# ArthurBrussee/brush

Measured on AMD Instinct MI355X. Metric: train views/sec @ 1M Gaussians, 1080p (fwd + L1/SSIM loss + bwd + Adam per view), higher is better.
Workload: dtype f32

## Files before the change

brush_amd/_ffi.py:

```python
import ctypes as C
import os

_DIR = os.path.dirname(os.path.abspath(__file__))
LIB_PATH = os.environ.get("BRUSH_HIP_LIB") or os.path.join(_DIR, "libbrush_hip.so")

FLAG_MIP = 1
FLAG_BWD_INFO = 2
FLAG_SMOOTH_CUTOFF = 4
FLAG_SLICED_LISTS = 8

fp = C.POINTER(C.c_float)
u32p = C.POINTER(C.c_uint32)


class BhCamera(C.Structure):
    _fields_ = [
        ("vm", C.c_float * 12),
        ("fx", C.c_float), ("fy", C.c_float), ("cx", C.c_float), ("cy", C.c_float),
        ("lim_pos_x", C.c_float), ("lim_pos_y", C.c_float),
        ("lim_neg_x", C.c_float), ("lim_neg_y", C.c_float),
        ("cam_pos", C.c_float * 3),
        ("img_w", C.c_uint32), ("img_h", C.c_uint32),
        ("tile_row_begin", C.c_uint32), ("tile_row_end", C.c_uint32),
        ("model", C.c_uint32), ("dist", C.c_float * 8), ("half_max_render_fov", C.c_float),
# ... 345 lines not shown
                ("reserved", C.c_uint32)]


FEATURE_TRAIN_SYMBOLS = {
    "bh_train_set_features": (C.c_int, [C.c_void_p, C.POINTER(BhFeatureField), C.POINTER(BhFeatureTarget)]),
    "bh_refine_carry_rows": (C.c_int, [C.c_void_p, C.c_void_p, C.c_void_p, C.c_uint32, C.c_uint32]),
}

REGION_BOX, REGION_ELLIPSOID = 0, 1


class BhSceneTransform(C.Structure):
    _fields_ = [("q", C.c_double * 4), ("t", C.c_double * 3), ("s", C.c_double), ("rot", C.c_float * 9), ("quat", C.c_float * 4),
                ("trans", C.c_float * 3), ("scale", C.c_float), ("log_scale", C.c_float), ("sh_rot", C.c_float * 164),
                ("reserved", C.c_uint32 * 2)]


class BhSceneRegion(C.Structure):
    _fields_ = [("kind", C.c_uint32), ("invert", C.c_uint32), ("center", C.c_float * 3), ("half_extent", C.c_float * 3),
                ("rot", C.c_float * 9), ("min_raw_opacity", C.c_float), ("reserved", C.c_uint32)]


SCENE_SYMBOLS = {
    "bh_scene_transform_make": (C.c_int, [dp, dp, C.c_double, C.POINTER(BhSceneTransform)]),
    "bh_scene_transform_compose": (C.c_int, [C.POINTER(BhSceneTransform), C.POINTER(BhSceneTransform), C.POINTER(BhSceneTransform)]),
    "bh_scene_transform_invert": (C.c_int, [C.POINTER(BhSceneTransform), C.POINTER(BhSceneTransform)]),
    "bh_camera_apply_scene_transform": (C.c_int, [C.POINTER(BhCamera), C.POINTER(BhSceneTransform), C.POINTER(BhCamera)]),
    "bh_splats_transform": (C.c_int, [C.c_void_p, C.POINTER(BhSceneTransform), C.c_uint32, C.c_uint32] + [C.c_void_p] * 6),
    "bh_splats_select_region": (C.c_int, [C.c_void_p, C.POINTER(BhSceneRegion), C.c_void_p, C.c_void_p, C.c_uint32, C.c_void_p, u32p]),
}

LIFT_MAX_LABELS, LIFT_UNASSIGNED, LIFT_ANY_LABEL = 256, 255, 0xFFFFFFFF
LIFT_VOTE_ONE = 16777216.0


class BhLiftSelect(C.Structure):
    _fields_ = [("label", C.c_uint32), ("min_share", C.c_float), ("min_weight", C.c_float), ("min_max_weight", C.c_float),
                ("min_pixels", C.c_uint32), ("invert", C.c_uint32)]


LIFT_SYMBOLS = {
    "bh_lift_accumulate": (C.c_int, [C.c_void_p, C.POINTER(BhRenderOut), C.c_void_p, C.c_uint32, C.c_void_p, C.c_void_p, C.c_void_p]),
    "bh_lift_assign": (C.c_int, [C.c_void_p, C.c_void_p, C.c_uint32, C.c_uint32, C.c_float, C.c_void_p, C.c_void_p]),
    "bh_lift_select": (C.c_int, [C.c_void_p, C.c_void_p, C.c_void_p, C.c_void_p, C.c_uint32, C.c_uint32, C.POINTER(BhLiftSelect), C.c_void_p]),
}

ENVMAP_MAX_RESOLUTION = 1024
ENVMAP_SYMBOLS = {
    "bh_envmap_create": (C.c_int, [C.c_void_p, C.c_uint32, C.POINTER(C.c_void_p)]),
    "bh_envmap_destroy": (C.c_int, [C.c_void_p, C.c_void_p]),
    "bh_envmap_set_params": (C.c_int, [C.c_void_p, C.c_void_p, fp]),
    "bh_envmap_get_params": (C.c_int, [C.c_void_p, C.c_void_p, fp]),
    "bh_envmap_get_grad": (C.c_int, [C.c_void_p, C.c_void_p, fp]),
    "bh_envmap_get_state": (C.c_int, [C.c_void_p, C.c_void_p, fp, fp, u32p]),
    "bh_envmap_set_state": (C.c_int, [C.c_void_p, C.c_void_p, fp, fp, C.c_uint32]),
    "bh_envmap_set_adam": (C.c_int, [C.c_void_p, C.c_void_p, C.c_double, C.c_double, C.c_double, C.c_double]),
    "bh_envmap_composite": (C.c_int, [C.c_void_p, C.c_void_p, C.POINTER(BhCamera), C.c_void_p, C.c_uint32, C.c_uint32, C.c_void_p]),
    "bh_envmap_backward": (C.c_int, [C.c_void_p, C.c_void_p, C.POINTER(BhCamera), C.c_void_p, C.c_void_p, C.c_uint32, C.c_uint32, C.c_void_p, C.c_int]),
    "bh_train_set_envmap": (C.c_int, [C.c_void_p, C.c_void_p]),
}

class BhCameraGradTerms(C.Structure):
    _fields_ = [("v_depth", C.c_void_p), ("v_normal", C.c_void_p), ("v_distortion", C.c_void_p), ("depth_mode", C.c_uint32),
                ("normal_mode", C.c_uint32), ("distortion", BhDistortionConfig)]


INTRINSICS_SYMBOLS = {
    "bh_render_backward_intrinsics_saved": (C.c_int, [C.c_void_p, C.POINTER(BhRenderOut)] + [C.c_void_p] * 10),
    "bh_render_backward_camera_saved": (C.c_int, [C.c_void_p, C.POINTER(BhRenderOut), C.c_void_p, C.POINTER(BhCameraGradTerms)] + [C.c_void_p] * 9),
    "bh_train_set_intrinsics_grad": (C.c_int, [C.c_void_p, C.c_void_p]),
    "bh_camera_set_intrinsics": (C.c_int, [C.POINTER(BhCamera), C.c_double, C.c_double, C.c_double, C.c_double]),
}

ABI_VERSION = 7
STRUCT_MIRRORS = (BhCamera, BhRenderOut, BhLossConfig, BhTrainConfig, BhTrainState, BhTrainBatch, BhTrainStats, BhRefineConfig, BhRefineStats, BhPlyInfo)

_lib = None
_lib_th = None
TEST_HOOKS_LIB_PATH = os.path.join(_DIR, "libbrush_hip_testhooks.so")
TEST_HOOK_SYMBOLS = {"bh_debug_fill_train_scratch": (C.c_int, [C.c_void_p, C.c_uint32]),
                     "bh_debug_split_counts": (C.c_int, [C.c_void_p, C.POINTER(C.c_uint32)]),
                     "bh_debug_depth_sort": (C.c_int, [C.c_void_p, C.c_void_p, C.c_void_p, C.c_void_p, C.c_uint32, C.c_void_p, C.c_void_p, C.c_void_p, C.c_void_p,
                                                       C.POINTER(C.c_int), C.POINTER(C.c_uint32)]),
                     "bh_debug_image_loss_window": (C.c_int, [C.c_void_p, C.c_void_p, C.c_void_p, C.c_uint32, C.c_uint32, C.POINTER(BhLossConfig), C.c_float, C.c_uint32,
                                                              C.c_uint32, C.c_void_p, C.c_void_p])}


class BrushHipError(RuntimeError):
    pass


def _bind(path, symbols):
    if not os.path.exists(path):
        raise BrushHipError(
            "%s not found: build it with `python -c 'import __graft_entry__ as g; g.build()'` "
            "(hipcc --offload-arch=gfx950). There is no CPU fallback." % path)
    lib = C.CDLL(path)
    for name, (res, args) in symbols.items():
        fn = getattr(lib, name)
        fn.restype = res
        fn.argtypes = args
    if lib.bh_abi_version() != ABI_VERSION:
        raise BrushHipError("%s speaks ABI %d, this binding ABI %d" % (path, lib.bh_abi_version(), ABI_VERSION))
    for i, mirror in enumerate(STRUCT_MIRRORS):
        if lib.bh_struct_size(i) != C.sizeof(mirror):
            raise BrushHipError("%s: sizeof(%s) is %d in the library, %d in this binding" % (path, mirror.__name__, lib.bh_struct_size(i), C.sizeof(mirror)))
    return lib


def load():
    global _lib
    if _lib is None:
        _lib = _bind(LIB_PATH, dict(SYMBOLS, **LPIPS_SYMBOLS, **COMPRESSED_PLY_SYMBOLS, **IMAGE_SYMBOLS, **DEPTH_SYMBOLS, **POSE_SYMBOLS, **EXPOSURE_SYMBOLS, **BILAGRID_SYMBOLS, **DEPTH_LOSS_SYMBOLS, **NORMAL_SYMBOLS, **NORMAL_LOSS_SYMBOLS, **DISTORTION_SYMBOLS, **MESH_SYMBOLS, **FEATURE_SYMBOLS, **FEATURE_TRAIN_SYMBOLS, **SCENE_SYMBOLS, **LIFT_SYMBOLS, **ENVMAP_SYMBOLS, **INTRINSICS_SYMBOLS))
    return _lib


def load_test_hooks():
    global _lib_th
    if _lib_th is None:
        _lib_th = _bind(TEST_HOOKS_LIB_PATH, dict(SYMBOLS, **LPIPS_SYMBOLS, **COMPRESSED_PLY_SYMBOLS, **IMAGE_SYMBOLS, **DEPTH_SYMBOLS, **POSE_SYMBOLS, **EXPOSURE_SYMBOLS, **BILAGRID_SYMBOLS, **DEPTH_LOSS_SYMBOLS, **NORMAL_SYMBOLS, **NORMAL_LOSS_SYMBOLS, **DISTORTION_SYMBOLS, **MESH_SYMBOLS, **FEATURE_SYMBOLS, **FEATURE_TRAIN_SYMBOLS, **SCENE_SYMBOLS, **LIFT_SYMBOLS, **ENVMAP_SYMBOLS, **INTRINSICS_SYMBOLS,
                                                   **TEST_HOOK_SYMBOLS))
    return _lib_th
```

brush_amd/csrc/api.hip:

```cpp
#include <cmath>
#include <cstdlib>
#include <cstdio>
#include <algorithm>
#include <cstring>
#include <new>

#include "../../include/brush_hip_intrinsics.h"
#include "context.h"
#include "device_rng.h"
#include "param_table.h"

namespace bh {

__global__ __launch_bounds__(256) void zero_two_kernel(float4* __restrict__ a, size_t na, float4* __restrict__ b, size_t nb) {
    const size_t stride = (size_t)gridDim.x * 256;
    const float4 z = make_float4(0.0f, 0.0f, 0.0f, 0.0f);
    for (size_t i = (size_t)blockIdx.x * 256 + threadIdx.x; i < na + nb; i += stride) {
        if (i < na) a[i] = z;
        else b[i - na] = z;
    }
}

int set_error(bh_ctx* ctx, int code, const std::string& msg) {
    if (ctx) ctx->last_error = msg;
    return code;
}

int check_hip(bh_ctx* ctx, hipError_t e, const char* what) {
    if (e == hipSuccess) return 0;
    std::string m = std::string(what) + ": " + hipGetErrorString(e);
    (void)hipGetLastError();
    return set_error(ctx, e == hipErrorOutOfMemory ? BH_ERR_OOM : BH_ERR_HIP, m);
}

static inline void cpu_relax() {
#if defined(__x86_64__) || defined(__i386__)
    __builtin_ia32_pause();
#elif defined(__aarch64__)
    __asm__ __volatile__("yield");
#endif
}
int wait_host_tag(bh_ctx* ctx, const volatile uint32_t* word, uint32_t want, const char* what) {
    for (uint64_t it = 1; it < (1ull << 21); ++it) {
        if (*word == want) return 0;
        if ((it & 0x3FFFull) == 0ull) {
            const hipError_t q = hipStreamQuery(ctx->stream);
            if (q == hipSuccess) break;
            if (q != hipErrorNotReady) return check_hip(ctx, q, what);
        }
        cpu_relax();
    }
    if (*word == want) return 0;
    BH_HIP(ctx, hipEventRecord(ctx->readback_ev, ctx->stream));
    BH_HIP(ctx, hipEventSynchronize(ctx->readback_ev));
    if (*word == want) return 0;
    return set_error(ctx, BH_ERR_STATE, std::string(what) + ": the kernel that signals the host never stored its tag");
}

void* ensure(bh_ctx* ctx, Slot s, size_t bytes) {
    Buffer& b = ctx->slots[s];
    if (bytes == 0) bytes = 16;
    if (b.cap >= bytes) return b.ptr;
    if (b.ptr) {
        (void)hipStreamSynchronize(ctx->stream);
        (void)hipFree(b.ptr);
        b.ptr = nullptr;
        b.cap = 0;
    }
    {
        int best = -1;
        for (size_t i = 0; i < ctx->pool.size(); ++i)
            if (ctx->pool[i].cap >= bytes && ctx->pool[i].cap <= 2 * bytes + 4096 && (best < 0 || ctx->pool[i].cap < ctx->pool[(size_t)best].cap)) best = (int)i;
        if (best >= 0) {
            b = ctx->pool[(size_t)best];
            ctx->pool.erase(ctx->pool.begin() + best);
            return b.ptr;
        }
    }
    size_t cap = bytes + bytes / 4;
    cap = (cap + 255) & ~(size_t)255;
    void* p = nullptr;
    hipError_t e = hipMalloc(&p, cap);
    if (e != hipSuccess) {
        (void)hipGetLastError();
        cap = (bytes + 255) & ~(size_t)255;
        e = hipMalloc(&p, cap);
    }
    if (e != hipSuccess) {
        char msg[160];
        snprintf(msg, sizeof msg, "hipMalloc(%zu bytes) for scratch slot %d failed: %s", cap, (int)s, hipGetErrorString(e));
        (void)hipGetLastError();
// ... 97 lines not shown
uint32_t bh_abi_version(void) { return BH_ABI_VERSION; }

uint32_t bh_struct_size(uint32_t which) {
    switch (which) {
        case BH_STRUCT_CAMERA: return (uint32_t)sizeof(BhCamera);
        case BH_STRUCT_RENDER_OUT: return (uint32_t)sizeof(BhRenderOut);
        case BH_STRUCT_LOSS_CONFIG: return (uint32_t)sizeof(BhLossConfig);
        case BH_STRUCT_TRAIN_CONFIG: return (uint32_t)sizeof(BhTrainConfig);
        case BH_STRUCT_TRAIN_STATE: return (uint32_t)sizeof(BhTrainState);
        case BH_STRUCT_TRAIN_BATCH: return (uint32_t)sizeof(BhTrainBatch);
        case BH_STRUCT_TRAIN_STATS: return (uint32_t)sizeof(BhTrainStats);
        case BH_STRUCT_REFINE_CONFIG: return (uint32_t)sizeof(BhRefineConfig);
        case BH_STRUCT_REFINE_STATS: return (uint32_t)sizeof(BhRefineStats);
        case BH_STRUCT_PLY_INFO: return (uint32_t)sizeof(BhPlyInfo);
        default: return 0u;
    }
}

bh_ctx* bh_create(int device, void* stream, int own_stream) {
    bh_ctx* ctx = new (std::nothrow) bh_ctx();
    if (!ctx) return nullptr;
    ctx->device = device;
    if (hipSetDevice(device) != hipSuccess) {
        (void)hipGetLastError();
        delete ctx;
        return nullptr;
    }
    if (!own_stream) {
        ctx->stream = (hipStream_t)stream;
        ctx->owns_stream = false;
    } else {
        if (hipStreamCreateWithFlags(&ctx->stream, hipStreamNonBlocking) != hipSuccess) {
            (void)hipGetLastError();
            delete ctx;
            return nullptr;
        }
        ctx->owns_stream = true;
    }
    if (hipHostMalloc((void**)&ctx->host_counters, bh::HOST_COUNTERS_BYTES, hipHostMallocCoherent)    != hipSuccess) {
        (void)hipGetLastError();
        if (ctx->owns_stream) (void)hipStreamDestroy(ctx->stream);
        delete ctx;
        return nullptr;
    }
    std::memset(ctx->host_counters, 0, bh::HOST_COUNTERS_BYTES);
#ifdef BH_TEST_HOOKS
    ctx->knob_break_allreduce = getenv("BH_BREAK_ALLREDUCE") != nullptr;
    if (ctx->knob_break_allreduce)
        fprintf(stderr, "brush_hip: BH_BREAK_ALLREDUCE is set - every all-reduce of this context's communicator is deliberately CORRUPTED (test hook)\n");
    if (const char* e = getenv("BH_TEST_FAIL_LOSS_AT")) {
        ctx->knob_fail_loss_at = (uint32_t)atoi(e);
        if (ctx->knob_fail_loss_at) fprintf(stderr, "brush_hip: BH_TEST_FAIL_LOSS_AT=%u - that train step of this context will FAIL on purpose (test hook)\n", ctx->knob_fail_loss_at);
    }
#endif
    if (hipEventCreateWithFlags(&ctx->readback_ev, hipEventDisableTiming) != hipSuccess ||
        hipEventCreateWithFlags(&ctx->gate_ev, hipEventDisableTiming) != hipSuccess) {
        if (ctx->readback_ev) (void)hipEventDestroy(ctx->readback_ev);
        (void)hipGetLastError();
        (void)hipHostFree(ctx->host_counters);
        if (ctx->owns_stream) (void)hipStreamDestroy(ctx->stream);
        delete ctx;
        return nullptr;
    }
    return ctx;
}

void bh_destroy(bh_ctx* ctx) {
    if (!ctx) return;
    (void)hipSetDevice(ctx->device);
    (void)hipStreamSynchronize(ctx->stream);
    prof_resolve(ctx);
    for (hipEvent_t e : ctx->prof.pool) (void)hipEventDestroy(e);
    for (auto& b : ctx->slots)
        if (b.ptr) (void)hipFree(b.ptr);
    for (auto& kv : ctx->views)
        if (kv.second.zcut) (void)hipFree(kv.second.zcut);
    for (auto& rt : ctx->retained)
        for (auto& b : rt.blocks)
            if (b.ptr) (void)hipFree(b.ptr);
    for (auto& b : ctx->pool)
        if (b.ptr) (void)hipFree(b.ptr);
    if (ctx->host_counters) (void)hipHostFree(ctx->host_counters);
    if (ctx->dsort_spl) (void)hipFree(ctx->dsort_spl);
    if (ctx->sort_groups) (void)hipFree(ctx->sort_groups);
    if (ctx->readback_ev) (void)hipEventDestroy(ctx->readback_ev);
    if (ctx->gate_ev) (void)hipEventDestroy(ctx->gate_ev);
    if (ctx->image_tab_host) (void)hipHostFree(ctx->image_tab_host);
    if (ctx->image_tab_ev) (void)hipEventDestroy(ctx->image_tab_ev);
    bh::param_tables_free_all(ctx);
    if (ctx->comm) (void)bh_comm_destroy(ctx);
    if (ctx->owns_stream) (void)hipStreamDestroy(ctx->stream);
    delete ctx;
}

const char* bh_last_error(bh_ctx* ctx) { return ctx ? ctx->last_error.c_str() : "null context"; }

int bh_sync(bh_ctx* ctx) {
    if (!ctx) return BH_ERR_INVALID_ARG;
    if (ctx->far_job.pending) {
        BH_HIP(ctx, hipSetDevice(ctx->device));
        BH_TRY(finish_far_slice(ctx, nullptr));
    }
    BH_HIP(ctx, hipStreamSynchronize(ctx->stream));
    deliver_pending_loss(ctx);
    return 0;
}

int bh_profile_enable(bh_ctx* ctx, int on) {
    if (!ctx) return BH_ERR_INVALID_ARG;
    ctx->prof.level = on < 0 ? 0 : (on > 2 ? 1 : on);
    return 0;
}

int bh_profile_fetch(bh_ctx* ctx, const char** names, float* ms, uint32_t* calls, int cap) {
    if (!ctx) return BH_ERR_INVALID_ARG;
    prof_resolve(ctx);
    Profiler& p = ctx->prof;
    const int n = p.count < cap ? p.count : cap;
    for (int i = 0; i < n; ++i) {
        names[i] = p.names[i];
        ms[i] = p.ms[i];
        calls[i] = p.calls[i];
    }
    p.count = 0;
    return n;
}

namespace {
bool parse_u32(const char* v, uint32_t lo, uint32_t hi, uint32_t* out) {
    if (!v || !*v) return false;
    char* end = nullptr;
    const unsigned long long x = strtoull(v, &end, 10);
    if (*end != '\0' || x < lo || x > hi) return false;
    *out = (uint32_t)x;
    return true;
}
bool parse_flag(const char* v, bool* out) {
    uint32_t x = 0;
    if (!parse_u32(v, 0, 1, &x)) return false;
    *out = x != 0;
    return true;
}
struct Option { const char* name; const char* help; bool (*apply)(bh_ctx* c, const char* v); };
const Option kOptions[] = {
    {"cut_min_pairs", "u32: a view whose last frame had fewer pairs keeps complete lists (= bh_set_list_cut_threshold)",
     [](bh_ctx* c, const char* v) { return parse_u32(v, 0, 0xFFFFFFFFu, &c->cut_min_pairs); }},
    {"cut_margin_pct", "0..10000: base margin behind a tile's last useful splat, % of its depth rank (default 150)",
     [](bh_ctx* c, const char* v) { return parse_u32(v, 0, 10000, &c->knob_cut_margin_pct); }},
    {"cut_margin_fixed", "0|1: the margin is cut_margin_pct for every frame instead of adaptive",
     [](bh_ctx* c, const char* v) { return parse_flag(v, &c->knob_fixed_margin); }},
    {"cut_ctrl", "up:down:floor:gap_exp — the margin controller's constants (default 1.5:0.998:0.5:0.3333)", [](bh_ctx* c, const char* v) {
        float a = 0, b = 0, d = 0, e = 0;
        if (sscanf(v, "%f:%f:%f:%f", &a, &b, &d, &e) != 4 || !(a >= 1.0f && b > 0.0f && b <= 1.0f && d > 0.0f && e >= 0.0f && e <= 1.0f)) return false;
        c->ctrl_up = a; c->ctrl_down = b; c->ctrl_floor = d; c->ctrl_gap_exp = e;
        return true;
    }},
    {"cut_sort_all", "0|1: with per-tile cuts, still depth-sort every visible splat",
     [](bh_ctx* c, const char* v) { return parse_flag(v, &c->knob_cut_sort_all); }},
    {"auto_exact_share", "0..1: a view whose last cut frame listed more than this share of its pairs renders complete lists (default 0.9; 0 = never)", [](bh_ctx* c, const char* v) {
        char* end = nullptr;
        const float x = strtof(v, &end);
        if (end == v || *end != '\0' || !(x >= 0.0f && x <= 1.0f)) return false;
        c->auto_exact_share = x;
        return true;
    }},
    {"no_view_hash", "0|1: frames without a view id share ONE table instead of being keyed by their camera",
     [](bh_ctx* c, const char* v) { return parse_flag(v, &c->knob_no_view_hash); }},
    {"k16_order", "0 index order | 1 by the view's last per-tile work | 2 dealt: the forward blend's tile order",
     [](bh_ctx* c, const char* v) { return parse_u32(v, 0, 2, &c->knob_k16_order); }},
    {"band_mode", "0|1: XCD bands of the blend kernels — contiguous eighths of the tile range, or dealt in chunks of 8 adjacent tiles (default 1)",
     [](bh_ctx* c, const char* v) { return parse_u32(v, 0, 1, &c->knob_band_mode); }},
    {"k16_waves", "0..8: forward blend: resident one-wave tiles per SIMD (0 = 8 = all resident at once; fewer: the lighter tiles are dispatched as the heavier ones finish)",
     [](bh_ctx* c, const char* v) { return parse_u32(v, 0, 8, &c->knob_k16_waves); }},
    {"k16_split", "0..1000: forward blend: a tile whose forecast work is at least max(256, k16_split / 100 x its band's mean) is blended by four quadrant waves (default 250; 0: no tile is split)",
     [](bh_ctx* c, const char* v) { return parse_u32(v, 0, 1000, &c->knob_k16_split); }},
    {"k16_split_of_max", "0..100: ... and at least this many percent of its band's heaviest tile (default 45)",
     [](bh_ctx* c, const char* v) { return parse_u32(v, 0, 100, &c->knob_k16_split_of_max); }},
    {"k16_split_min", "1..1023: a tile below this many blended splats (forecast) is never split (default 256)",
     [](bh_ctx* c, const char* v) { return parse_u32(v, 1, 1023, &c->knob_k16_split_min); }},
    {"k5_exact_spw", "16|32|64: splats per wave of the list builder for complete lists",
     [](bh_ctx* c, const char* v) { uint32_t u = 0; if (!parse_u32(v, 16, 64, &u) || !(u == 16 || u == 32 || u == 64)) return false; c->knob_k5_exact_spw = u; return true; }},
    {"bwd_jobs", "0|1: the blend backward works on checkpointed 128-entry segments of the tiles' lists (default 1) or on whole tiles",
     [](bh_ctx* c, const char* v) { return parse_flag(v, &c->knob_bwd_jobs); }},
    {"bwd_wide_rows", "0|1: the blend backward addresses the gradient accumulator in 64 bits, as it does by itself from 2^32 bytes of accumulator on (default 0)",
     [](bh_ctx* c, const char* v) { return parse_flag(v, &c->knob_bwd_wide_rows); }},
    {"no_lpt", "0|1: the blend backward takes its tiles in index order",
     [](bh_ctx* c, const char* v) { return parse_flag(v, &c->knob_no_lpt); }},
    {"lpt_classes", "log|linear: work classes of the backward's longest-first tile order — two per octave of blended splats, or 1/64 of the mean list length wide",
     [](bh_ctx* c, const char* v) { const std::string w(v); if (w == "log") { c->knob_lpt_linear = false; return true; } if (w == "linear") { c->knob_lpt_linear = true; return true; } return false; }},
    {"generic_depth_sort", "0|1: depth order by the generic radix sort + scan instead of the fused split sort",
     [](bh_ctx* c, const char* v) { return parse_flag(v, &c->knob_generic_depth_sort); }},
    {"dsort_splitters", "0|1: the fused depth sort splits at the 254 depth quantiles of the view's previous frame (default 1) or always linearly over the frame's key range",
     [](bh_ctx* c, const char* v) { return parse_flag(v, &c->knob_dsort_splitters); }},
    {"tile_sort", "auto|bucket|lsd: the forward's tile sort (auto: bucket sort unless the view's pairs are concentrated in few tiles)",
     [](bh_ctx* c, const char* v) { const std::string w(v); if (w == "auto") { c->knob_tile_sort = 0; return true; } if (w == "bucket") { c->knob_tile_sort = 1; return true; } if (w == "lsd") { c->knob_tile_sort = 2; return true; } return false; }},
    {"spec_k5", "0|1: queue the list builder before the host has read the frame's counts (default 1; 0: behind the count readback)",
     [](bh_ctx* c, const char* v) { return parse_flag(v, &c->knob_spec_k5); }},
    {"event_waits", "0|1: the host's mid-step waits use events behind the kernels instead of polled tag words",
     [](bh_ctx* c, const char* v) { return parse_flag(v, &c->knob_event_waits); }},
    {"readback_copy", "0|1: counts and gate word reach the host through copy launches",
     [](bh_ctx* c, const char* v) { return parse_flag(v, &c->knob_readback_copy); }},
    {"force_exchange", "0|1: a one-rank communicator still walks the whole gradient-exchange path (overhead measurement)",
     [](bh_ctx* c, const char* v) { return parse_flag(v, &c->knob_force_exchange); }},
    {"zero_grads", "0|1: the single-GPU train step zero-fills its gradient span like the exchange path",
     [](bh_ctx* c, const char* v) { return parse_flag(v, &c->knob_zero_grads); }},
    {"loss_bands", "0|1: the fused loss's blocks take their tiles by XCD column bands (1) or row-major (0)",
     [](bh_ctx* c, const char* v) { return parse_u32(v, 0, 1, &c->knob_loss_bands); }},
    {"update_rows", "0|64|128|256: splats per block of the update kernel (0 = default)",
     [](bh_ctx* c, const char* v) { uint32_t u = 0; if (!parse_u32(v, 0, 256, &u) || !(u == 0 || u == 64 || u == 128 || u == 256)) return false; c->knob_update_rows = u; return true; }},
    {"no_dormant", "0|1: the update kernel fetches and updates dormant splats like everyone else",
     [](bh_ctx* c, const char* v) { return parse_flag(v, &c->knob_no_dormant); }},
    {"sort_kpt", "0|4|8|16: keys per thread of the generic radix sort (0 = default)",
     [](bh_ctx* c, const char* v) { uint32_t u = 0; if (!parse_u32(v, 0, 16, &u) || !(u == 0 || u == 4 || u == 8 || u == 16)) return false; c->knob_sort_kpt = u; return true; }},
    {"grad_allreduce", "ring|direct: the dense gradient block's collective — ncclAllReduce, or reduce-scatter + all-gather over grouped send/recv",
     [](bh_ctx* c, const char* v) { const std::string w(v); if (w == "ring") { c->knob_direct_allreduce = false; return true; } if (w == "direct") { c->knob_direct_allreduce = true; return true; } return false; }},
    {"update_sparse", "0..256: an update block with at most this many non-dormant rows fetches them in one round trip (0: never; 256: every block that may skip dormant rows; default 64 at SH degree 0, else 0)",
     [](bh_ctx* c, const char* v) { uint32_t u = 0; if (!parse_u32(v, 0, 256, &u)) return false; c->knob_update_sparse = (int)u; return true; }},
    {"feature_chunk", "0|4|8|16: channels per pass over the lists of the feature-map blends (0 = chosen per channel count)",
     [](bh_ctx* c, const char* v) { uint32_t u = 0; if (!parse_u32(v, 0, 16, &u) || !(u == 0 || u == 4 || u == 8 || u == 16)) return false; c->feature_chunk = u; return true; }},
};
constexpr int kOptionCount = (int)(sizeof(kOptions) / sizeof(kOptions[0]));
}

extern "C" int bh_option_count(void) { return kOptionCount; }
extern "C" const char* bh_option_name(int i) { return i >= 0 && i < kOptionCount ? kOptions[i].name : nullptr; }
extern "C" const char* bh_option_help(int i) { return i >= 0 && i < kOptionCount ? kOptions[i].help : nullptr; }

extern "C" int bh_set_option(bh_ctx* ctx, const char* key, const char* value) {
    if (!ctx) return BH_ERR_INVALID_ARG;
    if (!key || !value) return set_error(ctx, BH_ERR_INVALID_ARG, "set_option: null key or value");
    const std::string k(key);
    for (const Option& o : kOptions) {
        if (k != o.name) continue;
        if (!o.apply(ctx, value)) return set_error(ctx, BH_ERR_INVALID_ARG, "set_option: bad value '" + std::string(value) + "' for '" + k + "'");
        return 0;
    }
    return set_error(ctx, BH_ERR_INVALID_ARG, "set_option: unknown key '" + k + "' (bh_option_name lists the keys)");
}

namespace {
struct Kb4Law {
    double k[4];
    explicit Kb4Law(const float* d) { for (int i = 0; i < 4; ++i) k[i] = d ? (double)d[i] : 0.0; }
    double value(double th) const {
        const double t2 = th * th, t3 = t2 * th, t5 = t3 * t2, t7 = t5 * t2, t9 = t7 * t2;
        return th + k[0] * t3 + k[1] * t5 + k[2] * t7 + k[3] * t9;
    }
    double slope(double th) const {
        const double t2 = th * th, t4 = t2 * t2, t6 = t4 * t2, t8 = t6 * t2;
        return 1.0 + 3.0 * k[0] * t2 + 5.0 * k[1] * t4 + 7.0 * k[2] * t6 + 9.0 * k[3] * t8;
    }
    double invert(double target) const {
        if (target <= 0.0) return 0.0;
        const double pi = 3.14159265358979323846;
        double th = target < pi - 1e-6 ? target : pi - 1e-6;
        for (int it = 0; it < 50; ++it) {
            const double fp = slope(th);
            if (std::fabs(fp) < 1e-12) break;
            double next = th - (value(th) - target) / fp;
            next = next < 0.0 ? 0.0 : (next > pi ? pi : next);
            const bool done = std::fabs(next - th) < 1e-12;
            th = next;
            if (done) break;
        }
        return th;
    }
};
struct Rt8Law {
    double k[6];
    explicit Rt8Law(const float* d) { for (int i = 0; i < 6; ++i) k[i] = d ? (double)d[i] : 0.0; }
    double radial(double r) const {
        const double r2 = r * r, r4 = r2 * r2, r6 = r4 * r2;
        return (1.0 + k[0] * r2 + k[1] * r4 + k[2] * r6) / (1.0 + k[3] * r2 + k[4] * r4 + k[5] * r6);
    }
    double undistort(double r_d) const {
        double r = r_d;
// ... 140 lines not shown
    if (!ctx) return BH_ERR_INVALID_ARG;
    if (!cam || !out || !background) return set_error(ctx, BH_ERR_INVALID_ARG, "render_forward: null argument");
    ForwardRequest req;
    req.cam = *cam;
    req.n = n; req.sh_degree = sh_degree; req.flags = flags;
    req.transforms = transforms; req.sh_coeffs = sh_coeffs; req.raw_opacities = raw_opacities;
    req.bg[0] = background[0]; req.bg[1] = background[1]; req.bg[2] = background[2];
    req.view_id = ctx->view_id;
    return render_forward(ctx, req, out);
}

int bh::forward_impl(bh_ctx* ctx, const ForwardRequest& req, BhRenderOut* out) {
    const uint32_t n = req.n, sh_degree = req.sh_degree, flags = req.flags;
    const float* transforms = req.transforms;
    const float* sh_coeffs = req.sh_coeffs;
    const float* raw_opacities = req.raw_opacities;
    ctx->have_forward = false;
    ctx->clears.begin_forward();
    const bool mip = flags & BH_FLAG_MIP;
    Frame f;
    f.bwd_info = flags & BH_FLAG_BWD_INFO; f.smooth = flags & BH_FLAG_SMOOTH_CUTOFF;
    f.bg[0] = req.bg[0]; f.bg[1] = req.bg[1]; f.bg[2] = req.bg[2];
    f.u = make_uniforms(req.cam);
    if (f.u.tile_y0 >= f.u.tile_y1 || f.u.tile_y1 > f.u.tile_bh) return set_error(ctx, BH_ERR_INVALID_ARG, "tile_row window must satisfy begin < end <= ceil(img_h / 16)");
    f.num_tiles = f.u.tile_bw * f.u.tile_bh;
    const size_t npad = n ? n : 1;

    constexpr size_t counter_set_bytes = COUNTER_SET_BYTES, counter_set_words = COUNTER_SET_BYTES / 4, counter_read_bytes = COUNTER_READ_BYTES;
    auto* counter_pairs = (uint32_t*)ensure(ctx, SLOT_COUNTERS, 2 * counter_set_bytes + 64);
    uint32_t* dev_sums = counter_pairs ? counter_pairs + 2 * counter_set_words : nullptr;
    uint32_t* counters = counter_pairs ? counter_pairs + counter_set_words * (ctx->counter_phase & 1u) : nullptr;
    auto* depth_keys = (uint32_t*)ensure(ctx, SLOT_DEPTH_KEYS, npad * 4);
    auto* isect_counts = (uint32_t*)ensure(ctx, SLOT_ISECT_COUNTS, npad * 4);
    auto* max_radius = req.max_radius ? req.max_radius : (float*)ensure(ctx, SLOT_MAX_RADIUS, npad * 4);
    f.proj_by_gid = (float*)ensure(ctx, SLOT_PROJECTED_BY_GID, npad * 9 * 4);
    if (!counters || !depth_keys || !isect_counts || !max_radius || !f.proj_by_gid) return BH_ERR_OOM;

    f.gfc = (uint32_t*)ensure(ctx, SLOT_GLOBAL_FROM_COMPACT, npad * 4);
    auto* depths_sorted = (uint32_t*)ensure(ctx, SLOT_DEPTHS_SORTED, npad * 4);
    if (!f.gfc || !depths_sorted) return BH_ERR_OOM;
    const bool bwd_jobs = f.bwd_info && ctx->knob_bwd_jobs && !ctx->knob_no_lpt && !((flags & BH_FLAG_SLICED_LISTS) && ctx->slice_fraction > 0.0f);
    const size_t lpt_words = LPT_HEADER_WORDS + (size_t)8 * LPT_CLASSES * band_slots(f.num_tiles);
    auto* tile_offsets = (uint32_t*)ensure(ctx, SLOT_TILE_OFFSETS, ((size_t)f.num_tiles * 2 + lpt_words) * 4);
    f.visible = (f.bwd_info && req.visible) ? req.visible : (float*)ensure(ctx, SLOT_VISIBLE, (f.bwd_info ? npad : 1) * 4);
    if (!tile_offsets || !f.visible) return BH_ERR_OOM;
    const size_t visible_words = f.bwd_info ? ((req.visible && req.visible_floats) ? req.visible_floats : npad) : 0;
    const bool want_sliced = (flags & BH_FLAG_SLICED_LISTS) != 0;
    const size_t slice_bit_words = ((size_t)f.num_tiles + 31) / 32;
    const size_t slice_group_words = (size_t)n / (256 * FAR_GROUP_BLOCKS) + 2;
    const size_t slice_words = want_sliced ? SLICE_CTRL_WORDS + slice_bit_words + (size_t)f.num_tiles * 2 + slice_group_words : 0;
    uint32_t* slice_tab = nullptr;
    if (want_sliced) {
        slice_tab = (uint32_t*)ensure(ctx, SLOT_SLICE, slice_words * 4);
        if (!slice_tab) return BH_ERR_OOM;
    }
    ViewState* view = nullptr;
    bool cut_active = false;
    const bool auto_cuts = want_sliced && !(ctx->slice_fraction > 0.0f);
    const bool order_only = !want_sliced && ctx->knob_k16_order != 0u && n >= 8u * 256u;
    if (n > 0 && (auto_cuts || order_only)) {
        view = frame_view(ctx, req, f.u.tile_bw, f.u.tile_bh, order_only && !f.bwd_info);
        if (!view && auto_cuts) return set_error(ctx, BH_ERR_OOM, "hipMalloc for the per-view tile table failed");
        if (!view) (void)hipGetLastError();
        cut_active = auto_cuts && view && cut_this_frame(ctx, view, req.allow_cut);
    }
    uint32_t* const vtab = view_table(view);
    uint32_t* near_counts = nullptr;
    uint32_t* tile_order = nullptr;
    uint32_t* tile_split = nullptr;
    if (cut_active) {
        near_counts = (uint32_t*)ensure(ctx, SLOT_NEAR_COUNTS, npad * 4);
        if (!near_counts) return BH_ERR_OOM;
    }

    uint32_t near_total = 0, nv_true = 0;
    bool fused_scan = false;
    uint32_t* cum_early = nullptr;
    bool k5_queued = false;
    uint32_t spec_pair_cap = 0;
    float* spec_projected = nullptr;
    float4* spec_vc = nullptr;
    uint32_t *spec_tile_ids = nullptr, *spec_isect_gids = nullptr;
    if (n > 0) {
        {
            ProfScope ps(ctx, "ProjectSplats");
            if (!ctx->counters_ready) BH_HIP(ctx, hipMemsetAsync(counter_pairs, 0, 2 * counter_set_bytes, ctx->stream));
            ctx->counters_ready = false;
            ForwardPrep prep;
            prep.next_counters = reinterpret_cast<unsigned long long*>(counter_pairs + counter_set_words * ((ctx->counter_phase & 1u) ^ 1u));
            prep.visible = visible_words ? reinterpret_cast<uint32_t*>(f.visible) : nullptr;
            prep.visible_words = (uint32_t)visible_words;
            prep.tile_table = tile_offsets;
            prep.tile_words = f.num_tiles * 2 + LPT_HEADER_WORDS;
            prep.slice_table = slice_tab;
            prep.slice_words = (uint32_t)slice_words;
            prep.list_all_visible = ctx->knob_cut_sort_all;
            if (view && ctx->knob_k16_order && n >= 8u * 256u) {
                const uint32_t win_t = f.u.tile_bw * (f.u.tile_y1 - f.u.tile_y0);
                tile_order = (uint32_t*)ensure(ctx, SLOT_TILE_ORDER, ((size_t)8 * band_slots(win_t) + SPLIT_TAIL_WORDS) * 4);
                if (!tile_order) return BH_ERR_OOM;
                prep.order_work = vtab + (size_t)f.num_tiles;
                prep.order_out = tile_order;
                prep.order_tiles = win_t;
                prep.order_tile_begin = f.u.tile_bw * f.u.tile_y0;
                prep.order_mode = ctx->knob_k16_order;
                prep.band_mode = ctx->knob_band_mode;
                if (ctx->knob_k16_split && ctx->knob_k16_order == 1u) {
                    tile_split = tile_order + (size_t)8 * band_slots(win_t);
                    prep.split_out = tile_split;
                    prep.split_factor = (float)ctx->knob_k16_split * 0.01f;
                    prep.split_min = ctx->knob_k16_split_min;
                    prep.split_of_max = (float)ctx->knob_k16_split_of_max * 0.01f;
                }
            }
            if (f.bwd_info && req.grad_begin && req.grad_floats && (req.grad_floats & 3u) == 0 &&
                (reinterpret_cast<uintptr_t>(req.grad_begin) & 15u) == 0 && req.grad_floats / 4 <= 0xFFFFFFFFull) {
                prep.span = reinterpret_cast<float4*>(req.grad_begin);
                prep.span_f4 = (uint32_t)(req.grad_floats / 4);
                ctx->clears.k1_cleared_span();
            }
            BH_TRY(launch_project_forward(ctx, f.u, n, mip, sh_degree, transforms, sh_coeffs, raw_opacities, depth_keys, isect_counts, max_radius,
                                          f.proj_by_gid, counters, prep, cut_active ? vtab : nullptr, near_counts));
            ctx->counter_phase ^= 1u;
            ctx->counters_ready = true;
        }
        auto* hslots = reinterpret_cast<unsigned long long*>(ctx->host_counters + 16);
        fused_scan = depth_sort_supported(n) && !ctx->knob_generic_depth_sort;
        const bool sums_on_device = fused_scan && !ctx->knob_readback_copy;
        const bool poll_tag = sums_on_device && !ctx->knob_event_waits;
        if (!sums_on_device) {
            BH_HIP(ctx, hipMemcpyAsync(hslots, counters, counter_read_bytes, hipMemcpyDeviceToHost, ctx->stream));
            BH_HIP(ctx, hipEventRecord(ctx->readback_ev, ctx->stream));
        }
        {
            ProfScope ps(ctx, "DepthSort");
            if (fused_scan) {
                cum_early = (uint32_t*)ensure(ctx, SLOT_CUM_TILES_HIT, npad * 4);
                if (!cum_early) return BH_ERR_OOM;
                if (poll_tag && ++ctx->readback_tag == 0u) ctx->readback_tag = 1u;
                bool* spl_written = nullptr;
                uint32_t* spl = view_splitters(view, cut_active, &spl_written);
                BH_TRY(depth_sort_scan(ctx, depth_keys, counters + COUNTER_MINMAX_WORD, cut_active ? near_counts : isect_counts, n, depths_sorted, f.gfc, cum_early,
                                       sums_on_device ? counters : nullptr, ctx->host_counters + 16, ctx->readback_ev, poll_tag ? ctx->readback_tag : 0u,
                                       sums_on_device ? dev_sums : nullptr, spl, spl_written));
            } else {
                BH_TRY(radix_argsort(ctx, depth_keys, nullptr, n, 32, depths_sorted, f.gfc));
            }
        }
        if (poll_tag && ctx->knob_spec_k5 && !(want_sliced && ctx->slice_fraction > 0.0f)) {
            const size_t cap_pairs = std::min(ctx->slots[SLOT_TILE_IDS].cap, ctx->slots[SLOT_ISECT_GIDS].cap) / 4;
            if (cap_pairs >= 4096) {
                spec_projected = (float*)ensure(ctx, SLOT_PROJECTED, npad * 9 * 4);
                spec_vc = f.bwd_info ? (float4*)ensure(ctx, SLOT_V_COMBINED, npad * 10 * 4 + 16) : nullptr;
                if (!spec_projected || (f.bwd_info && !spec_vc)) return BH_ERR_OOM;
                spec_tile_ids = (uint32_t*)ctx->slots[SLOT_TILE_IDS].ptr;
                spec_isect_gids = (uint32_t*)ctx->slots[SLOT_ISECT_GIDS].ptr;
                spec_pair_cap = (uint32_t)std::min<size_t>(cap_pairs, 0xFFFFFFFEull);
                ProfScope ps(ctx, "MapGaussiansToIntersect");
                BH_TRY(launch_map_gaussians(ctx, n, f.u, f.proj_by_gid, f.gfc, spec_projected, cum_early, spec_tile_ids, spec_isect_gids, spec_vc,
                                            spec_vc ? (uint32_t)(((size_t)n * 10 + 3) / 4) : 0u, 0xFFFFFFFFu, cut_active ? slice_tab : nullptr,
                                            cut_active ? vtab : nullptr, cut_active ? depths_sorted : nullptr, dev_sums + (cut_active ? 3 : 0), spec_pair_cap));
                k5_queued = true;
            }
        }
        if (poll_tag) BH_TRY(wait_host_tag(ctx, reinterpret_cast<const volatile uint32_t*>(hslots) + HOST_SUM_WORDS - 1u, ctx->readback_tag, "count readback"));
        else BH_HIP(ctx, hipEventSynchronize(ctx->readback_ev));
        if (ctx->gate_learn) {
            ctx->gate_learn = false;
            ctx->far_direct = reinterpret_cast<const volatile uint32_t*>(ctx->host_counters)[HOST_GATE_WORD] != 0u;
        }
        unsigned long long hc[4] = {0ull, 0ull, 0ull, 0ull};
        if (sums_on_device) {
            const volatile unsigned long long* hs = hslots;
            for (uint32_t c = 0; c < COUNTER_K1_U64; ++c) hc[c] = hs[c];
        } else {
            for (uint32_t k = 0; k < COUNTER_SLOTS; ++k)
                for (uint32_t c = 0; c < COUNTER_K1_U64; ++c) hc[c] += hslots[COUNTER_K1_U64 * k + c];
        }
        if (hc[1] > 0xFFFFFFFFull) return set_error(ctx, BH_ERR_UNSUPPORTED, "more than 2^32-1 tile intersections");
        nv_true = (uint32_t)hc[0];
        f.ni = (uint32_t)hc[1];
        near_total = cut_active ? (uint32_t)hc[2] : f.ni;
        f.nv = cut_active ? (uint32_t)hc[3] : nv_true;
    } else {
        BH_HIP(ctx, hipMemsetAsync(tile_offsets, 0, ((size_t)f.num_tiles * 2 + LPT_HEADER_WORDS) * 4, ctx->stream));
        if (visible_words) BH_HIP(ctx, hipMemsetAsync(f.visible, 0, visible_words * 4, ctx->stream));
    }

    const size_t nvpad = f.nv ? f.nv : 1, nipad = f.ni ? f.ni : 1;
    f.cum = fused_scan ? cum_early : (uint32_t*)ensure(ctx, SLOT_CUM_TILES_HIT, nvpad * 4);
    f.projected = (float*)ensure(ctx, SLOT_PROJECTED, nvpad * 9 * 4);
    f.tile_ids = (uint32_t*)ensure(ctx, SLOT_TILE_IDS, nipad * 4);
    f.isect_gids = (uint32_t*)ensure(ctx, SLOT_ISECT_GIDS, nipad * 4);
    f.tile_ids_sorted = (uint32_t*)ensure(ctx, SLOT_TILE_IDS_SORTED, nipad * 4);
    f.isect_gids_sorted = (uint32_t*)ensure(ctx, SLOT_ISECT_GIDS_SORTED, nipad * 4);
    const size_t pixels = (size_t)f.u.img_w * f.u.img_h;
    void* out_img = ensure(ctx, SLOT_OUT_IMG, pixels * (f.bwd_info ? 16 : 4));
    if (!f.cum || !f.projected || !f.tile_ids || !f.isect_gids || !f.tile_ids_sorted || !f.isect_gids_sorted || !out_img)
        return BH_ERR_OOM;
    if (k5_queued && ((cut_active ? near_total : f.ni) > spec_pair_cap || f.projected != spec_projected || f.tile_ids != spec_tile_ids || f.isect_gids != spec_isect_gids))
        k5_queued = false;

    f.budget = want_sliced && f.ni > 0 ? list_budget(ctx, cut_active ? view : nullptr, near_total, f.ni) : f.ni;
    const bool sliced = f.budget < f.ni;
    const bool by_cut = cut_active && sliced;
    const uint32_t* zcut_lists = cut_active ? vtab : nullptr;
    f.slice_info = slice_tab;
    f.done_bits = slice_tab ? slice_tab + SLICE_CTRL_WORDS : nullptr;
    f.tile_offsets_far = slice_tab ? slice_tab + SLICE_CTRL_WORDS + slice_bit_words : nullptr;
    f.far_group_totals = slice_tab ? slice_tab + SLICE_CTRL_WORDS + slice_bit_words + (size_t)f.num_tiles * 2 : nullptr;
    while (f.tile_bits < 32 && (f.num_tiles >> f.tile_bits) != 0) f.tile_bits++;
    if (bwd_jobs) {
        const uint32_t listed = cut_active ? near_total : f.ni;
        const uint32_t ckpt_cap = (uint32_t)std::min<uint64_t>((uint64_t)listed / BWD_SEG + f.num_tiles + 1u, BWD_CKPT_MAX_SLOTS);
        f.rs.jobs.ckpt = (float4*)ensure(ctx, SLOT_BWD_CKPT, (size_t)ckpt_cap * 256 * sizeof(float4));
        f.rs.jobs.ckpt_cap = ckpt_cap;
        f.rs.jobs.top_cap = band_slots(f.num_tiles) + ckpt_cap;
        f.rs.jobs.top_list = (uint32_t*)ensure(ctx, SLOT_BWD_TOPLIST, (size_t)8 * f.rs.jobs.top_cap * 4);
        if (!f.rs.jobs.ckpt || !f.rs.jobs.top_list) return BH_ERR_OOM;
    }
    if (view) {
        f.rs.zcut = vtab;
        f.rs.depth_keys_sorted = depths_sorted;
        f.rs.nv = f.nv;
        f.rs.cut_active = by_cut;
        f.rs.margin_pct = cut_margin_pct(ctx, view);
        f.rs.work = vtab + (size_t)f.num_tiles;
        f.rs.order = tile_order;
        f.rs.order_mode = ctx->knob_k16_order;
        f.rs.split = tile_split;
#ifdef BH_TEST_HOOKS
        ctx->last_split = tile_split;
#endif
    }
    const uint32_t win_tiles = f.u.tile_bw * (f.u.tile_y1 - f.u.tile_y0);
    const float class_width_raw = (float)f.ni / (float)(win_tiles ? win_tiles : 1u) / 64.0f;
    f.class_width = ctx->knob_lpt_linear ? (class_width_raw < 8.0f ? 8.0f : class_width_raw) : 0.0f;
    f.lpt = (f.bwd_info && !ctx->knob_no_lpt) ? tile_offsets + (size_t)f.num_tiles * 2 : nullptr;
    f.out_f32 = f.bwd_info ? (float*)out_img : nullptr;
    f.out_u8 = f.bwd_info ? nullptr : (uint32_t*)out_img;

    bool offsets_done = false;
    if (f.nv > 0) {
        if (!fused_scan) {
            ProfScope ps(ctx, "PrefixSumGaussHits");
            BH_TRY(prefix_sum(ctx, cut_active ? near_counts : isect_counts, f.gfc, f.nv, f.cum, false));
        }
        if (f.ni == 0) {
            ProfScope ps(ctx, "ProjectVisible");
            BH_TRY(launch_project_visible(ctx, f.nv, f.proj_by_gid, f.gfc, f.projected));
        }
        if (f.ni > 0) {
            {
                ProfScope ps(ctx, "MapGaussiansToIntersect");
                float4* vc = nullptr;
                if (f.bwd_info) {
                    vc = (float4*)ensure(ctx, SLOT_V_COMBINED, (size_t)f.nv * 10 * 4 + 16);
                    if (!vc) return BH_ERR_OOM;
                }
                if (zcut_lists && near_total == 0u) {
                } else if (k5_queued && (!f.bwd_info || vc == spec_vc)) {
                    ctx->clears.k5_cleared_accum(vc != nullptr);
                } else {
                    ctx->clears.k5_cleared_accum(vc != nullptr);
                    BH_TRY(launch_map_gaussians(ctx, f.nv, f.u, f.proj_by_gid, f.gfc, f.projected, f.cum, f.tile_ids, f.isect_gids, vc, vc ? (uint32_t)(((size_t)f.nv * 10 + 3) / 4) : 0u,
                                                (sliced && !by_cut) ? f.budget : 0xFFFFFFFFu, (sliced || zcut_lists) ? f.slice_info : nullptr, zcut_lists,
// ... 53 lines not shown
        if (ctx->far_direct && !by_cut) {
            BH_TRY(enqueue_far_slice(ctx, j));
            ctx->gate_learn = true;
        } else {
            if (++ctx->gate_tag == 0u) ctx->gate_tag = 1u;
            j.gate_tag = ctx->gate_tag;
            ctx->gate_signal_queued = false;
            j.gate_event_recorded = !(req.defer_decision && !ctx->knob_event_waits && !ctx->knob_readback_copy);
            if (j.gate_event_recorded) BH_HIP(ctx, hipEventRecord(ctx->gate_ev, ctx->stream));
            j.pending = true;
            if (!req.defer_decision) {
                bool again = false;
                BH_TRY(finish_far_slice(ctx, &again));
                if (by_cut && again) {
                    *out = ctx->latest.out;
                    return 0;
                }
            }
        }
    }

    BhRenderOut r{};
    r.num_visible = nv_true;
    r.num_listed_splats = f.nv;
    r.num_intersections = f.ni;
    r.num_tiles = f.num_tiles;
    r.tile_bw = f.u.tile_bw;
    r.tile_bh = f.u.tile_bh;
    r.flags = flags;
    r.out_img = f.bwd_info ? (float*)out_img : nullptr;
    r.out_img_packed = f.bwd_info ? nullptr : (uint32_t*)out_img;
    r.visible = f.bwd_info ? f.visible : nullptr;
    r.max_radius = max_radius;
    r.tile_offsets = tile_offsets;
    r.projected = f.projected;
    r.compact_gid_from_isect = f.isect_gids_sorted;
    r.tile_id_from_isect = f.tile_ids_sorted;
    r.global_from_compact_gid = f.gfc;
    r.cum_tiles_hit = f.cum;
    r.intersect_counts = isect_counts;
    r.depths_sorted = (float*)depths_sorted;
    r.tile_offsets_far = sliced ? f.tile_offsets_far : nullptr;
    r.list_budget = f.budget;
    r.generation = ++ctx->generation;
    ctx->clears.stamp(r.generation);
    *out = r;
    ForwardState& latest = ctx->latest;
    latest.out = r;
    latest.uniforms = f.u;
    latest.n = n; latest.sh_degree = sh_degree; latest.flags = flags;
    latest.bg[0] = f.bg[0]; latest.bg[1] = f.bg[1]; latest.bg[2] = f.bg[2];
    latest.lpt = f.lpt;
    latest.jobs = f.rs.jobs;
    ctx->have_forward = true;
    if (view) view_rendered(view, f.ni);
    return 0;
}

extern "C" {

int bh_set_list_slicing(bh_ctx* ctx, float near_share) {
    if (!ctx) return BH_ERR_INVALID_ARG;
    if (near_share != near_share || near_share > 1.0f) return set_error(ctx, BH_ERR_INVALID_ARG, "set_list_slicing: the near slice's share must be <= 1 (<= 0: automatic)");
    ctx->slice_fraction = near_share > 0.0f ? near_share : 0.0f;
    return 0;
}

int bh_set_list_cut_threshold(bh_ctx* ctx, uint32_t min_pairs) {
    if (!ctx) return BH_ERR_INVALID_ARG;
    ctx->cut_min_pairs = min_pairs;
    return 0;
}

int bh_set_view_id(bh_ctx* ctx, uint32_t view_id) {
    if (!ctx) return BH_ERR_INVALID_ARG;
    ctx->view_id = view_id;
    return 0;
}

int bh_forget_views(bh_ctx* ctx) {
    if (!ctx) return BH_ERR_INVALID_ARG;
    BH_HIP(ctx, hipSetDevice(ctx->device));
    if (ctx->far_job.pending) BH_TRY(finish_far_slice(ctx, nullptr));
    if (ctx->dsort_spl) { BH_HIP(ctx, hipMemsetAsync(ctx->dsort_spl, 0, DSORT_SPL_STRIDE * 4, ctx->stream)); ctx->dsort_spl_written = false; }
    if (ctx->views.empty()) return 0;
    BH_HIP(ctx, hipStreamSynchronize(ctx->stream));
    deliver_pending_loss(ctx);
    for (auto& kv : ctx->views)
        if (kv.second.zcut) (void)hipFree(kv.second.zcut);
    ctx->views.clear();
    ctx->casual_views = 0;
    for (uint64_t& k : ctx->seen_keys) k = 0ull;
    ctx->far_job.view = nullptr;
    ctx->margin_scale = 1.0f;
    return 0;
}

float bh_last_list_share(bh_ctx* ctx) { return ctx ? ctx->last_slice_share : 0.0f; }
uint32_t bh_far_slices_queued(bh_ctx* ctx) { return ctx ? ctx->far_launches : 0u; }
uint32_t bh_view_table_count(bh_ctx* ctx) { return ctx ? (uint32_t)ctx->views.size() : 0u; }

}

namespace bh {

int backward_impl(bh_ctx* ctx, const ForwardState& fs, const float* v_output, const BackwardCall& call) {
    const float *transforms = call.transforms, *sh_coeffs = call.sh_coeffs, *raw_opacities = call.raw_opacities;
    float *v_transforms = call.v_transforms, *v_sh_coeffs = call.v_sh_coeffs, *v_raw_opacities = call.v_raw_opacities, *v_refine_weight = call.v_refine_weight;
    const size_t span_floats = call.span_floats;
    const BhRenderOut& r = fs.out;
    const uint32_t n = fs.n, nv = r.num_listed_splats, C = (fs.sh_degree + 1) * (fs.sh_degree + 1);
    const size_t nvpad = nv ? nv : 1;
    auto* v_combined = (float*)ensure(ctx, SLOT_V_COMBINED, nvpad * 10 * 4 + 16);
    if (!v_combined) return BH_ERR_OOM;
    bool row_marks = false;
    float* v_z = nullptr;
    const float* v_n = nullptr;
    const float* v_f = nullptr;
    {
        ProfScope ps(ctx, "ZeroGradBuffers");
        const bool one_span = n > 0 && span_floats;
        const bool vc_done = ctx->clears.take_accum(r.generation);
        const GradClears::Span span = ctx->clears.take_span(r.generation);
        row_marks = span == GradClears::ROW_MARKS;
        if (row_marks && !one_span) return set_error(ctx, BH_ERR_STATE, "internal: row-marked gradients without the train step's gradient span");
        const bool span_done = one_span && span != GradClears::NONE;
        if (one_span && (span_floats & 3u) == 0 && (reinterpret_cast<uintptr_t>(v_transforms) & 15u) == 0) {
            const size_t na = vc_done ? 0 : (nvpad * 10 + 3) / 4, nb = span_done ? 0 : span_floats / 4;
            if (na + nb) {
                hipLaunchKernelGGL(zero_two_kernel, dim3(2048), dim3(256), 0, ctx->stream, reinterpret_cast<float4*>(v_combined), na,
                                   reinterpret_cast<float4*>(v_transforms), nb);
                BH_LAUNCH_CHECK(ctx, "zero_two_kernel");
            }
        } else {
            if (!vc_done) BH_HIP(ctx, hipMemsetAsync(v_combined, 0, nvpad * 10 * 4, ctx->stream));
            if (n > 0) {
                if (one_span) {
                    BH_HIP(ctx, hipMemsetAsync(v_transforms, 0, span_floats * 4, ctx->stream));
                } else {
                    BH_HIP(ctx, hipMemsetAsync(v_transforms, 0, (size_t)n * 10 * 4, ctx->stream));
                    BH_HIP(ctx, hipMemsetAsync(v_sh_coeffs, 0, (size_t)n * C * 3 * 4, ctx->stream));
                    BH_HIP(ctx, hipMemsetAsync(v_raw_opacities, 0, (size_t)n * 4, ctx->stream));
                    BH_HIP(ctx, hipMemsetAsync(v_refine_weight, 0, (size_t)n * 4, ctx->stream));
                }
            }
        }
    }
    {
        ProfScope ps(ctx, "RasterizeBackwards", true);
        if (r.num_intersections > 0 && v_output)
            BH_TRY(launch_rasterize_backward(ctx, fs.uniforms, fs.bg, fs.flags & BH_FLAG_SMOOTH_CUTOFF,
                                             r.compact_gid_from_isect, r.tile_offsets, r.projected, r.out_img, v_output, v_combined, fs.lpt,
                                             r.tile_offsets_far, call.want_refine, &fs.jobs, nv));
        if (call.depth) BH_TRY(launch_depth_backward(ctx, fs, *call.depth, v_combined, &v_z));
        if (call.normal) BH_TRY(launch_normal_backward(ctx, fs, *call.normal, transforms, v_combined, &v_n));
        if (call.distortion) BH_TRY(launch_distortion_backward(ctx, fs, *call.distortion, v_combined, &v_z));
        if (call.feature) BH_TRY(launch_feature_backward(ctx, fs, *call.feature, v_combined, &v_f));
    }
    {
        ProfScope ps(ctx, "ProjectBackwards");
        BH_TRY(launch_project_backward(ctx, fs.uniforms, nv, fs.flags & BH_FLAG_MIP, fs.sh_degree, transforms, sh_coeffs,
                                       raw_opacities, r.global_from_compact_gid, v_combined, v_transforms, v_sh_coeffs,
                                       v_raw_opacities, v_refine_weight, row_marks, r.projected));
        if (v_z) BH_TRY(launch_depth_vz_scatter(ctx, fs, v_z, v_transforms, row_marks, v_sh_coeffs, v_raw_opacities, v_refine_weight));
        if (v_n) BH_TRY(launch_normal_vn_scatter(ctx, fs, v_n, transforms, v_transforms, row_marks, v_sh_coeffs, v_raw_opacities, v_refine_weight));
        if (v_f) BH_TRY(launch_feature_scatter(ctx, fs, *call.feature, v_f));
    }
// ... 212 lines not shown
        const float v = strength > 0.0f ? base[k] + (2.0f * u[k] - 1.0f) * strength : base[k];
        out[k] = v < 0.0f ? 0.0f : (v > 1.0f ? 1.0f : v);
    }
}

int bh_normal_samples(bh_ctx* ctx, uint64_t seed, uint32_t step, uint64_t n, float* out) {
    if (!ctx) return BH_ERR_INVALID_ARG;
    if (n > 0 && !out) return set_error(ctx, BH_ERR_INVALID_ARG, "normal_samples: null argument");
    if (n > 0xFFFFFFFFull) return set_error(ctx, BH_ERR_INVALID_ARG, "normal_samples: n must fit 32 bits (the splat index is one counter word)");
    BH_HIP(ctx, hipSetDevice(ctx->device));
    return launch_normal_samples(ctx, out, n, seed, step);
}

int bh_fold_min_scale(bh_ctx* ctx, const float* transforms, const float* raw_opacities, const float* min_scale, uint32_t n,
                      float* out_transforms, float* out_raw_opacities) {
    if (!ctx) return BH_ERR_INVALID_ARG;
    if (n > 0 && (!transforms || !raw_opacities || !min_scale || !out_transforms || !out_raw_opacities))
        return set_error(ctx, BH_ERR_INVALID_ARG, "fold_min_scale: null argument");
    BH_HIP(ctx, hipSetDevice(ctx->device));
    return launch_fold_min_scale(ctx, transforms, raw_opacities, min_scale, n, out_transforms, out_raw_opacities);
}

int bh_fold_min_scale_backward(bh_ctx* ctx, const float* transforms, const float* raw_opacities, const float* min_scale, uint32_t n,
                               float* v_transforms, float* v_raw_opacities) {
    if (!ctx) return BH_ERR_INVALID_ARG;
    if (n > 0 && (!transforms || !raw_opacities || !min_scale || !v_transforms || !v_raw_opacities))
        return set_error(ctx, BH_ERR_INVALID_ARG, "fold_min_scale_backward: null argument");
    BH_HIP(ctx, hipSetDevice(ctx->device));
    return launch_fold_min_scale_backward(ctx, transforms, raw_opacities, min_scale, n, v_transforms, v_raw_opacities);
}

int bh_compute_min_scale(bh_ctx* ctx, const float* transforms, uint32_t n, const float* view_cams, uint32_t num_views, float factor,
                         float* out) {
    if (!ctx) return BH_ERR_INVALID_ARG;
    if (!(factor > 0.0f) || num_views == 0) return set_error(ctx, BH_ERR_INVALID_ARG, "compute_min_scale: needs factor > 0 and at least one view camera");
    if (!view_cams || (n > 0 && (!transforms || !out))) return set_error(ctx, BH_ERR_INVALID_ARG, "compute_min_scale: null argument");
    BH_HIP(ctx, hipSetDevice(ctx->device));
    return launch_compute_min_scale(ctx, transforms, n, view_cams, num_views, factor, out);
}

}

extern "C" int bh_tile_sort_offsets(bh_ctx* ctx, const uint32_t* tile_ids, const uint32_t* compact_gids, uint32_t n, uint32_t num_tiles,
                                    uint32_t* tile_ids_sorted, uint32_t* compact_gids_sorted, uint32_t* tile_offsets) {
    if (!ctx) return BH_ERR_INVALID_ARG;
    if (!tile_offsets || (n > 0 && (!tile_ids || !compact_gids || !tile_ids_sorted || !compact_gids_sorted)))
        return set_error(ctx, BH_ERR_INVALID_ARG, "tile_sort_offsets: null argument");
    if (num_tiles == 0) return set_error(ctx, BH_ERR_INVALID_ARG, "tile_sort_offsets: num_tiles == 0");
    BH_HIP(ctx, hipSetDevice(ctx->device));
    uint32_t bits = 0;
    while (bits < 32 && (num_tiles >> bits) != 0) bits++;
    BH_HIP(ctx, hipMemsetAsync(tile_offsets, 0, (size_t)num_tiles * 2 * 4, ctx->stream));
    if (n == 0) return 0;
    if (tile_sort_supported(bits, n) && !(ctx->knob_tile_sort == 2u))
        return tile_sort_offsets(ctx, tile_ids, compact_gids, n, bits, num_tiles, tile_ids_sorted, compact_gids_sorted, tile_offsets);
    BH_TRY(radix_argsort(ctx, tile_ids, compact_gids, n, bits, tile_ids_sorted, compact_gids_sorted));
    return launch_tile_offsets(ctx, tile_ids_sorted, n, num_tiles, tile_offsets, true);
}

#ifdef BH_TEST_HOOKS
extern "C" int bh_debug_split_counts(bh_ctx* ctx, uint32_t* out) {
    if (!ctx || !out) return BH_ERR_INVALID_ARG;
    if (!ctx->last_split) return 0;
    BH_HIP(ctx, hipSetDevice(ctx->device));
    BH_HIP(ctx, hipMemcpyAsync(out, ctx->last_split, 8 * 4, hipMemcpyDeviceToHost, ctx->stream));
    BH_HIP(ctx, hipStreamSynchronize(ctx->stream));
    return 1;
}
extern "C" int bh_debug_depth_sort(bh_ctx* ctx, const uint32_t* keys, const uint32_t* minmax, const uint32_t* counts, uint32_t n, uint32_t* out_keys, uint32_t* out_vals,
                                   uint32_t* cum, uint32_t* spl, int* spl_written, uint32_t* totals_out) {
    if (!ctx) return BH_ERR_INVALID_ARG;
    if (!keys || !minmax || !counts || !out_keys || !out_vals || !cum || !totals_out || (spl && !spl_written))
        return set_error(ctx, BH_ERR_INVALID_ARG, "debug_depth_sort: null argument");
    if (n == 0 || !depth_sort_supported(n)) return set_error(ctx, BH_ERR_INVALID_ARG, "debug_depth_sort: n is outside the fused sort's reach");
    BH_HIP(ctx, hipSetDevice(ctx->device));
    bool written = spl_written ? *spl_written != 0 : false;
    BH_TRY(depth_sort_scan(ctx, keys, minmax, counts, n, out_keys, out_vals, cum, nullptr, nullptr, nullptr, 0u, nullptr, spl, spl ? &written : nullptr));
    if (spl) *spl_written = written ? 1 : 0;
    else if (spl_written) *spl_written = ctx->dsort_spl_written ? 1 : 0;
    BH_HIP(ctx, hipMemcpyAsync(totals_out, ctx->slots[SLOT_SORT_HIST].ptr, 2 * 256 * 4, hipMemcpyDeviceToHost, ctx->stream));
    BH_HIP(ctx, hipStreamSynchronize(ctx->stream));
    return 0;
}
extern "C" int bh_debug_image_loss_window(bh_ctx* ctx, const float* img_hwc4, const uint32_t* gt_packed, uint32_t h, uint32_t w, const BhLossConfig* cfg,
                                          float alpha_weight, uint32_t tile_y0, uint32_t tile_y1, float* loss_out, float* v_output) {
    if (!ctx) return BH_ERR_INVALID_ARG;
    if (!img_hwc4 || !gt_packed || !cfg || !loss_out || !v_output || h == 0 || w == 0)
        return set_error(ctx, BH_ERR_INVALID_ARG, "debug_image_loss_window: bad argument");
    if (tile_y0 >= tile_y1) return set_error(ctx, BH_ERR_INVALID_ARG, "debug_image_loss_window: empty tile-row window");
    BH_HIP(ctx, hipSetDevice(ctx->device));
    const size_t hw = (size_t)h * w;
    const bool alpha = alpha_weight > 0.0f;
    BH_TRY(launch_image_loss_fused_window(ctx, img_hwc4, gt_packed, h, w, *cfg, alpha, 1.0f / (float)(hw * 3), alpha ? alpha_weight / (float)hw : 0.0f, tile_y0,
                                          tile_y1, loss_out, v_output, nullptr, nullptr, 0u));
    BH_HIP(ctx, hipStreamSynchronize(ctx->stream));
    return 0;
}
#endif
```

brush_amd/csrc/context.h:

```cpp
#pragma once
#include <hip/hip_runtime.h>
#include <stdint.h>

#include <memory>
#include <string>
#include <unordered_map>
#include <vector>

#include "../../include/brush_hip.h"
#include "../../include/brush_hip_lpips.h"
#include "../../include/brush_hip_image.h"
#include "../../include/brush_hip_exposure.h"
#include "../../include/brush_hip_bilagrid.h"
#include "../../include/brush_hip_depth_loss.h"
#include "../../include/brush_hip_normal_loss.h"
#include "../../include/brush_hip_distortion.h"
#include "../../include/brush_hip_mesh.h"
#include "../../include/brush_hip_features.h"
#include "../../include/brush_hip_feature_train.h"
#include "../../include/brush_hip_envmap.h"
#include "device_math.h"

namespace bh {

enum Slot : int {
    SLOT_COUNTERS = 0,
    SLOT_DEPTH_KEYS,
    SLOT_ISECT_COUNTS,
    SLOT_MAX_RADIUS,
    SLOT_SORT_KEYS_A,
    SLOT_SORT_KEYS_B,
    SLOT_SORT_VALS_A,
    SLOT_SORT_VALS_B,
    SLOT_SORT_HIST,
    SLOT_COMM_SCRATCH,
    SLOT_BWD_CKPT,
    SLOT_BWD_TOPLIST,
    SLOT_SORT_PARTS,
    SLOT_SCAN_SUMS,
    SLOT_GLOBAL_FROM_COMPACT,
    SLOT_DEPTHS_SORTED,
    SLOT_CUM_TILES_HIT,
    SLOT_PROJECTED,
    SLOT_TILE_IDS,
    SLOT_ISECT_GIDS,
    SLOT_TILE_IDS_SORTED,
    SLOT_ISECT_GIDS_SORTED,
    SLOT_TILE_OFFSETS,
    SLOT_OUT_IMG,
    SLOT_VISIBLE,
    SLOT_V_COMBINED,
    SLOT_LOSS_MAP,
    SLOT_V_OUTPUT,
    SLOT_GRADS,
    SLOT_STATS,
    SLOT_LOSS_SCALAR,
    SLOT_MISC,
    SLOT_REFINE,
    SLOT_REFINE_BOUNDS,
    SLOT_FOLDED_TRANSFORMS,
    SLOT_FOLDED_RAW_OPAC,
    SLOT_PLY_ROWS,
    SLOT_EXCH_BLOCKS,
    SLOT_EXCH_IDX,
    SLOT_EXCH_COMPACT,
    SLOT_PROJECTED_BY_GID,
    SLOT_SLICE,
    SLOT_SLICE_STATE,
    SLOT_SLICE_COUNTS,
    SLOT_SLICE_CUM,
    SLOT_NEAR_COUNTS,
    SLOT_TILE_ORDER,
    SLOT_LOD_GRADS,
    SLOT_LOD_FOLDED,
    SLOT_LOD_LOSS,
    SLOT_LOD_SORT,
    SLOT_KNN,
    SLOT_EVAL,
    SLOT_LPIPS,
    SLOT_PLY_COMPRESS,
    SLOT_IMAGE,
    SLOT_DEPTH,
    SLOT_POSE,
    SLOT_INTRINSICS,
    SLOT_EXPOSURE,
    SLOT_CORRECTED,
    SLOT_PIXEL_LOSS,
    SLOT_DEPTH_TERM,
    SLOT_NORMAL,
    SLOT_NORMAL_TERM,
    SLOT_DISTORTION,
    SLOT_DISTORTION_TERM,
    SLOT_BILAGRID,
    SLOT_TSDF,
    SLOT_FEATURES,
    SLOT_FEATURE_TERM,
    SLOT_FEATURE_GRAD,
    SLOT_ENVMAP_FRAME,
    SLOT_SCENE,
    SLOT_COUNT
};

struct Buffer {
    void* ptr = nullptr;
    size_t cap = 0;
};

constexpr int MAX_PROF = 32;

constexpr uint32_t COUNTER_SLOTS = 128;
constexpr uint32_t COUNTER_K1_U64 = 4;
constexpr size_t COUNTER_SET_BYTES = COUNTER_SLOTS * 8 * COUNTER_K1_U64 + COUNTER_SLOTS * 8;
constexpr uint32_t COUNTER_SET_U64 = (uint32_t)(COUNTER_SET_BYTES / 8);
constexpr uint32_t COUNTER_MINMAX_WORD = COUNTER_SLOTS * 2 * COUNTER_K1_U64;
constexpr uint32_t SLICE_CTRL_WORDS = 8;
constexpr uint32_t SORT_GROUP_BLOCKS = 32;
constexpr uint32_t FAR_GROUP_BLOCKS = 64;
constexpr size_t COUNTER_READ_BYTES = COUNTER_SLOTS * 8 * COUNTER_K1_U64;
constexpr uint32_t HOST_SUM_WORDS = 2 * COUNTER_K1_U64 + 1;
constexpr size_t HOST_LOSS_WORD = 16 + COUNTER_READ_BYTES / 4;
constexpr size_t HOST_GATE_WORD = HOST_LOSS_WORD + 16;
constexpr size_t HOST_GATE_TAG_WORD = HOST_GATE_WORD + 1;
constexpr size_t HOST_COUNTERS_BYTES = 64 + COUNTER_READ_BYTES + 64 + 64;

struct Profiler {
    int level = 0;
    const char* names[MAX_PROF];
    float ms[MAX_PROF];
    uint32_t calls[MAX_PROF];
    int count = 0;
    struct Pending { int idx; hipEvent_t a, b; };
    std::vector<Pending> pending;
    std::vector<hipEvent_t> pool;
    hipEvent_t ext_a = nullptr, ext_b = nullptr;
};

constexpr uint32_t ZCUT_ALL = 0xFFFFFFFEu;
BH_DEV bool zcut_near(uint32_t key, uint32_t cut) { return (key >> 1) <= (cut >> 1); }
struct ViewState {
    uint32_t* zcut = nullptr;
    uint32_t tile_bw = 0, tile_bh = 0;
    bool seeded = false;
    uint32_t exact_frames = 0;
    uint32_t penalty = 0;
    uint64_t last_used = 0;
    uint32_t gap = 0;
    uint32_t last_pairs = 0;
    uint32_t complete_frames = 0;
    bool spl_written[2] = {false, false};
    bool casual = false;
};
constexpr uint32_t CUT_MIN_PAIRS = 1500000u;
constexpr uint32_t LPT_CLASSES = 64;
constexpr uint32_t LPT_HEADER_WORDS = 8 * LPT_CLASSES + 64;
constexpr uint32_t BWD_SEG = 128;
constexpr uint32_t BWD_MAX_SEGS = 64;
struct BwdJobs {
    float4* ckpt = nullptr;
    uint32_t ckpt_cap = 0;
    uint32_t* top_list = nullptr;
    uint32_t top_cap = 0;
};
constexpr uint32_t BAND_CHUNK = 4;
inline __host__ __device__ uint32_t band_slots(uint32_t num_tiles) {
    const uint32_t p = (num_tiles + 7u) / 8u;
    return ((p + BAND_CHUNK - 1u) / BAND_CHUNK) * BAND_CHUNK;
}
inline __host__ __device__ uint32_t band_tile(uint32_t band, uint32_t i, uint32_t per, uint32_t mode) {
    return mode ? ((i / BAND_CHUNK) * 8u + band) * BAND_CHUNK + (i % BAND_CHUNK) : band * per + i;
}
BH_DEV uint32_t tile_of_block(uint32_t b, uint32_t num_tiles, uint32_t band_mode) {
    const uint32_t per = band_slots(num_tiles);
    const uint32_t i = b >> 3;
    return i < per ? band_tile(b & 7u, i, per, band_mode) : 0xFFFFFFFFu;
}
constexpr uint32_t SPLIT_MAX = 128;
constexpr uint32_t SPLIT_MIN_WORK = 256;
constexpr uint32_t SPLIT_TAIL_WORDS = 8u + 8u * SPLIT_MAX * 4u;
constexpr uint32_t BWD_CKPT_MAX_SLOTS = 96u * 1024u;
constexpr uint32_t DSORT_SPL_STRIDE = 260;
constexpr uint32_t VIEW_SPL_WORDS = 2 * DSORT_SPL_STRIDE;
constexpr size_t MAX_VIEW_STATES = 4096;
constexpr uint64_t DIRECT_ALLREDUCE_MIN_FLOATS = 1u << 16;
constexpr uint32_t AUTO_EXACT_FRAMES = 12;
constexpr size_t CASUAL_VIEW_STATES = 32;
constexpr size_t SEEN_KEYS = 64;
constexpr size_t VIEW_TABLE_BYTES = (size_t)256 << 20;

struct RasterSlice {
    uint32_t* done_bits = nullptr;
    uint32_t* unsat_count = nullptr;
    uint32_t* gate_host = nullptr;
    float* state = nullptr;
    const uint32_t* offsets_near = nullptr;
    uint32_t* zcut = nullptr;
    const uint32_t* depth_keys_sorted = nullptr;
    uint32_t nv = 0;
    bool cut_active = false;
    uint32_t* live_bands = nullptr;
    uint32_t* work = nullptr;
    const uint32_t* order = nullptr;
    uint32_t order_mode = 1;
    uint32_t* split = nullptr;
    uint32_t margin_pct = 150;
    BwdJobs jobs{};
};

struct ForwardRequest {
    BhCamera cam{};
    uint32_t n = 0, sh_degree = 0, flags = 0;
    const float* transforms = nullptr;
    const float* sh_coeffs = nullptr;
    const float* raw_opacities = nullptr;
    float bg[3] = {0, 0, 0};
    uint32_t view_id = 0;
    float* visible = nullptr;
    float* max_radius = nullptr;
    size_t visible_floats = 0;
    float* grad_begin = nullptr;
    size_t grad_floats = 0;
    bool defer_decision = false;
    bool allow_cut = true;
};

struct Frame {
    ViewUniforms u{};
    float bg[3] = {0, 0, 0};
    bool bwd_info = false, smooth = false;
    uint32_t nv = 0, ni = 0, budget = 0, num_tiles = 0, tile_bits = 0;
    float* proj_by_gid = nullptr;
    uint32_t* gfc = nullptr;
    float* projected = nullptr;
    uint32_t* cum = nullptr;
    uint32_t* slice_info = nullptr;
    uint32_t* done_bits = nullptr;
    uint32_t* tile_offsets_far = nullptr;
    uint32_t* far_counts = nullptr;
    uint32_t* far_block_totals = nullptr;
    uint32_t* far_group_totals = nullptr;
    uint32_t* tile_ids = nullptr;
    uint32_t* isect_gids = nullptr;
    uint32_t* tile_ids_sorted = nullptr;
    uint32_t* isect_gids_sorted = nullptr;
    float* out_f32 = nullptr;
    uint32_t* out_u8 = nullptr;
    float* visible = nullptr;
    uint32_t* lpt = nullptr;
    float class_width = 8.0f;
    RasterSlice rs{};
};

struct FarJob {
    bool pending = false;
    Frame frame{};
    bool gate_event_recorded = false;
    uint32_t gate_tag = 0;
    bool by_cut = false;
    ViewState* view = nullptr;
    bool view_shared = false;
    ForwardRequest req{};
};

struct GradClears {
    enum Span : uint8_t { NONE = 0, ZEROED, ROW_MARKS };
// ... 81 lines not shown
    bool normal_attached = false;
    BhNormalTermConfig normal_term{};
    bool distortion_attached = false;
    BhDistortionTermConfig distortion_term{};
    bool feature_attached = false;
    BhFeatureField feature_field{};
    BhFeatureTarget feature_target{};
    bh_exposure* exposure = nullptr;
    bh_bilagrid* bilagrid = nullptr;
    float bilagrid_tv_weight = 0.0f;
    bh_envmap* envmap = nullptr;

    bool lpips_on() const { return lpips != nullptr && lpips_weight > 0.0f; }
    bool depth_on() const { return depth_attached && depth_target.weight > 0.0f; }
    bool normal_on() const { return normal_attached && normal_term.weight > 0.0f; }
    bool distortion_on() const { return distortion_attached; }
    bool feature_on() const { return feature_attached && feature_target.weight > 0.0f; }
};

}


struct bh_ctx {
    int device = 0;
    hipStream_t stream = nullptr;
    bool owns_stream = false;
    std::string last_error;
    bh::Buffer slots[bh::SLOT_COUNT];
    uint32_t* host_counters = nullptr;
    hipEvent_t readback_ev = nullptr;
    hipEvent_t gate_ev = nullptr;
    bool counters_ready = false;
    uint32_t counter_phase = 0;
    bool have_forward = false;
    bh::ForwardState latest;
    uint64_t generation = 0;
    std::vector<bh::Retained> retained;
    std::vector<bh::Buffer> pool;
    bh::GradClears clears;
    float* pending_loss_dst = nullptr;
    void* image_tab_host = nullptr;
    size_t image_tab_cap = 0;
    hipEvent_t image_tab_ev = nullptr;
    bh::StepTerms terms;
    std::vector<bh::ParamTable*> param_tables;
    void* comm = nullptr;
    hipStream_t comm_stream = nullptr;
    hipEvent_t comm_ev = nullptr;
    int comm_rank = 0, comm_world = 1;
    float slice_fraction = 0.0f;
    float last_slice_share = 1.0f;
    bool far_direct = false;
    uint32_t readback_tag = 0;
    uint32_t gate_tag = 0;
    bool gate_signal_queued = false;
    bool gate_learn = false;
    uint32_t far_launches = 0;
    std::unordered_map<uint64_t, bh::ViewState> views;
    uint64_t seen_keys[bh::SEEN_KEYS] = {};
    uint32_t seen_pos = 0;
    uint32_t casual_views = 0;
    uint32_t view_id = 0;
    uint64_t view_clock = 0;
    float margin_scale = 1.0f;
    float ctrl_up = 1.5f, ctrl_down = 0.998f, ctrl_floor = 0.5f, ctrl_gap_exp = 1.0f / 3.0f;
    uint32_t cut_min_pairs = bh::CUT_MIN_PAIRS;
    bool knob_spec_k5 = true;
    bool knob_event_waits = false;
    bool knob_readback_copy = false;
    bool knob_no_view_hash = false;
    bool knob_fixed_margin = false;
    bool knob_cut_sort_all = false;
    uint32_t feature_chunk = 0;
    uint32_t knob_band_mode = 1;
    uint32_t knob_k16_waves = 0;
    uint32_t knob_k16_split = 250;
    uint32_t knob_k16_split_min = bh::SPLIT_MIN_WORK;
    uint32_t knob_k16_split_of_max = 45;
    const uint32_t* last_split = nullptr;
    uint32_t knob_k16_order = 1;
    uint32_t knob_cut_margin_pct = 150;
    bh::FarJob far_job;
    uint32_t refine_n = 0, refine_new_n = 0;
    bool dsort_lds_raised = false;
    uint32_t* sort_groups = nullptr;
    size_t sort_groups_cap = 0, sort_groups_dirty = 0;
    uint32_t sort_groups_cur = 0;
    uint32_t* dsort_spl = nullptr;
    bool dsort_spl_written = false;
    bool knob_dsort_splitters = true;
    bool adam_lds_raised = false;
    uint32_t update_lds_raised = 0;
    size_t lds_optin_max = 0;
    bool knob_no_lpt = false;
    bool knob_bwd_wide_rows = false;
    bool knob_bwd_jobs = true;
    bool knob_lpt_linear = false;
    bool knob_force_exchange = false;
    bool knob_break_allreduce = false;
    bool knob_generic_depth_sort = false;
    bool knob_zero_grads = false;
    uint32_t knob_fail_loss_at = 0;
    uint32_t train_steps_seen = 0;
    uint32_t knob_loss_bands = 1;
    uint32_t knob_tile_sort = 0;
    float auto_exact_share = 0.9f;
    bool knob_direct_allreduce = false;
    uint32_t knob_k5_exact_spw = 32;
    bool knob_no_dormant = false;
    int knob_update_sparse = -1;
    uint32_t knob_update_rows = 0;
    uint32_t knob_sort_kpt = 0;
    const void* marks_m2_sh = nullptr; const void* marks_m1_t = nullptr; uint32_t marks_n = 0, marks_step = 0;
    bh::Profiler prof;
};

namespace bh {

int set_error(bh_ctx* ctx, int code, const std::string& msg);
int forward_impl(bh_ctx* ctx, const ForwardRequest& req, BhRenderOut* out);
int wait_host_tag(bh_ctx* ctx, const volatile uint32_t* word, uint32_t want, const char* what);
int find_saved_bwd_forward(bh_ctx* ctx, const BhRenderOut* saved, int not_bwd_code, const char* who, const ForwardState** fs);
int backward_impl(bh_ctx* ctx, const ForwardState& fs, const float* v_output, const BackwardCall& call);
int render_forward(bh_ctx* ctx, const ForwardRequest& req, BhRenderOut* out);
enum : uint32_t { NEED_V_OUTPUT = 1u, NEED_V_DEPTH = 2u, NEED_V_NORMAL = 4u, NEED_V_DISTORTION = 8u, NEED_V_VIEWMAT = 16u, NEED_V_FEATURES = 32u, NEED_V_INTRINSICS = 64u };
int backward_entry(bh_ctx* ctx, const char* who, int not_bwd_code, uint32_t required, const BhRenderOut* saved, const float* v_output, BackwardCall call);
int launch_depth_backward(bh_ctx* ctx, const ForwardState& fs, const DepthTerm& term, float* v_combined, float** v_z);
int launch_depth_vz_scatter(bh_ctx* ctx, const ForwardState& fs, const float* v_z, float* v_transforms, bool mark_rows, float* v_sh_coeffs,
                            float* v_raw_opacities, float* v_refine_weight);
int launch_depth_forward(bh_ctx* ctx, const ForwardState& fs, uint32_t mode, float* out_depth);
int launch_normal_backward(bh_ctx* ctx, const ForwardState& fs, const NormalTerm& term, const float* transforms, float* v_combined, const float** v_n);
int launch_normal_vn_scatter(bh_ctx* ctx, const ForwardState& fs, const float* v_n, const float* transforms, float* v_transforms, bool mark_rows,
                             float* v_sh_coeffs, float* v_raw_opacities, float* v_refine_weight);
int launch_normal_map(bh_ctx* ctx, const ForwardState& fs, const float* transforms, uint32_t mode, float* out);
int launch_normal_loss(bh_ctx* ctx, const BhCamera& cam, const float* normal, const float* depth, const float* image, uint32_t h, uint32_t w, float weight,
                       bool accumulate_v_depth, float* loss, float* v_normal, float* v_depth, float* accum, float* accum_host);
int launch_distortion_backward(bh_ctx* ctx, const ForwardState& fs, const DistortionTerm& term, float* v_combined, float** v_z);
int launch_distortion_map(bh_ctx* ctx, const ForwardState& fs, const DistortionTerm& term, bool moments, float* out);
int check_distortion_kind(bh_ctx* ctx, uint32_t kind, float near_z, float far_z, const char* who);
int launch_distortion_loss(bh_ctx* ctx, const float* map, uint32_t h, uint32_t w, uint32_t channels, float weight, float* loss, float* accum,
                           float* accum_host);
int launch_feature_backward(bh_ctx* ctx, const ForwardState& fs, const FeatureTerm& term, float* v_combined, const float** v_compact);
int launch_feature_scatter(bh_ctx* ctx, const ForwardState& fs, const FeatureTerm& term, const float* v_compact);
int launch_feature_gather(bh_ctx* ctx, const ForwardState& fs, const float* features, uint32_t channels, float* feat);
int launch_feature_forward(bh_ctx* ctx, const ForwardState& fs, uint32_t channels, const float* feat, float* out);
int feature_term_rows(bh_ctx* ctx, const ForwardState& fs, uint32_t channels, float** feat);
int launch_feature_loss(bh_ctx* ctx, const float* map, const BhFeatureTarget& t, float* loss, float* v_map, float* accum, float* accum_host);
int launch_depth_loss(bh_ctx* ctx, const float* depth, const BhDepthTarget& t, float* loss, float* v_depth, float* accum, float* accum_host);
double* loss_partials(bh_ctx* ctx, uint64_t pixels, uint32_t* blocks);
int launch_loss_pair_final(bh_ctx* ctx, uint32_t rows, const double* partials, float c, float* loss, float* accum, float* accum_host);
int launch_pose_grad(bh_ctx* ctx, const ViewUniforms& u, uint32_t nv, bool mip, uint32_t sh_degree, const float* transforms,
                     const float* sh, const uint32_t* gid, const float* v_combined, float* v_viewmat);
int launch_intrinsics_grad(bh_ctx* ctx, const ViewUniforms& u, uint32_t nv, bool mip, const float* transforms, const uint32_t* gid,
                           const float* v_combined, float* v_intrinsics);
int launch_exposure_apply(bh_ctx* ctx, const bh_exposure* tab, uint32_t view, const float* img, uint32_t h, uint32_t w, float* out);
int launch_exposure_backward(bh_ctx* ctx, bh_exposure* tab, uint32_t view, const float* img, const float* v_exposed, uint32_t h, uint32_t w,
                             float* v_img, bool update);
int launch_bilagrid_slice(bh_ctx* ctx, const bh_bilagrid* tab, uint32_t view, const float* img, uint32_t h, uint32_t w, float* out);
int launch_bilagrid_backward(bh_ctx* ctx, bh_bilagrid* tab, uint32_t view, const float* img, const float* v_sliced, uint32_t h, uint32_t w, float* v_img,
                             float tv_weight, bool update);
int launch_bilagrid_tv(bh_ctx* ctx, const bh_bilagrid* tab, uint32_t view, float* value, float weight, float* accum, float* accum_host);
float* bilagrid_tv_scratch(bh_ctx* ctx);
int check_envmap_frame(bh_ctx* ctx, const BhCamera* cam, uint32_t h, uint32_t w, const char* who);
int launch_envmap_composite(bh_ctx* ctx, const bh_envmap* map, const BhCamera& cam, const float* img, uint32_t h, uint32_t w, float* out);
int launch_envmap_backward(bh_ctx* ctx, bh_envmap* map, const BhCamera& cam, const float* img, const float* v_out, uint32_t h, uint32_t w, float* v_img,
                           bool update, float gscale, bool check_host);
int launch_envmap_adam(bh_ctx* ctx, bh_envmap* map, float gscale);
ViewState* frame_view(bh_ctx* ctx, const ForwardRequest& req, uint32_t tile_bw, uint32_t tile_bh, bool casual);
bool cut_this_frame(const bh_ctx* ctx, ViewState* vs, bool allow_cut);
uint32_t* view_table(const ViewState* vs);
uint32_t* view_splitters(ViewState* vs, bool cut, bool** written);
uint32_t cut_margin_pct(const bh_ctx* ctx, const ViewState* vs);
uint32_t list_budget(bh_ctx* ctx, ViewState* cut_view, uint32_t near_total, uint32_t ni);
void view_rendered(ViewState* vs, uint32_t ni);
int enqueue_far_slice(bh_ctx* ctx, const FarJob& j);
int finish_far_slice(bh_ctx* ctx, bool* launched);
bool far_job_decides_first(const bh_ctx* ctx);
void drop_far_job(bh_ctx* ctx);
inline void deliver_pending_loss(bh_ctx* ctx) {
    if (ctx->pending_loss_dst) {
        *ctx->pending_loss_dst = reinterpret_cast<const volatile float*>(ctx->host_counters)[HOST_LOSS_WORD];
        ctx->pending_loss_dst = nullptr;
    }
}
int check_hip(bh_ctx* ctx, hipError_t e, const char* what);
int lpips_train_term(bh_ctx* ctx, const float* img_hwc4, const uint32_t* gt_packed, uint32_t h, uint32_t w, const float* bg, float* v_output,
                     float* loss, float* loss_host);
std::string ply_header_comments(uint32_t sh_degree, bool render_mip, const float* up_axis);
enum ResizeOut : int { RESIZE_OUT_U8 = 0, RESIZE_OUT_PACKED = 1, RESIZE_OUT_PACKED_PREMUL = 2 };
size_t resize_table_bytes(uint32_t src, uint32_t dst, uint32_t filter);
void build_resize_table(uint32_t src, uint32_t dst, uint32_t filter, void* host);
using ResizeTable = std::shared_ptr<const std::vector<uint8_t>>;
ResizeTable resize_table(uint32_t src, uint32_t dst, uint32_t filter);
hipError_t enqueue_resize(hipStream_t st, const uint8_t* src, uint32_t w, uint32_t h, uint32_t channels, uint32_t nw, uint32_t nh,
                          const int32_t* vtab, const int32_t* htab, float* tmp, void* out, int mode);
hipError_t enqueue_mask_merge(hipStream_t st, const uint8_t* img, uint32_t channels, const uint8_t* mask, uint64_t pixels, int invert,
                              int premultiply, uint32_t* out);
void* ensure(bh_ctx* ctx, Slot s, size_t bytes);

struct ProfScope {
    bh_ctx* ctx;
    int idx = -1;
    hipEvent_t a = nullptr, b = nullptr;
    ProfScope(bh_ctx* c, const char* name, bool dominant = false);
    ~ProfScope();
};

#define BH_HIP(ctx, expr)                                            \
    do {                                                             \
        hipError_t _e = (expr);                                      \
        if (_e != hipSuccess) return bh::check_hip(ctx, _e, #expr);  \
    } while (0)
#define BH_TRY(expr)            \
    do {                        \
        int _rc = (expr);       \
        if (_rc != 0) return _rc; \
    } while (0)
#define BH_LAUNCH_CHECK(ctx, what)                                      \
    do {                                                                \
        hipError_t _e = hipGetLastError();                              \
        if (_e != hipSuccess) return bh::check_hip(ctx, _e, what);      \
    } while (0)

ViewUniforms make_uniforms(const BhCamera& c);


struct ForwardPrep {
    unsigned long long* next_counters = nullptr;
    uint32_t* visible = nullptr;
    uint32_t visible_words = 0;
    uint32_t* tile_table = nullptr;
    uint32_t tile_words = 0;
    float4* span = nullptr;
    uint32_t span_f4 = 0;
    uint32_t* slice_table = nullptr;
    uint32_t slice_words = 0;
    const uint32_t* order_work = nullptr;
    uint32_t* order_out = nullptr;
    uint32_t order_tiles = 0, order_tile_begin = 0;
    uint32_t order_mode = 1;
    uint32_t band_mode = 0;
    uint32_t* split_out = nullptr;
    float split_factor = 2.5f;
    uint32_t split_min = SPLIT_MIN_WORK;
    float split_of_max = 0.45f;
    bool list_all_visible = false;
};
int launch_project_forward(bh_ctx* ctx, const ViewUniforms& u, uint32_t n, bool mip, uint32_t sh_degree, const float* transforms,
                           const float* sh, const float* raw_opac, uint32_t* depth_keys, uint32_t* isect_counts, float* max_radius,
                           float* projected_by_gid, uint32_t* counters, const ForwardPrep& prep, uint32_t* zcut = nullptr,
                           uint32_t* near_counts = nullptr);
int launch_project_visible(bh_ctx* ctx, uint32_t nv, const float* projected_by_gid, const uint32_t* gid, float* projected);
int launch_map_gaussians(bh_ctx* ctx, uint32_t nv, const ViewUniforms& u, const float* projected_by_gid, const uint32_t* gid,
                         float* projected, const uint32_t* cum_tiles_hit, uint32_t* tile_ids, uint32_t* isect_gids,
                         float4* zero_span = nullptr, uint32_t zero_f4 = 0, uint32_t budget = 0xFFFFFFFFu, uint32_t* slice_info = nullptr,
                         const uint32_t* zcut = nullptr, const uint32_t* depth_keys_sorted = nullptr, const uint32_t* nv_dev = nullptr, uint32_t pair_cap = 0xFFFFFFFFu);
int launch_map_gaussians_far(bh_ctx* ctx, uint32_t nv, const ViewUniforms& u, const float* projected_by_gid, const uint32_t* gid,
                             float* projected, const uint32_t* cum_tiles_hit, uint32_t budget, const uint32_t* done_bits, const uint32_t* gate,
                             uint32_t* counts, uint32_t* block_totals, uint32_t* group_totals, uint32_t* slice_info, uint32_t* tile_ids, uint32_t* isect_gids);
int launch_project_backward(bh_ctx* ctx, const ViewUniforms& u, uint32_t nv, bool mip, uint32_t sh_degree,
                            const float* transforms, const float* sh, const float* raw_opac, const uint32_t* gid,
                            float* v_combined, float* v_transforms, float* v_sh, float* v_raw_opac,
                            float* v_refine, bool mark_written = false, const float* projected = nullptr);
struct SortGroups {
    uint32_t* sums = nullptr;
    uint32_t* stale = nullptr;
    uint32_t stale_words = 0;
};
inline uint32_t sort_group_count(uint32_t nblocks) { return (nblocks + SORT_GROUP_BLOCKS - 1u) / SORT_GROUP_BLOCKS; }
int sort_groups_next(bh_ctx* ctx, size_t words, SortGroups* out);
constexpr uint32_t SORT_DIRECT_GROUPS = 32;
inline bool sort_groups_scanned(uint32_t ngroups) { return ngroups > SORT_DIRECT_GROUPS; }
int sort_groups_scan(bh_ctx* ctx, uint32_t* sums, uint32_t ngroups, uint32_t tables, uint32_t* totals);
int radix_argsort(bh_ctx* ctx, const uint32_t* keys, const uint32_t* vals, uint32_t n, uint32_t bits,
                  uint32_t* out_keys, uint32_t* out_vals);
int radix_argsort_dev(bh_ctx* ctx, const uint32_t* keys, const uint32_t* vals, uint32_t n_max, const uint32_t* n_dev, const uint32_t* gate,
                      const uint32_t* out_base, uint32_t bits, uint32_t* out_keys, uint32_t* out_vals, uint32_t alloc_n = 0);
bool tile_sort_supported(uint32_t bits, uint32_t n);
int tile_sort_offsets(bh_ctx* ctx, const uint32_t* keys, const uint32_t* vals, uint32_t n, uint32_t bits, uint32_t num_tiles,
                      uint32_t* out_keys, uint32_t* out_vals, uint32_t* tile_offsets, uint32_t alloc_n = 0);
bool depth_sort_supported(uint32_t n);
int depth_sort_scan(bh_ctx* ctx, const uint32_t* keys, const uint32_t* minmax, const uint32_t* counts, uint32_t n, uint32_t* out_keys,
                    uint32_t* out_vals, uint32_t* cum, const uint32_t* rb_set = nullptr, uint32_t* rb_host = nullptr, hipEvent_t rb_done = nullptr,
                    uint32_t rb_tag = 0, uint32_t* rb_dev = nullptr, uint32_t* spl = nullptr, bool* spl_written = nullptr);
int prefix_sum(bh_ctx* ctx, const uint32_t* in, const uint32_t* gather, uint32_t n, uint32_t* out, bool exclusive, const uint32_t* gate = nullptr);
int launch_tile_offsets(bh_ctx* ctx, const uint32_t* tile_ids_sorted, uint32_t num_isect, uint32_t num_tiles,
                        uint32_t* tile_offsets, bool pre_zeroed = false);
int launch_tile_offsets_dev(bh_ctx* ctx, const uint32_t* tile_ids_sorted, uint32_t n_max, const uint32_t* n_dev, const uint32_t* gate,
                            const uint32_t* base, uint32_t num_tiles, uint32_t* tile_offsets);

int launch_rasterize(bh_ctx* ctx, const ViewUniforms& u, const float bg[3], bool bwd_info, bool smooth,
                     const uint32_t* isect_gids, uint32_t* tile_offsets, const float* projected,
                     const uint32_t* global_from_compact, float* out_img, uint32_t* out_packed, float* visible,
                     uint32_t* lpt, float class_width, int phase = 0, const RasterSlice* slice = nullptr);
int launch_rasterize_backward(bh_ctx* ctx, const ViewUniforms& u, const float bg[3], bool smooth,
                              const uint32_t* isect_gids, const uint32_t* tile_offsets, const float* projected,
                              const float* out_img, const float* v_output, float* v_combined, const uint32_t* lpt,
                              const uint32_t* tile_offsets_far = nullptr, bool want_refine = true, const BwdJobs* jobs = nullptr,
                              uint32_t accum_rows = 0u);
int launch_image_loss_forward(bh_ctx* ctx, const float* pred, const uint32_t* gt, uint32_t channels, uint32_t h,
                              uint32_t w, const BhLossConfig& cfg, float* loss_map);
int launch_image_loss_backward(bh_ctx* ctx, const float* pred, const uint32_t* gt, const float* dl_dmap,
                               float dl_const, uint32_t channels, uint32_t h, uint32_t w, const BhLossConfig& cfg,
                               float* dl_dpred);
int launch_image_loss_fused(bh_ctx* ctx, const float* img_hwc4, const uint32_t* gt, uint32_t h, uint32_t w, const BhLossConfig& cfg,
                            bool alpha_match, float dl_rgb, float dl_alpha, float* loss_out, float* v_output, float* loss_host = nullptr,
                            uint32_t* started_host = nullptr, uint32_t started_tag = 0);
int launch_image_loss_fused_window(bh_ctx* ctx, const float* img_hwc4, const uint32_t* gt, uint32_t h, uint32_t w, const BhLossConfig& cfg,
                                   bool alpha_match, float dl_rgb, float dl_alpha, uint32_t tile_y0, uint32_t tile_y1, float* loss_out,
                                   float* v_output, float* loss_host = nullptr, uint32_t* started_host = nullptr, uint32_t started_tag = 0);
int launch_adam(bh_ctx* ctx, float* param, const float* grad, float* m1, float* m2, uint64_t rows, uint32_t row_len,
                const float* col_scale, float lr, uint32_t t, bool reduce_m2, float beta1, float beta2, float eps, float gscale = 1.0f);
struct NoiseArgs { uint64_t seed; uint32_t step; float scale, clamp_abs; };
struct UpdateCall {
    const float *g_transforms, *g_sh, *g_opac;
    const float *refine_weight, *visible, *screen_radius;
    float gscale;
    bool vis_clamp;
    float tab_t[10];
    float lr_sh, sh_rest_scale, lr_opac;
    uint32_t t;
    float beta1, beta2, eps;
    const NoiseArgs* noise;
    bool masked_rows;
};
int launch_train_update(bh_ctx* ctx, const BhTrainState* st, const UpdateCall& c);
int launch_gather_stats(bh_ctx* ctx, float* refine_weight_norm, float* vis_weight, float* max_screen_size,
                        const float* refine_weight, const float* visible, const float* screen_radius, uint64_t n);
int launch_mean_noise(bh_ctx* ctx, float* transforms, const float* raw_opac, const float* visible,
                      const float* samples, uint64_t n, float noise_scale, float clamp_abs, uint64_t seed = 0, uint32_t step = 0);
int launch_normal_samples(bh_ctx* ctx, float* out, uint64_t n, uint64_t seed, uint32_t step);

int launch_fold_min_scale(bh_ctx* ctx, const float* transforms, const float* raw_opac, const float* min_scale, uint32_t n,
                          float* out_transforms, float* out_raw_opac);
int launch_fold_min_scale_backward(bh_ctx* ctx, const float* transforms, const float* raw_opac, const float* min_scale, uint32_t n,
                                   float* v_transforms, float* v_raw_opac);
int launch_compute_min_scale(bh_ctx* ctx, const float* transforms, uint32_t n, const float* view_cams, uint32_t k, float factor, float* out);

int comm_allreduce(bh_ctx* ctx, float* buf, uint64_t count, bool max_op);
int comm_exchange_strip_halos(bh_ctx* ctx, float* img, uint32_t h, uint32_t w, uint32_t row_begin_px, uint32_t row_end_px);

int launch_union_index(bh_ctx* ctx, const float* visible_sum, uint32_t n, uint32_t* block_scratch , uint32_t* count_dev,
                       uint32_t* idx);
int launch_exchange_rows(bh_ctx* ctx, bool gather, const uint32_t* idx, uint32_t count, uint32_t c3, float* g_tr, float* g_sh, float* g_op,
                         float* g_ref , float* compact);

}
```

brush_amd/csrc/depth_sort.hip:

```cpp
#include <cstddef>

#include "context.h"
#include "sort_groups.h"

namespace bh {

constexpr int DS_WG = 256;
constexpr int DS_WAVES = DS_WG / 64;
#define BH_DS_KPT 8
constexpr int DS_KPT = BH_DS_KPT;
constexpr int DS_TILE = DS_WG * DS_KPT;
constexpr int DS_RADIX = 256;
constexpr uint32_t CULLED_KEY = 0xFFFFFFFFu;

struct DepthSplit {
    uint32_t kmin, kmax;
    uint32_t scale;
    bool any_visible;
    const uint32_t* spl;
};
constexpr uint32_t SPL_WORDS = 258;
static_assert(SPL_WORDS <= DSORT_SPL_STRIDE, "context.h reserves the table");
constexpr uint32_t SPL_MIN_KEYS = 16384;
constexpr uint32_t SPL_SAMPLE_STRIDE = 64;
constexpr uint32_t SPL_SAMPLE_MIN_N = 1u << 17;
constexpr uint32_t SPL_SAMPLE_MIN_KEYS = 1024;
BH_DEV DepthSplit make_split(uint32_t kmax, uint32_t nmin) {
    DepthSplit sp;
    sp.any_visible = nmin != 0u;
    sp.kmin = ~nmin;
    sp.kmax = kmax;
    const uint32_t range = sp.any_visible ? kmax - sp.kmin : 0u;
    sp.scale = (uint32_t)min((unsigned long long)0xFFFFFFFFull, (255ull << 32) / ((unsigned long long)range + 1ull));
    if ((((unsigned long long)range * sp.scale) >> 32) > 254ull) sp.scale -= 1u;
    sp.spl = nullptr;
    return sp;
}

BH_DEV DepthSplit depth_split(const uint32_t* __restrict__ minmax, uint32_t* s_red , const uint32_t* __restrict__ spl_in ,
                              uint32_t* s_spl ) {
    const int tid = threadIdx.x, lane = tid & 63, wave = tid >> 6;
    uint32_t a = 0, b = 0;
    if (tid < (int)COUNTER_SLOTS) {
        a = minmax[2 * tid];
        b = minmax[2 * tid + 1];
    }
    if (spl_in != nullptr) {
        s_spl[tid] = spl_in[tid];
        if (tid < (int)SPL_WORDS - DS_WG) s_spl[DS_WG + tid] = spl_in[DS_WG + tid];
    }
#pragma unroll
    for (int off = 32; off > 0; off >>= 1) {
        a = max(a, (uint32_t)__shfl_xor((int)a, off));
        b = max(b, (uint32_t)__shfl_xor((int)b, off));
    }
    if (lane == 0) { s_red[wave] = a; s_red[DS_WAVES + wave] = b; }
    __syncthreads();
    uint32_t kmax = 0, nmin = 0;
#pragma unroll
    for (int w = 0; w < DS_WAVES; ++w) { kmax = max(kmax, s_red[w]); nmin = max(nmin, s_red[DS_WAVES + w]); }
    __syncthreads();
    DepthSplit sp = make_split(kmax, nmin);
    if (spl_in != nullptr && sp.any_visible && s_spl[255] != 0u) {
        const uint32_t tmin = s_spl[256], tmax = s_spl[257], tol = (tmax - tmin) >> 4;
        const uint32_t dmin = sp.kmin > tmin ? sp.kmin - tmin : tmin - sp.kmin, dmax = sp.kmax > tmax ? sp.kmax - tmax : tmax - sp.kmax;
        if (dmin <= tol && dmax <= tol) sp.spl = s_spl;
    }
    return sp;
}
BH_DEV uint32_t depth_digit(uint32_t key, const DepthSplit& sp) {
    if (key == CULLED_KEY) return 255u;
    if (sp.spl != nullptr) {
        uint32_t d = 0;
#pragma unroll
        for (uint32_t step = 128u; step != 0u; step >>= 1) d += sp.spl[d + step - 1u] <= key ? step : 0u;
        return d;
    }
    return min(254u, (uint32_t)(((unsigned long long)(key - sp.kmin) * sp.scale) >> 32));
}

BH_DEV unsigned long long ds_match(uint32_t d) {
    uint32_t lo = 0xFFFFFFFFu, hi = 0xFFFFFFFFu;
#pragma unroll
    for (int b = 0; b < 8; ++b) {
        const uint32_t bit = (d >> b) & 1u;
        const unsigned long long bal = __ballot(bit);
        const uint32_t flip = bit - 1u;
        lo &= (uint32_t)bal ^ flip;
        hi &= (uint32_t)(bal >> 32) ^ flip;
    }
    return ((unsigned long long)hi << 32) | lo;
}

BH_DEV void counter_sums_to_host(const uint32_t* __restrict__ set, uint32_t* __restrict__ host_sums, int lane, uint32_t tag, uint32_t* __restrict__ dev_sums) {
    const unsigned long long* c64 = reinterpret_cast<const unsigned long long*>(set);
    unsigned long long tot[COUNTER_K1_U64];
#pragma unroll
    for (uint32_t c = 0; c < COUNTER_K1_U64; ++c) tot[c] = 0ull;
    for (uint32_t k = (uint32_t)lane; k < COUNTER_SLOTS; k += 64u) {
#pragma unroll
        for (uint32_t c = 0; c < COUNTER_K1_U64; ++c) tot[c] += c64[COUNTER_K1_U64 * k + c];
    }
#pragma unroll
    for (int off = 32; off > 0; off >>= 1) {
#pragma unroll
        for (uint32_t c = 0; c < COUNTER_K1_U64; ++c) tot[c] += __shfl_down(tot[c], off);
    }
    if (lane == 0) {
        if (dev_sums) {
#pragma unroll
            for (uint32_t c = 0; c < COUNTER_K1_U64; ++c) dev_sums[c] = tot[c] > 0xFFFFFFFFull ? 0xFFFFFFFFu : (uint32_t)tot[c];
        }
        volatile unsigned long long* h64 = reinterpret_cast<volatile unsigned long long*>(host_sums);
#pragma unroll
        for (uint32_t c = 0; c < COUNTER_K1_U64; ++c) h64[c] = tot[c];
        if (tag) {
            __threadfence_system();
            reinterpret_cast<volatile uint32_t*>(host_sums)[HOST_SUM_WORDS - 1u] = tag;
        }
    }
}

__global__ __launch_bounds__(DS_WG) void dsort_hist_kernel(const uint32_t* __restrict__ keys, const uint32_t* __restrict__ counts,
                                                          uint32_t n, uint32_t nblocks, const uint32_t* __restrict__ minmax,
                                                          uint32_t* __restrict__ hist , SortGroups grp, uint32_t ngroups,
                                                          const uint32_t* __restrict__ rb_set, uint32_t* __restrict__ rb_host, uint32_t rb_tag, uint32_t* __restrict__ rb_dev,
                                                          const uint32_t* __restrict__ spl_in, uint8_t* __restrict__ digits ) {
    __shared__ uint32_t s_hist[DS_WAVES][DS_RADIX];
    __shared__ uint32_t s_csum[DS_WAVES][DS_RADIX];
    __shared__ uint32_t s_red[2 * DS_WAVES];
    __shared__ uint32_t s_spl[SPL_WORDS];
    const int tid = threadIdx.x, wave = tid >> 6;
    sort_groups_clear(grp.stale, grp.stale_words);
    if (blockIdx.x == nblocks) {
        if (wave == 0) counter_sums_to_host(rb_set, rb_host, tid, rb_tag, rb_dev);
        return;
    }
    for (int i = tid; i < DS_WAVES * DS_RADIX; i += DS_WG) { (&s_hist[0][0])[i] = 0; (&s_csum[0][0])[i] = 0; }
    const DepthSplit sp = depth_split(minmax, s_red, spl_in, s_spl);
    const uint32_t base = blockIdx.x * DS_TILE;
    auto count_one = [&](uint32_t key, uint32_t cnt) {
        const uint32_t d = depth_digit(key, sp);
        if (d != 255u) {
            atomicAdd(&s_hist[wave][d], 1u);
            atomicAdd(&s_csum[wave][d], cnt);
        }
        return d;
    };
    if (base + (uint32_t)DS_TILE <= n && ((reinterpret_cast<uintptr_t>(keys) | reinterpret_cast<uintptr_t>(counts)) & 15u) == 0) {
        const uint4* k4 = reinterpret_cast<const uint4*>(keys + base);
        const uint4* c4 = reinterpret_cast<const uint4*>(counts + base);
        uint4 kv[DS_KPT / 4], cv[DS_KPT / 4];
#pragma unroll
        for (int k = 0; k < DS_KPT / 4; ++k) { kv[k] = k4[k * DS_WG + tid]; cv[k] = c4[k * DS_WG + tid]; }
        uint32_t* d4 = reinterpret_cast<uint32_t*>(digits + base);
#pragma unroll
        for (int k = 0; k < DS_KPT / 4; ++k) {
            const uint32_t d0 = count_one(kv[k].x, cv[k].x);
            const uint32_t d1 = count_one(kv[k].y, cv[k].y);
            const uint32_t d2 = count_one(kv[k].z, cv[k].z);
            const uint32_t d3 = count_one(kv[k].w, cv[k].w);
            d4[k * DS_WG + tid] = d0 | (d1 << 8) | (d2 << 16) | (d3 << 24);
        }
    } else {
#pragma unroll
        for (int k = 0; k < DS_KPT; ++k) {
            const uint32_t idx = base + k * DS_WG + tid;
            if (idx < n) digits[idx] = (uint8_t)count_one(keys[idx], counts[idx]);
        }
    }
    __syncthreads();
    uint32_t t = 0, c = 0;
#pragma unroll
    for (int w = 0; w < DS_WAVES; ++w) { t += s_hist[w][tid]; c += s_csum[w][tid]; }
    hist[(size_t)blockIdx.x * DS_RADIX + tid] = t;
    const size_t gw = (size_t)(blockIdx.x / SORT_GROUP_BLOCKS) * DS_RADIX + tid;
    if (t != 0u) atomicAdd(&grp.sums[gw], t);
    if (c != 0u) atomicAdd(&grp.sums[(size_t)ngroups * DS_RADIX + gw], c);
}

template <int WG>
struct ChunkLds {
    uint32_t cnt[WG / 64][DS_RADIX];
    uint32_t dbase[DS_RADIX];
    uint32_t gofs[DS_RADIX];
    uint32_t wsum[WG / 64];
    uint32_t keys[DS_TILE];
    uint32_t vals[DS_TILE];
    uint8_t digs[DS_TILE];
};
template <int WG, class DigitFn>
BH_DEV void scatter_chunk(ChunkLds<WG>& L, uint32_t* __restrict__ s_base , const uint32_t* __restrict__ src_k,
                          const uint32_t* __restrict__ src_v , uint32_t first, uint32_t count, uint32_t* __restrict__ dst_k,
                          uint32_t* __restrict__ dst_v, DigitFn digit, uint32_t* __restrict__ alt_k = nullptr, uint32_t* __restrict__ alt_v = nullptr,
                          const uint8_t* __restrict__ pre_dig = nullptr ) {
    constexpr int WAVES = WG / 64, KPT = DS_TILE / WG;
    const int tid = threadIdx.x, lane = tid & 63, wave = tid >> 6;
    for (int i = tid; i < WAVES * DS_RADIX; i += WG) (&L.cnt[0][0])[i] = 0;
// ... 129 lines not shown

#define BH_BK_WG 1024
constexpr int BK_WG = BH_BK_WG;
constexpr int BK_WAVES = BK_WG / 64;
constexpr int BK_KPT = DS_TILE / BK_WG;
constexpr int FAST_CAP = BK_WG <= 512 ? 8192 : 7168;
constexpr int FAST_NDIG = 512;
constexpr size_t FAST_LDS_WORDS = 4 * FAST_CAP + (BK_WAVES + 1) * FAST_NDIG;
static_assert(FAST_LDS_WORDS * 4 >= sizeof(ChunkLds<BK_WG>), "the dynamic LDS block holds either path's arrays");
static_assert(offsetof(ChunkLds<BK_WG>, vals) == offsetof(ChunkLds<BK_WG>, keys) + sizeof(uint32_t) * DS_TILE, "scan staging spans keys[] and vals[]");

BH_DEV uint32_t bk_excl_scan(uint32_t v, uint32_t& total, uint32_t* s_w) {
    const int lane = threadIdx.x & 63, wave = threadIdx.x >> 6;
    uint32_t incl = v;
#pragma unroll
    for (int off = 1; off < 64; off <<= 1) {
        const uint32_t x = __shfl_up(incl, off);
        if (lane >= off) incl += x;
    }
    if (lane == 63) s_w[wave] = incl;
    __syncthreads();
    uint32_t wofs = 0, tot = 0;
#pragma unroll
    for (int w = 0; w < BK_WAVES; ++w) { wofs += (w < wave) ? s_w[w] : 0u; tot += s_w[w]; }
    total = tot;
    __syncthreads();
    return incl - v + wofs;
}

BH_DEV void bk_scan_counts(const uint32_t* vals, uint32_t size, const uint32_t* __restrict__ counts, uint32_t carry, uint32_t* __restrict__ cum_out,
                           uint32_t* stage, uint32_t* s_w) {
    const int tid = threadIdx.x;
    const uint32_t nch = (size + DS_TILE - 1) / DS_TILE;
    for (uint32_t c = 0; c < nch; ++c) {
        const uint32_t first = c * DS_TILE;
        const uint32_t count = size - first < (uint32_t)DS_TILE ? size - first : (uint32_t)DS_TILE;
#pragma unroll
        for (int k = 0; k < BK_KPT; ++k) {
            const uint32_t e = k * BK_WG + tid;
            stage[e + e / BK_KPT] = e < count ? counts[vals[first + e]] : 0u;
        }
        __syncthreads();
        uint32_t v[BK_KPT], tsum = 0;
#pragma unroll
        for (int k = 0; k < BK_KPT; ++k) { v[k] = stage[tid * (BK_KPT + 1) + k]; tsum += v[k]; }
        uint32_t total;
        uint32_t run = carry + bk_excl_scan(tsum, total, s_w);
#pragma unroll
        for (int k = 0; k < BK_KPT; ++k) { run += v[k]; stage[tid * (BK_KPT + 1) + k] = run; }
        __syncthreads();
#pragma unroll
        for (int k = 0; k < BK_KPT; ++k) {
            const uint32_t e = k * BK_WG + tid;
            if (e < count) cum_out[first + e] = stage[e + e / BK_KPT];
        }
        carry += total;
        __syncthreads();
    }
}

BH_DEV uint32_t bk_key_bits(uint32_t& lo, uint32_t hi, uint32_t* s_w) {
    const int lane = threadIdx.x & 63, wave = threadIdx.x >> 6;
#pragma unroll
    for (int off = 32; off > 0; off >>= 1) {
        lo = min(lo, (uint32_t)__shfl_xor((int)lo, off));
        hi = max(hi, (uint32_t)__shfl_xor((int)hi, off));
    }
    if (lane == 0) { s_w[wave] = lo; s_w[BK_WAVES + wave] = hi; }
    __syncthreads();
#pragma unroll
    for (int w = 0; w < BK_WAVES; ++w) { lo = min(lo, s_w[w]); hi = max(hi, s_w[BK_WAVES + w]); }
    __syncthreads();
    return hi > lo ? 32u - (uint32_t)__clz(hi - lo) : 0u;
}

BH_DEV void bk_write_splitters(const uint32_t* sorted , uint32_t start, uint32_t size, uint32_t nv,
                               uint32_t* __restrict__ spl_out, uint32_t spl_min_keys) {
    const uint32_t j = threadIdx.x;
    if (spl_out == nullptr || nv < spl_min_keys || j >= 254u) return;
    const uint32_t r = (uint32_t)(((unsigned long long)(j + 1u) * nv) / 255ull);
    if (r >= start && r - start < size) spl_out[j] = sorted[r - start];
}

__global__ __launch_bounds__(BK_WG) void dsort_bucket_kernel(uint32_t* __restrict__ a_keys, uint32_t* __restrict__ a_vals ,
                                                            uint32_t* __restrict__ out_keys, uint32_t* __restrict__ out_vals,
                                                            const uint32_t* __restrict__ minmax, const uint32_t* __restrict__ digit_totals,
                                                            const uint32_t* __restrict__ counts, uint32_t* __restrict__ cum ,
                                                            uint32_t* __restrict__ spl_out , uint32_t spl_min_keys) {
    extern __shared__ __attribute__((aligned(16))) uint32_t s_dyn[];
    __shared__ uint32_t s_base[DS_RADIX];
    __shared__ uint32_t s_hist[DS_RADIX];
    __shared__ uint32_t s_red[2 * BK_WAVES];
    const int tid = threadIdx.x, lane = tid & 63, wave = tid >> 6;
    const uint32_t b = blockIdx.x;
    uint32_t start, size, tiles_before, nv;
    {
        const uint32_t gt = tid < DS_RADIX ? digit_totals[tid] : 0u;
        const uint32_t ct = tid < 255 ? digit_totals[DS_RADIX + tid] : 0u;
        uint32_t tot;
        const uint32_t gex = bk_excl_scan(gt, nv, s_red);
        const uint32_t cex = bk_excl_scan(ct, tot, s_red);
        if (tid < DS_RADIX) { s_base[tid] = gex; s_hist[tid] = cex; }
        __syncthreads();
        start = s_base[b];
        size = s_base[b + 1u] - start;
        tiles_before = s_hist[b];
        __syncthreads();
    }
    if (b == 0u && spl_out != nullptr) {
        uint32_t x = 0, y = 0;
        if (tid < (int)COUNTER_SLOTS) { x = minmax[2 * tid]; y = minmax[2 * tid + 1]; }
#pragma unroll
        for (int off = 32; off > 0; off >>= 1) {
            x = max(x, (uint32_t)__shfl_xor((int)x, off));
            y = max(y, (uint32_t)__shfl_xor((int)y, off));
        }
        if (lane == 0) { s_red[wave] = x; s_red[BK_WAVES + wave] = y; }
        __syncthreads();
        if (tid == 0) {
            uint32_t kmax = 0, nmin = 0;
            for (int w = 0; w < BK_WAVES; ++w) { kmax = max(kmax, s_red[w]); nmin = max(nmin, s_red[BK_WAVES + w]); }
            spl_out[254] = 0xFFFFFFFFu;
            spl_out[255] = nv >= spl_min_keys ? 1u : 0u;
            spl_out[256] = ~nmin;
            spl_out[257] = kmax;
        }
        __syncthreads();
    }
    if (size == 0u) return;
    if (size <= (uint32_t)FAST_CAP) {
        uint32_t* fcnt = s_dyn + 4 * FAST_CAP;
        uint32_t* fdb = fcnt + BK_WAVES * FAST_NDIG;
        uint32_t lo = 0xFFFFFFFFu, hi = 0u;
        for (uint32_t i = tid; i < size; i += BK_WG) {
            const uint32_t k = a_keys[start + i];
            s_dyn[i] = k;
            s_dyn[FAST_CAP + i] = a_vals[start + i];
            lo = min(lo, k);
            hi = max(hi, k);
        }
        const uint32_t bits = bk_key_bits(lo, hi, s_red);
        const uint32_t passes = (bits + 8u) / 9u;
        const uint32_t base_w = passes ? bits / passes : 0u, wide = passes ? bits % passes : 0u;
        const unsigned long long lt_mask = (1ull << lane) - 1ull;
        const uint32_t steps = (size + (uint32_t)BK_WG - 1u) / (uint32_t)BK_WG;
        const uint32_t wave_first = wave * steps * 64u;
        uint32_t cur = 0;
        for (uint32_t p = 0; p < passes; ++p) {
            const uint32_t width = base_w + (p < wide ? 1u : 0u);
            const uint32_t pshift = p * base_w + (p < wide ? p : wide);
            const uint32_t mask = (1u << width) - 1u;
            const uint32_t* sk = s_dyn + cur * (2 * FAST_CAP); const uint32_t* sv = sk + FAST_CAP;
            uint32_t* dk = s_dyn + (cur ^ 1u) * (2 * FAST_CAP); uint32_t* dv = dk + FAST_CAP;
            for (int i = tid; i < BK_WAVES * FAST_NDIG; i += BK_WG) fcnt[i] = 0;
            __syncthreads();
            for (uint32_t r = 0; r < steps; ++r) {
                const uint32_t e = wave_first + r * 64u + lane;
                if (e < size) atomicAdd(&fcnt[wave * FAST_NDIG + (((sk[e] - lo) >> pshift) & mask)], 1u);
            }
            __syncthreads();
            {
                uint32_t run = 0;
                if (tid < FAST_NDIG) {
#pragma unroll
                    for (int w = 0; w < BK_WAVES; ++w) {
                        const uint32_t c = fcnt[w * FAST_NDIG + tid];
                        fcnt[w * FAST_NDIG + tid] = run;
                        run += c;
                    }
                }
                uint32_t tot;
                const uint32_t ex = bk_excl_scan(run, tot, s_red);
                if (tid < FAST_NDIG) fdb[tid] = ex;
            }
            __syncthreads();
            for (uint32_t r = 0; r < steps; ++r) {
                const uint32_t e = wave_first + r * 64u + lane;
                const bool valid = e < size;
                const uint32_t key = valid ? sk[e] : 0u, val = valid ? sv[e] : 0u;
                const uint32_t d = valid ? ((key - lo) >> pshift) & mask : mask;
                uint32_t plo = 0xFFFFFFFFu, phi = 0xFFFFFFFFu;
                for (uint32_t bb = 0; bb < width; ++bb) {
                    const uint32_t bit = (d >> bb) & 1u;
                    const unsigned long long bal = __ballot(bit);
                    const uint32_t flip = bit - 1u;
                    plo &= (uint32_t)bal ^ flip;
                    phi &= (uint32_t)(bal >> 32) ^ flip;
                }
                const unsigned long long peers = ((unsigned long long)phi << 32) | plo;
                const uint32_t cursor = fcnt[wave * FAST_NDIG + d];
                const uint32_t pos = fdb[d] + cursor + (uint32_t)__popcll(peers & lt_mask);
                if ((peers & lt_mask) == 0ull) fcnt[wave * FAST_NDIG + d] = cursor + (uint32_t)__popcll(peers);
                if (valid) { dk[pos] = key; dv[pos] = val; }
            }
            __syncthreads();
            cur ^= 1u;
        }
        const uint32_t* fk = s_dyn + cur * (2 * FAST_CAP); const uint32_t* fv = fk + FAST_CAP;
        uint32_t* spare = s_dyn + (cur ^ 1u) * (2 * FAST_CAP);
        bk_write_splitters(fk, start, size, nv, spl_out, spl_min_keys);
        for (uint32_t i = tid; i < size; i += BK_WG) {
            const uint32_t v = fv[i];
            out_keys[start + i] = fk[i];
            out_vals[start + i] = v;
            if (cum != nullptr) { const uint32_t e = i; spare[e + e / BK_KPT] = counts[v]; }
        }
        if (cum == nullptr) return;
        __syncthreads();
        {
            uint32_t carry = tiles_before;
            const uint32_t nch = (size + DS_TILE - 1) / DS_TILE;
            for (uint32_t c = 0; c < nch; ++c) {
                const uint32_t first = c * DS_TILE;
                uint32_t v[BK_KPT], tsum = 0;
#pragma unroll
                for (int k = 0; k < BK_KPT; ++k) {
                    const uint32_t e = first + tid * BK_KPT + k;
                    v[k] = e < size ? spare[e + e / BK_KPT] : 0u;
                    tsum += v[k];
                }
                uint32_t total;
                uint32_t run = carry + bk_excl_scan(tsum, total, s_red);
#pragma unroll
                for (int k = 0; k < BK_KPT; ++k) {
                    const uint32_t e = first + tid * BK_KPT + k;
                    run += v[k];
                    if (e < size) spare[e + e / BK_KPT] = run;
                }
                carry += total;
            }
            __syncthreads();
            for (uint32_t i = tid; i < size; i += BK_WG) cum[start + i] = spare[i + i / BK_KPT];
        }
        return;
    }
    ChunkLds<BK_WG>& L = *reinterpret_cast<ChunkLds<BK_WG>*>(s_dyn);
    uint32_t lo = 0xFFFFFFFFu, hi = 0u;
    for (uint32_t i = tid; i < size; i += BK_WG) {
        const uint32_t k = a_keys[start + i];
        lo = min(lo, k);
        hi = max(hi, k);
    }
    const uint32_t bits = bk_key_bits(lo, hi, s_red);
    const uint32_t passes = bits <= 8u ? 1u : (bits <= 24u ? 3u : 5u);
    const uint32_t base_w = bits / passes, wide = bits % passes;
    uint32_t* src_k = a_keys; uint32_t* src_v = a_vals;
    uint32_t* dst_k = out_keys; uint32_t* dst_v = out_vals;
    const uint32_t nchunks = (size + DS_TILE - 1) / DS_TILE;
    for (uint32_t p = 0; p < passes; ++p) {
        const uint32_t width = base_w + (p < wide ? 1u : 0u);
        const uint32_t pshift = p * base_w + (p < wide ? p : wide);
        const uint32_t mask = (1u << width) - 1u;
        auto digit = [=](uint32_t k) { return ((k - lo) >> pshift) & mask; };
        if (tid < DS_RADIX) s_hist[tid] = 0;
        __syncthreads();
        if (width != 0u) {
            for (uint32_t i = tid; i < size; i += BK_WG) atomicAdd(&s_hist[digit(src_k[start + i])], 1u);
        } else if (tid == 0) {
            s_hist[0] = size;
        }
        __syncthreads();
        {
            uint32_t tot;
            const uint32_t ex = bk_excl_scan(tid < DS_RADIX ? s_hist[tid] : 0u, tot, s_red);
            if (tid < DS_RADIX) s_base[tid] = start + ex;
        }
        __syncthreads();
        for (uint32_t c = 0; c < nchunks; ++c) {
            const uint32_t first = start + c * DS_TILE;
            const uint32_t count = size - c * DS_TILE < (uint32_t)DS_TILE ? size - c * DS_TILE : (uint32_t)DS_TILE;
            scatter_chunk<BK_WG>(L, s_base, src_k, src_v, first, count, dst_k, dst_v, digit);
        }
        __threadfence_block();
        __syncthreads();
        uint32_t* tk = src_k; src_k = dst_k; dst_k = tk;
        uint32_t* tv = src_v; src_v = dst_v; dst_v = tv;
    }
    bk_write_splitters(out_keys + start, start, size, nv, spl_out, spl_min_keys);
    if (cum != nullptr) bk_scan_counts(out_vals + start, size, counts, tiles_before, cum + start, &L.keys[0], s_red);
}

#define BH_DSORT_MAX_N (16u << 20)
constexpr uint32_t DSORT_MAX_N = BH_DSORT_MAX_N;
constexpr uint32_t DS_MAX_BLOCKS = 4096;
bool depth_sort_supported(uint32_t n) { return n > 0 && n <= DSORT_MAX_N && (n + DS_TILE - 1) / DS_TILE <= DS_MAX_BLOCKS; }

__global__ __launch_bounds__(256) void dsort_sample_kernel(const uint32_t* __restrict__ keys, uint32_t stride, uint32_t m, uint32_t* __restrict__ out) {
    const uint32_t i = blockIdx.x * 256u + threadIdx.x;
    if (i < m) out[i] = keys[(size_t)i * stride];
}

static int dsort_launches(bh_ctx* ctx, const uint32_t* keys, const uint32_t* minmax, const uint32_t* counts, uint32_t n, uint32_t* out_keys, uint32_t* out_vals,
                          uint32_t* cum, const uint32_t* rb_set, uint32_t* rb_host, hipEvent_t rb_done, uint32_t rb_tag, uint32_t* rb_dev, uint32_t* totals,
                          uint32_t* a_keys, uint32_t* a_vals, const uint32_t* spl_in, uint32_t* spl_out, uint32_t spl_min_keys) {
    const uint32_t nblocks = (n + DS_TILE - 1) / DS_TILE;
    uint32_t* hist = totals + 2 * DS_RADIX;
    uint8_t* digits = reinterpret_cast<uint8_t*>(hist + (size_t)DS_RADIX * nblocks);
    const uint32_t ngroups = sort_group_count(nblocks);
    SortGroups grp;
    BH_TRY(sort_groups_next(ctx, (size_t)2 * ngroups * DS_RADIX, &grp));
    hipLaunchKernelGGL(dsort_hist_kernel, dim3(nblocks + (rb_set ? 1u : 0u)), dim3(DS_WG), 0, ctx->stream, keys, counts, n, nblocks, minmax, hist, grp, ngroups,
                       rb_set, rb_host, rb_tag, rb_dev, spl_in, digits);
    BH_LAUNCH_CHECK(ctx, "dsort_hist_kernel");
    if (rb_set && !rb_tag) BH_HIP(ctx, hipEventRecord(rb_done, ctx->stream));
    const uint32_t scanned = sort_groups_scanned(ngroups) ? 1u : 0u;
    if (scanned) BH_TRY(sort_groups_scan(ctx, grp.sums, ngroups, 2u, totals));
    hipLaunchKernelGGL(dsort_split_kernel, dim3(nblocks), dim3(DS_WG), 0, ctx->stream, keys, n, nblocks, hist, grp.sums, ngroups, scanned, totals, a_keys, a_vals, out_keys, out_vals,
                       digits);
    BH_LAUNCH_CHECK(ctx, "dsort_split_kernel");
    if (!ctx->dsort_lds_raised) {
        BH_HIP(ctx, hipFuncSetAttribute((const void*)dsort_bucket_kernel, hipFuncAttributeMaxDynamicSharedMemorySize, (int)(FAST_LDS_WORDS * 4)));
        ctx->dsort_lds_raised = true;
    }
    hipLaunchKernelGGL(dsort_bucket_kernel, dim3(DS_RADIX - 1), dim3(BK_WG), FAST_LDS_WORDS * 4, ctx->stream, a_keys, a_vals, out_keys, out_vals, minmax, totals, counts, cum, spl_out,
                       spl_min_keys);
    BH_LAUNCH_CHECK(ctx, "dsort_bucket_kernel");
    return 0;
}

int depth_sort_scan(bh_ctx* ctx, const uint32_t* keys, const uint32_t* minmax, const uint32_t* counts, uint32_t n, uint32_t* out_keys,
                    uint32_t* out_vals, uint32_t* cum, const uint32_t* rb_set, uint32_t* rb_host, hipEvent_t rb_done, uint32_t rb_tag, uint32_t* rb_dev, uint32_t* spl,
                    bool* spl_written) {
    if (n == 0) return 0;
    const uint32_t nblocks = (n + DS_TILE - 1) / DS_TILE;
    if (!ctx->knob_dsort_splitters) spl = nullptr;
    else if (spl == nullptr) {
        if (ctx->dsort_spl == nullptr) {
            if (hipMalloc((void**)&ctx->dsort_spl, DSORT_SPL_STRIDE * 4) != hipSuccess) { (void)hipGetLastError(); ctx->dsort_spl = nullptr; return BH_ERR_OOM; }
            BH_HIP(ctx, hipMemsetAsync(ctx->dsort_spl, 0, DSORT_SPL_STRIDE * 4, ctx->stream));
            ctx->dsort_spl_written = false;
        }
        spl = ctx->dsort_spl;
        spl_written = &ctx->dsort_spl_written;
    }
    uint32_t* totals = (uint32_t*)ensure(ctx, SLOT_SORT_HIST, ((size_t)DS_RADIX * nblocks + 2 * DS_RADIX) * 4 + (size_t)nblocks * DS_TILE);
    uint32_t* a_keys = (uint32_t*)ensure(ctx, SLOT_SORT_KEYS_A, (size_t)n * 4);
    uint32_t* a_vals = (uint32_t*)ensure(ctx, SLOT_SORT_VALS_A, (size_t)n * 4);
    if (!totals || !a_keys || !a_vals) return BH_ERR_OOM;
    if (spl && spl_written && !*spl_written && n >= SPL_SAMPLE_MIN_N) {
        const uint32_t m = n / SPL_SAMPLE_STRIDE;
        uint32_t* sample = (uint32_t*)ensure(ctx, SLOT_SORT_KEYS_B, (size_t)m * 4);
        if (!sample) return BH_ERR_OOM;
        hipLaunchKernelGGL(dsort_sample_kernel, dim3((m + 255u) / 256u), dim3(256), 0, ctx->stream, keys, SPL_SAMPLE_STRIDE, m, sample);
        BH_LAUNCH_CHECK(ctx, "dsort_sample_kernel");
        BH_TRY(dsort_launches(ctx, sample, minmax, sample, m, out_keys, out_vals, nullptr, nullptr, nullptr, nullptr, 0u, nullptr, totals, a_keys, a_vals, nullptr, spl,
                              SPL_SAMPLE_MIN_KEYS));
    }
    BH_TRY(dsort_launches(ctx, keys, minmax, counts, n, out_keys, out_vals, cum, rb_set, rb_host, rb_done, rb_tag, rb_dev, totals, a_keys, a_vals, spl, spl, SPL_MIN_KEYS));
    if (spl && spl_written) *spl_written = true;
    return 0;
}

}
```

brush_amd/csrc/lists.hip:

```cpp
#include <algorithm>
#include <cmath>
#include <cstring>

#include "context.h"

namespace bh {

static uint64_t view_key(const bh_ctx* ctx, uint32_t view_id, const BhCamera& c) {
    if (view_id != 0u || ctx->knob_no_view_hash) return (uint64_t)view_id;
    uint64_t h = 0x9E3779B97F4A7C15ull;
    auto mix = [&](uint32_t w) {
        h += (uint64_t)w + 0x9E3779B97F4A7C15ull;
        uint64_t z = h;
        z = (z ^ (z >> 30)) * 0xBF58476D1CE4E5B9ull;
        z = (z ^ (z >> 27)) * 0x94D049BB133111EBull;
        h = z ^ (z >> 31);
    };
    auto bits = [](float f) { uint32_t u; std::memcpy(&u, &f, 4); return u; };
    for (int i = 0; i < 12; ++i) mix(bits(c.vm[i]));
    mix(bits(c.fx)); mix(bits(c.fy)); mix(bits(c.cx)); mix(bits(c.cy));
    mix(c.img_w); mix(c.img_h); mix(c.tile_row_begin); mix(c.tile_row_end); mix(c.model);
    if (c.model != BH_CAMERA_PINHOLE) for (int i = 0; i < 8; ++i) mix(bits(c.dist[i]));
    return h | (1ull << 63);
}
// ... 9 lines not shown
        else {
            (void)hipStreamSynchronize(ctx->stream);
            (void)hipFree(v->second.zcut);
        }
        ctx->views.erase(v);
    };
    if (it != ctx->views.end() && (it->second.tile_bw != tile_bw || it->second.tile_bh != tile_bh)) {
        forget(it, false);
        it = ctx->views.end();
    }
    if (it == ctx->views.end()) {
        if (casual) {
            bool seen = false;
            for (uint64_t k : ctx->seen_keys) seen = seen || k == key;
            if (!seen) {
                ctx->seen_keys[ctx->seen_pos++ % SEEN_KEYS] = key;
                return nullptr;
            }
            while (ctx->casual_views >= CASUAL_VIEW_STATES) {
                auto old = ctx->views.end();
                for (auto k = ctx->views.begin(); k != ctx->views.end(); ++k)
                    if (k->second.casual && (old == ctx->views.end() || k->second.last_used < old->second.last_used)) old = k;
                if (old == ctx->views.end()) { ctx->casual_views = 0; break; }
                forget(old, recycled == nullptr && old->second.tile_bw == tile_bw && old->second.tile_bh == tile_bh);
            }
        }
        const size_t max_views = std::min(MAX_VIEW_STATES, std::max<size_t>(8, VIEW_TABLE_BYTES / ((2 * words + VIEW_SPL_WORDS) * 4)));
        while (ctx->views.size() >= max_views) {
            auto old = ctx->views.begin();
            for (auto k = ctx->views.begin(); k != ctx->views.end(); ++k)
                if (k->second.last_used < old->second.last_used) old = k;
            forget(old, recycled == nullptr && old->second.tile_bw == tile_bw && old->second.tile_bh == tile_bh);
        }
        ViewState vs;
        vs.tile_bw = tile_bw;
        vs.tile_bh = tile_bh;
        vs.casual = casual;
        vs.zcut = recycled;
        if (!vs.zcut && hipMalloc((void**)&vs.zcut, (2 * words + VIEW_SPL_WORDS) * 4) != hipSuccess) {
            (void)hipGetLastError();
            return nullptr;
        }
        if (hipMemsetD32Async(reinterpret_cast<hipDeviceptr_t>(vs.zcut), (int)ZCUT_ALL, words, ctx->stream) != hipSuccess ||
            hipMemsetD32Async(reinterpret_cast<hipDeviceptr_t>(vs.zcut + words), 0, words + VIEW_SPL_WORDS, ctx->stream) != hipSuccess) {
            (void)hipGetLastError();
            (void)hipFree(vs.zcut);
            return nullptr;
        }
        vs.gap = (uint32_t)ctx->views.size() + 1u;
        vs.last_used = ++ctx->view_clock;
        if (casual) ctx->casual_views++;
        return &ctx->views.emplace(key, vs).first->second;
    }
    if (it->second.casual && !casual) {
        it->second.casual = false;
        if (ctx->casual_views) ctx->casual_views--;
    }
    if (touch) {
        const uint64_t now = ++ctx->view_clock;
        it->second.gap = (uint32_t)std::min<uint64_t>(now - it->second.last_used, 1u << 20);
        it->second.last_used = now;
    }
    return &it->second;
}

ViewState* frame_view(bh_ctx* ctx, const ForwardRequest& req, uint32_t tile_bw, uint32_t tile_bh, bool casual) {
    const uint64_t vkey = view_key(ctx, req.view_id, req.cam);
    return view_state(ctx, vkey, tile_bw, tile_bh, req.allow_cut, casual && (vkey >> 63) != 0ull);
}

bool cut_this_frame(const bh_ctx* ctx, ViewState* vs, bool allow_cut) {
    if (!allow_cut) return false;
    if (vs->seeded && vs->exact_frames == 0u && vs->last_pairs >= ctx->cut_min_pairs) {
        if (vs->complete_frames == 0u) return true;
        vs->complete_frames--;
    } else if (vs->exact_frames) {
        vs->exact_frames--;
    }
    return false;
}

uint32_t* view_table(const ViewState* vs) { return vs ? vs->zcut : nullptr; }

uint32_t* view_splitters(ViewState* vs, bool cut, bool** written) {
    *written = vs ? &vs->spl_written[cut ? 1 : 0] : nullptr;
    return vs ? vs->zcut + 2 * (size_t)vs->tile_bw * vs->tile_bh + (cut ? DSORT_SPL_STRIDE : 0u) : nullptr;
}

uint32_t cut_margin_pct(const bh_ctx* ctx, const ViewState* vs) {
    if (ctx->knob_fixed_margin) return ctx->knob_cut_margin_pct;
    const float gap = vs && vs->gap > 2u ? (float)vs->gap : 2.0f;
    const float m = (float)ctx->knob_cut_margin_pct * ctx->margin_scale * std::pow(gap * 0.5f, ctx->ctrl_gap_exp);
    return m < 6400.0f ? (m > 10.0f ? (uint32_t)m : 10u) : 6400u;
}

uint32_t list_budget(bh_ctx* ctx, ViewState* cut_view, uint32_t near_total, uint32_t ni) {
    uint32_t budget = ni;
    const float share = ctx->slice_fraction;
    if (share > 0.0f) {
        if (share < 1.0f) {
            const double b = (double)share * (double)ni;
            const uint32_t floor_b = ni < 1024u ? ni : 1024u;
            budget = b < (double)floor_b ? floor_b : (uint32_t)b;
            if (budget > ni) budget = ni;
        }
        ctx->last_slice_share = (float)((double)budget / (double)ni);
    } else if (cut_view && near_total < ni) {
        budget = near_total;
        const float cut_share = (float)((double)near_total / (double)ni);
        ctx->last_slice_share = cut_share;
        if (ctx->auto_exact_share > 0.0f && cut_share > ctx->auto_exact_share) cut_view->complete_frames = AUTO_EXACT_FRAMES;
    } else {
        if (cut_view && ctx->auto_exact_share > 0.0f) cut_view->complete_frames = AUTO_EXACT_FRAMES;
        ctx->last_slice_share = 1.0f;
    }
    return budget;
}

void view_rendered(ViewState* vs, uint32_t ni) {
    vs->seeded = true;
    vs->last_pairs = ni;
}

static void view_outcome(bh_ctx* ctx, ViewState* vs, bool missed, bool shared_table) {
    if (!ctx->knob_fixed_margin) {
        const float s = ctx->margin_scale * (missed ? ctx->ctrl_up : ctx->ctrl_down);
        ctx->margin_scale = s < ctx->ctrl_floor ? ctx->ctrl_floor : (s > 16.0f ? 16.0f : s);
    }
    if (!vs) return;
    vs->penalty = ((vs->penalty << 1) | (missed ? 1u : 0u)) & 0xFFu;
    if (__builtin_popcount(vs->penalty) >= (shared_table ? 3 : 6)) {
        vs->exact_frames = shared_table ? 32u : 8u;
        vs->penalty = 0u;
    }
}

int enqueue_far_slice(bh_ctx* ctx, const FarJob& j) {
    const Frame& f = j.frame;
    const uint32_t* gate = f.slice_info + 2;
    const uint32_t far_max = f.ni;
    {
        ProfScope ps(ctx, "MapGaussiansToIntersect");
        BH_TRY(launch_map_gaussians_far(ctx, f.nv, f.u, f.proj_by_gid, f.gfc, f.projected, f.cum, f.budget, f.done_bits, gate, f.far_counts, f.far_block_totals,
                                        f.far_group_totals, f.slice_info, f.tile_ids, f.isect_gids));
    }
    {
        ProfScope ps(ctx, "TileSort");
        BH_TRY(radix_argsort_dev(ctx, f.tile_ids, f.isect_gids, far_max, f.slice_info + 3, gate, f.slice_info + 1, f.tile_bits, f.tile_ids_sorted,
                                 f.isect_gids_sorted));
    }
    {
        ProfScope ps(ctx, "GetTileOffsets");
        BH_TRY(launch_tile_offsets_dev(ctx, f.tile_ids_sorted, far_max, f.slice_info + 3, gate, f.slice_info + 1, f.num_tiles, f.tile_offsets_far));
    }
    {
        ProfScope ps(ctx, "Rasterize");
        BH_TRY(launch_rasterize(ctx, f.u, f.bg, f.bwd_info, f.smooth, f.isect_gids_sorted, f.tile_offsets_far, f.projected, f.gfc, f.out_f32, f.out_u8, f.visible,
                                f.lpt, f.class_width, 2, &f.rs));
    }
    ctx->far_launches++;
    return 0;
}

int finish_far_slice(bh_ctx* ctx, bool* launched) {
    if (launched) *launched = false;
    if (!ctx->far_job.pending) return 0;
    ctx->far_job.pending = false;
    if (!ctx->far_job.gate_event_recorded && ctx->gate_signal_queued) {
// ... 40 lines not shown
```

brush_amd/csrc/project.hip:

```cpp
#include "context.h"
#include "device_camera.h"
#include "device_f64_sum.h"
#include "device_sh.h"

namespace bh {

constexpr int PROJ_WG = 256;
constexpr int PROJ_WAVES = PROJ_WG / 64;
constexpr uint32_t ORDER_BINS = 1024;

struct WalkLds {
    uint32_t count[64];
    float mx[64], my[64], c00[64], c01[64], c11[64], pt[64];
    uint32_t magic[64];
    uint32_t box[64];
    uint32_t boxw[64];
    uint32_t start[64];
    uint32_t lane_of[64];
    uint32_t zkey[64];
    uint32_t near[64];
    uint8_t flags[64];
};

BH_DEV uint32_t walk_magic(uint32_t bw, uint32_t nb) {
    if (bw < 2u || (unsigned long long)nb * bw >= (1ull << 32)) return 0u;
    return 0xFFFFFFFFu / bw + 1u;
}
BH_DEV uint32_t walk_row(uint32_t i, uint32_t bw, uint32_t magic) {
    if (magic) return __umulhi(i, magic);
    if (bw < 2u) return i;
    uint32_t row = (uint32_t)(((float)i + 0.5f) / (float)bw);
    if (row * bw > i) --row;
    else if ((row + 1u) * bw <= i) ++row;
    return row;
}

BH_DEV uint32_t wave_inclusive_scan_u32(uint32_t v, int lane) {
#pragma unroll
    for (int off = 1; off < 64; off <<= 1) {
        const uint32_t t = __shfl_up(v, off);
        if (lane >= off) v += t;
    }
    return v;
}

struct KeepAllTiles { static constexpr bool EAGER = false; BH_DEV bool operator()(const WalkLds&, uint32_t, uint32_t, uint32_t) const { return true; } };
struct KeepLiveTiles {
    static constexpr bool EAGER = false;
    const uint32_t* done_bits;
    uint32_t tile_bw;
    BH_DEV bool operator()(const WalkLds&, uint32_t, uint32_t tx, uint32_t ty) const {
        const uint32_t t = tx + ty * tile_bw;
        return ((done_bits[t >> 5] >> (t & 31u)) & 1u) == 0u;
    }
};
struct KeepNearOfCut {
    const uint32_t* zcut;
    uint32_t tile_bw;
    static constexpr bool EAGER = true;
    BH_DEV uint32_t fetch(uint32_t tx, uint32_t ty) const { return zcut[tx + ty * tile_bw]; }
    BH_DEV bool decide(const WalkLds& w, uint32_t r, uint32_t cut) const { return zcut_near(w.zkey[r], cut); }
    BH_DEV bool operator()(const WalkLds& w, uint32_t r, uint32_t tx, uint32_t ty) const { return decide(w, r, fetch(tx, ty)); }
};

struct NoPrefetch { BH_DEV uint32_t operator()(uint32_t, uint32_t) const { return 0u; } };
template <class OnHit, class Keep = KeepAllTiles, class Pre = NoPrefetch>
BH_DEV uint32_t flat_tile_walk(WalkLds& w, int lane, uint32_t nb, float mx, float my, Sym2 conic, float pt, TileBbox bb,
                               OnHit on_hit, Keep keep = Keep{}, uint32_t zkey = 0u, Pre pre = Pre{}) {
    const uint32_t incl = wave_inclusive_scan_u32(nb, lane);
    const uint32_t start = incl - nb;
    const bool nz = nb > 0u;
    const unsigned long long nzmask = __ballot(nz);
    const unsigned long long below = (1ull << lane) - 1ull;
    const uint32_t rank = (uint32_t)__popcll(nzmask & below);
    const uint32_t bb_w = bb.max_x - bb.min_x;
    if (nz) {
        w.count[rank] = 0;
        w.near[rank] = 0;
        w.zkey[rank] = zkey;
        w.mx[rank] = mx; w.my[rank] = my;
        w.c00[rank] = conic.c00; w.c01[rank] = conic.c01; w.c11[rank] = conic.c11;
        w.pt[rank] = pt;
        w.magic[rank] = walk_magic(bb_w, nb);
// ... 40 lines not shown
    const uint32_t start = incl - nb;
    const bool nz = nb > 0u;
    const unsigned long long nzmask = __ballot(nz);
    const unsigned long long below = (1ull << lane) - 1ull;
    const uint32_t rank = (uint32_t)__popcll(nzmask & below);
    const uint32_t bb_w = bb.max_x - bb.min_x;
    if (nz) {
        w.zkey[rank] = zkey;
        w.mx[rank] = mx; w.my[rank] = my;
        w.c00[rank] = conic.c00; w.c01[rank] = conic.c01; w.c11[rank] = conic.c11;
        w.pt[rank] = pt;
        w.magic[rank] = walk_magic(bb_w, nb);
        w.box[rank] = bb.min_x | (bb.min_y << 16);
        w.boxw[rank] = bb_w;
        w.start[rank] = start;
        w.lane_of[rank] = (uint32_t)lane;
    }
    __builtin_amdgcn_fence(__ATOMIC_SEQ_CST, "wavefront");
    uint8_t* flags = w.flags;
    const uint32_t tot = __shfl(incl, 63);
    const unsigned long long le = below | (1ull << lane);
    uint32_t before = 0;
    uint32_t emitted = 0;
    for (uint32_t base = 0; base < tot; base += 64) {
        flags[lane] = 0;
        const uint32_t rel = start - base;
        if (nz && rel < 64u) flags[rel] = 1;
        asm volatile("" ::: "memory");
        const unsigned long long marks = __ballot(flags[lane] != 0);
        asm volatile("" ::: "memory");
        const uint32_t c = base + (uint32_t)lane;
        bool hit = false;
        uint32_t tile = 0, owner = 0;
        if (c < tot) {
            const uint32_t r = before + (uint32_t)__popcll(marks & le) - 1u;
            const uint32_t i = c - w.start[r];
            const uint32_t box = w.box[r];
            const uint32_t bw = w.boxw[r];
            const uint32_t row = walk_row(i, bw, w.magic[r]);
            const uint32_t tx = (box & 0xFFFFu) + (i - __umul24(row, bw));
            const uint32_t ty = (box >> 16) + row;
            if constexpr (Keep::EAGER) {
                const uint32_t cut = keep.fetch(tx, ty);
                uint32_t contributes = will_primitive_contribute(tx, ty, w.mx[r], w.my[r], Sym2{w.c00[r], w.c01[r], w.c11[r]}, w.pt[r]) ? 1u : 0u;
                asm volatile("" : "+v"(contributes));
                hit = contributes != 0u && keep.decide(w, r, cut);
            } else {
                hit = keep(w, r, tx, ty) && will_primitive_contribute(tx, ty, w.mx[r], w.my[r], Sym2{w.c00[r], w.c01[r], w.c11[r]}, w.pt[r]);
            }
            tile = tx + ty * tile_bw;
            owner = cg0 + w.lane_of[r];
        }
        const unsigned long long hits = __ballot(hit);
        if (hit) {
            const uint32_t local = emitted + (uint32_t)__popcll(hits & below);
            if (local < wave_total) {
                tile_ids[wave_base + local] = tile;
                isect_gids[wave_base + local] = owner;
            }
        }
        emitted += (uint32_t)__popcll(hits);
        before += (uint32_t)__popcll(marks);
    }
    for (uint32_t k = emitted + (uint32_t)lane; k < wave_total; k += 64u) {
        tile_ids[wave_base + k] = 0xFFFFFFFFu;
        isect_gids[wave_base + k] = 0u;
    }
    return emitted;
}

template <bool MIP, bool PINHOLE, int DEG>
__global__ __launch_bounds__(PROJ_WG) void project_forward_kernel(
    ViewUniforms u, uint32_t n, const float* __restrict__ transforms, const float* __restrict__ coeffs,
    const float* __restrict__ raw_opacities, uint32_t* __restrict__ depth_keys, uint32_t* __restrict__ isect_counts,
    float* __restrict__ max_radius, float* __restrict__ projected_by_gid, unsigned long long* __restrict__ counters, ForwardPrep prep,
    uint32_t* __restrict__ zcut, uint32_t* __restrict__ near_counts) {
    __shared__ WalkLds s_walk[PROJ_WAVES];
    __shared__ uint32_t s_vis[PROJ_WAVES];
    __shared__ uint32_t s_hit[PROJ_WAVES];
    __shared__ uint32_t s_near[PROJ_WAVES];
    __shared__ uint32_t s_listed[PROJ_WAVES];
    __shared__ uint32_t s_kmax[PROJ_WAVES];
    __shared__ uint32_t s_nmax[PROJ_WAVES];
    const uint32_t gid = blockIdx.x * PROJ_WG + threadIdx.x;
    if (prep.order_out && blockIdx.x < 8u) {
        __shared__ uint32_t s_bins[ORDER_BINS];
        const uint32_t per = band_slots(prep.order_tiles);
        __shared__ uint32_t s_band_work, s_band_cnt, s_band_tail, s_band_max;
        for (uint32_t i = threadIdx.x; i < ORDER_BINS; i += PROJ_WG) s_bins[i] = 0u;
        if (threadIdx.x == 0) s_band_work = s_band_cnt = s_band_tail = s_band_max = 0u;
        __syncthreads();
        uint32_t my_work = 0u, my_cnt = 0u, my_max = 0u;
        for (uint32_t i = threadIdx.x; i < per; i += PROJ_WG) {
            const uint32_t lt = band_tile(blockIdx.x, i, per, prep.band_mode);
            if (lt >= prep.order_tiles) continue;
            const uint32_t wk = prep.order_work[prep.order_tile_begin + lt];
            atomicAdd(&s_bins[ORDER_BINS - 1u - (wk < ORDER_BINS ? wk : ORDER_BINS - 1u)], 1u);
            my_work += wk < ORDER_BINS ? wk : ORDER_BINS - 1u;
            my_max = max(my_max, wk < ORDER_BINS ? wk : ORDER_BINS - 1u);
            my_cnt++;
        }
        if (prep.split_out && my_work) atomicAdd(&s_band_work, my_work);
        if (my_cnt) atomicAdd(&s_band_cnt, my_cnt);
        if (prep.split_out && my_max) atomicMax(&s_band_max, my_max);
        __syncthreads();
        const uint32_t cnt = s_band_cnt;
        {
            __shared__ uint32_t s_part[PROJ_WG];
            const uint32_t b0 = threadIdx.x * (ORDER_BINS / PROJ_WG);
            uint32_t loc[ORDER_BINS / PROJ_WG], sum = 0;
#pragma unroll
            for (uint32_t k = 0; k < ORDER_BINS / PROJ_WG; ++k) { loc[k] = sum; sum += s_bins[b0 + k]; }
            s_part[threadIdx.x] = sum;
            __syncthreads();
            if (threadIdx.x == 0) {
                uint32_t run = 0;
                for (uint32_t k = 0; k < (uint32_t)PROJ_WG; ++k) { const uint32_t t = s_part[k]; s_part[k] = run; run += t; }
            }
            __syncthreads();
#pragma unroll
            for (uint32_t k = 0; k < ORDER_BINS / PROJ_WG; ++k) s_bins[b0 + k] = s_part[threadIdx.x] + loc[k];
        }
        __syncthreads();
        if (prep.split_out) {
            if (threadIdx.x == 0) {
                const float mean = cnt ? (float)s_band_work / (float)cnt : 0.0f;
                const float thr_f = fmaxf(fmaxf((float)prep.split_min, prep.split_factor * mean), prep.split_of_max * (float)s_band_max);
                uint32_t h = 0u;
                if (prep.order_mode == 1u && thr_f < (float)(ORDER_BINS - 1u)) {
                    const uint32_t thr = (uint32_t)ceilf(thr_f);
                    h = s_bins[ORDER_BINS - thr];
                }
                prep.split_out[blockIdx.x] = h < SPLIT_MAX ? h : SPLIT_MAX;
            }
            uint32_t* scr = prep.split_out + 8u + blockIdx.x * (SPLIT_MAX * 4u);
            for (uint32_t i = threadIdx.x; i < SPLIT_MAX * 4u; i += PROJ_WG) scr[i] = 0u;
        }
        __syncthreads();
        for (uint32_t i = threadIdx.x; i < per; i += PROJ_WG) {
            const uint32_t lt = band_tile(blockIdx.x, i, per, prep.band_mode);
            if (lt < prep.order_tiles) {
                const uint32_t wk = prep.order_work[prep.order_tile_begin + lt];
                const uint32_t rank = atomicAdd(&s_bins[ORDER_BINS - 1u - (wk < ORDER_BINS ? wk : ORDER_BINS - 1u)], 1u);
                prep.order_out[blockIdx.x * per + rank] = lt;
            } else {
                prep.order_out[blockIdx.x * per + cnt + atomicAdd(&s_band_tail, 1u)] = 0xFFFFFFFFu;
            }
        }
        __syncthreads();
    }
    if (gid < prep.visible_words) prep.visible[gid] = 0u;
    if (gid < prep.tile_words) prep.tile_table[gid] = 0u;
    if (gid < prep.slice_words) prep.slice_table[gid] = 0u;
    if (gid < COUNTER_SET_U64 && prep.next_counters) prep.next_counters[gid] = 0ull;
    for (size_t i = gid; i < prep.span_f4; i += (size_t)gridDim.x * PROJ_WG) prep.span[i] = make_float4(0.0f, 0.0f, 0.0f, 0.0f);
    const int lane = threadIdx.x & 63, wave = threadIdx.x >> 6;
    uint32_t key = 0xFFFFFFFFu;
    float radius = 0.0f;
    bool visible = false;
    float mx = 0.0f, my = 0.0f, pt = 0.0f, opac = 0.0f;
    Sym2 conic = Sym2{0.0f, 0.0f, 0.0f};
    TileBbox bb = TileBbox{0, 0, 0, 0};
    Vec3A mean = v3(0.0f, 0.0f, 0.0f);
    const uint32_t gsafe = gid < n ? gid : (n ? n - 1u : 0u);
    float tr[10];
    {
        const float* trp = transforms + (size_t)gsafe * 10;
#pragma unroll
        for (int k = 0; k < 10; ++k) tr[k] = trp[k];
    }
    float raw_opac = raw_opacities[gsafe];
    constexpr int C_ALL = (DEG + 1) * (DEG + 1);
    float sh_dc[3];
#pragma unroll
    for (int k = 0; k < 3; ++k) sh_dc[k] = coeffs[(size_t)gsafe * C_ALL * 3 + k];
    asm volatile("" : "+v"(tr[0]), "+v"(tr[1]), "+v"(tr[2]), "+v"(tr[3]), "+v"(tr[4]), "+v"(tr[5]), "+v"(tr[6]), "+v"(tr[7]), "+v"(tr[8]), "+v"(tr[9]),
                      "+v"(raw_opac), "+v"(sh_dc[0]), "+v"(sh_dc[1]), "+v"(sh_dc[2]));
    if (gid < n) {
        do {
            mean = v3(tr[0], tr[1], tr[2]);
            const Vec3A mean_c = world_to_cam(mean, u);
            if (!(finite3(mean_c) && mean_c.z <= 1.0e10f)) break;
            if (!in_front_of_camera<PINHOLE>(mean_c, u)) break;
            const Vec3A scl = v3(bh_expf(tr[7]), bh_expf(tr[8]), bh_expf(tr[9]));
            if (!finite3(scl)) break;
            const Quat qu = Quat{tr[3], tr[4], tr[5], tr[6]};
            const float qn = qdot(qu, qu);
            if (!(qn >= 1.0e-6f && is_finite_f32(qn))) break;
            if (!is_finite_f32(raw_opac)) break;
            const Quat q = qnormalize(qu);
            const Sym2 raw_cov = calc_cov2d<PINHOLE>(scl, q, mean_c, u);
            float filter_comp;
            const Sym2 cov = compensate_cov2d<MIP>(raw_cov, filter_comp);
            opac = sigmoid(raw_opac) * filter_comp;
            if (!sym2_finite(cov)) break;
            project_point<PINHOLE>(mean_c, u, mx, my);
            if (!(opac >= 1.0f / 255.0f)) break;
            pt = bh_logf(opac * 255.0f);
            conic = sym2_inverse(cov);
            float ex, ey;
            compute_bbox_extent(conic, pt, ex, ey);
            if (!(ex >= 0.0f && ey >= 0.0f)) break;
            const float wf = (float)u.img_w, hf = (float)u.img_h;
            const bool on_screen = mx + ex > 0.0f && mx - ex < wf && my + ey > 0.0f && my - ey < hf;
            if (!on_screen) break;
            bb = get_tile_bbox(mx, my, ex, ey, u.tile_bw, u.tile_y0, u.tile_y1);
            const bool whole = u.tile_y0 == 0u && u.tile_y1 == u.tile_bh;
            if (!whole && (bb.max_y <= bb.min_y || bb.max_x <= bb.min_x)) break;
            radius = __builtin_fmaxf(ex / wf, ey / hf);
            key = f2u(mean_c.z);
            visible = true;
        } while (false);
    }
    const uint32_t nb = visible ? (bb.max_y - bb.min_y) * (bb.max_x - bb.min_x) : 0u;
    WalkLds& w = s_walk[wave];
    const uint32_t tile_bw = u.tile_bw;
    struct CutOfTile {
        const uint32_t* zcut;
        uint32_t tile_bw;
        BH_DEV uint32_t operator()(uint32_t tx, uint32_t ty) const { return zcut ? zcut[tx + ty * tile_bw] : 0u; }
    };
    const uint32_t wrank = flat_tile_walk(w, lane, nb, mx, my, conic, pt, bb, [&](uint32_t r, uint32_t tx, uint32_t ty, uint32_t cut) {
        atomicAdd(&w.count[r], 1u);
        if (zcut) {
            if (zcut_near(w.zkey[r], cut)) atomicAdd(&w.near[r], 1u);
            else if ((cut & 1u) == 0u) zcut[tx + ty * tile_bw] = cut | 1u;
        }
    }, KeepAllTiles{}, key, CutOfTile{zcut, tile_bw});
    const uint32_t tiles_hit = nb ? w.count[wrank] : 0u;
    const uint32_t near_hit = (nb && zcut) ? w.near[wrank] : 0u;
    const bool listed = visible && (!zcut || near_hit > 0u || prep.list_all_visible);
    if (listed) {
        const Vec3A v = normalize(sub(mean, camera_pos(u)));
        constexpr int C = (DEG + 1) * (DEG + 1);
        const Vec3A raw = sh_coeffs_to_color_dc<DEG>(coeffs + (size_t)gid * C * 3, v, sh_dc);
        const float cr = raw.x + 0.5f, cgc = raw.y + 0.5f, cb = raw.z + 0.5f;
        float* o = projected_by_gid + (size_t)gid * 9;
        o[0] = mx;
        o[1] = my;
        o[2] = conic.c00;
        o[3] = conic.c01;
        o[4] = conic.c11;
        o[5] = opac;
        o[6] = clampf(is_finite_f32(cr) ? cr : 0.0f, -100.0f, 100.0f);
        o[7] = clampf(is_finite_f32(cgc) ? cgc : 0.0f, -100.0f, 100.0f);
        o[8] = clampf(is_finite_f32(cb) ? cb : 0.0f, -100.0f, 100.0f);
    }
    if (gid < n) {
        depth_keys[gid] = listed ? key : 0xFFFFFFFFu;
        isect_counts[gid] = tiles_hit;
        max_radius[gid] = radius;
        if (zcut) near_counts[gid] = near_hit;
    }
    const unsigned long long ball = __ballot(visible);
    const unsigned long long lball = __ballot(listed);
    uint32_t wave_hits = tiles_hit;
#pragma unroll
    for (int off = 32; off > 0; off >>= 1) wave_hits += __shfl_down(wave_hits, off);
    uint32_t wave_near = 0;
    if (zcut) {
        wave_near = near_hit;
#pragma unroll
        for (int off = 32; off > 0; off >>= 1) wave_near += __shfl_down(wave_near, off);
    }
    uint32_t kmax = listed ? key : 0u, nmax = listed ? ~key : 0u;
#pragma unroll
    for (int off = 32; off > 0; off >>= 1) {
        kmax = max(kmax, (uint32_t)__shfl_xor((int)kmax, off));
        nmax = max(nmax, (uint32_t)__shfl_xor((int)nmax, off));
    }
    if (lane == 0) {
        s_vis[wave] = (uint32_t)__popcll(ball);
        s_hit[wave] = wave_hits;
        s_near[wave] = wave_near;
        s_listed[wave] = (uint32_t)__popcll(lball);
        s_kmax[wave] = kmax;
        s_nmax[wave] = nmax;
    }
    __syncthreads();
    if (threadIdx.x == 0) {
        uint32_t v = 0, h = 0, nh = 0, ls = 0, km = 0, nm = 0;
#pragma unroll
        for (int k = 0; k < PROJ_WAVES; ++k) { v += s_vis[k]; h += s_hit[k]; nh += s_near[k]; ls += s_listed[k]; km = max(km, s_kmax[k]); nm = max(nm, s_nmax[k]); }
        const uint32_t sl = blockIdx.x & (COUNTER_SLOTS - 1u);
        unsigned long long* slot = counters + COUNTER_K1_U64 * sl;
        if (v) atomicAdd(&slot[0], (unsigned long long)v);
        if (h) atomicAdd(&slot[1], (unsigned long long)h);
        if (nh) atomicAdd(&slot[2], (unsigned long long)nh);
        if (ls && zcut) atomicAdd(&slot[3], (unsigned long long)ls);
        if (ls) {
            uint32_t* mm = reinterpret_cast<uint32_t*>(counters) + COUNTER_MINMAX_WORD + 2u * sl;
            atomicMax(&mm[0], km);
            atomicMax(&mm[1], nm);
        }
    }
}

template <bool MIP, bool PINHOLE>
static int launch_pf_deg(bh_ctx* ctx, const ViewUniforms& u, uint32_t n, uint32_t deg, const float* t, const float* sh, const float* ro,
                         uint32_t* keys, uint32_t* counts, float* radius, float* proj, unsigned long long* c64, const ForwardPrep& prep,
                         uint32_t* zcut, uint32_t* near_counts) {
    const dim3 grid((n + PROJ_WG - 1) / PROJ_WG), block(PROJ_WG);
    switch (deg) {
        case 0: hipLaunchKernelGGL((project_forward_kernel<MIP, PINHOLE, 0>), grid, block, 0, ctx->stream, u, n, t, sh, ro, keys, counts, radius, proj, c64, prep, zcut, near_counts); break;
        case 1: hipLaunchKernelGGL((project_forward_kernel<MIP, PINHOLE, 1>), grid, block, 0, ctx->stream, u, n, t, sh, ro, keys, counts, radius, proj, c64, prep, zcut, near_counts); break;
        case 2: hipLaunchKernelGGL((project_forward_kernel<MIP, PINHOLE, 2>), grid, block, 0, ctx->stream, u, n, t, sh, ro, keys, counts, radius, proj, c64, prep, zcut, near_counts); break;
        case 3: hipLaunchKernelGGL((project_forward_kernel<MIP, PINHOLE, 3>), grid, block, 0, ctx->stream, u, n, t, sh, ro, keys, counts, radius, proj, c64, prep, zcut, near_counts); break;
        case 4: hipLaunchKernelGGL((project_forward_kernel<MIP, PINHOLE, 4>), grid, block, 0, ctx->stream, u, n, t, sh, ro, keys, counts, radius, proj, c64, prep, zcut, near_counts); break;
        default: return set_error(ctx, BH_ERR_INVALID_ARG, "sh_degree must be 0..4");
    }
    BH_LAUNCH_CHECK(ctx, "project_forward_kernel");
    return 0;
}

int launch_project_forward(bh_ctx* ctx, const ViewUniforms& u, uint32_t n, bool mip, uint32_t sh_degree, const float* transforms,
                           const float* sh, const float* raw_opac, uint32_t* depth_keys, uint32_t* isect_counts, float* max_radius,
                           float* projected_by_gid, uint32_t* counters, const ForwardPrep& want, uint32_t* zcut, uint32_t* near_counts) {
    if (zcut && !near_counts) return set_error(ctx, BH_ERR_INVALID_ARG, "project_forward: a depth-cut table needs the near-count output");
    ForwardPrep prep = want;
    const size_t covered = (size_t)((n + PROJ_WG - 1) / PROJ_WG) * PROJ_WG;
    if (prep.visible && prep.visible_words > covered) {
        BH_HIP(ctx, hipMemsetAsync(prep.visible, 0, (size_t)prep.visible_words * 4, ctx->stream));
        prep.visible_words = 0;
    }
    if (prep.next_counters && COUNTER_SET_U64 > covered) {
        BH_HIP(ctx, hipMemsetAsync(prep.next_counters, 0, COUNTER_SET_BYTES, ctx->stream));
        prep.next_counters = nullptr;
    }
    if (prep.tile_table && prep.tile_words > covered) {
        BH_HIP(ctx, hipMemsetAsync(prep.tile_table, 0, (size_t)prep.tile_words * 4, ctx->stream));
        prep.tile_words = 0;
    }
    if (prep.slice_table && prep.slice_words > covered) {
        BH_HIP(ctx, hipMemsetAsync(prep.slice_table, 0, (size_t)prep.slice_words * 4, ctx->stream));
        prep.slice_words = 0;
    }
    if (n == 0) {
        if (prep.next_counters) BH_HIP(ctx, hipMemsetAsync(prep.next_counters, 0, COUNTER_SET_BYTES, ctx->stream));
        if (prep.span && prep.span_f4) BH_HIP(ctx, hipMemsetAsync(prep.span, 0, (size_t)prep.span_f4 * 16, ctx->stream));
        return 0;
    }
    auto* c64 = reinterpret_cast<unsigned long long*>(counters);
    const bool pinhole = u.model == CAM_PINHOLE;
    if (mip && pinhole) return launch_pf_deg<true, true>(ctx, u, n, sh_degree, transforms, sh, raw_opac, depth_keys, isect_counts, max_radius, projected_by_gid, c64, prep, zcut, near_counts);
    if (pinhole) return launch_pf_deg<false, true>(ctx, u, n, sh_degree, transforms, sh, raw_opac, depth_keys, isect_counts, max_radius, projected_by_gid, c64, prep, zcut, near_counts);
    if (mip) return launch_pf_deg<true, false>(ctx, u, n, sh_degree, transforms, sh, raw_opac, depth_keys, isect_counts, max_radius, projected_by_gid, c64, prep, zcut, near_counts);
    return launch_pf_deg<false, false>(ctx, u, n, sh_degree, transforms, sh, raw_opac, depth_keys, isect_counts, max_radius, projected_by_gid, c64, prep, zcut, near_counts);
}

__global__ __launch_bounds__(PROJ_WG) void project_visible_kernel(uint32_t nv, const float* __restrict__ projected_by_gid,
                                                                 const uint32_t* __restrict__ global_from_compact_gid,
                                                                 float* __restrict__ projected) {
    const uint32_t e = blockIdx.x * PROJ_WG + threadIdx.x;
    if (e >= nv * 9u) return;
    const uint32_t cg = e / 9u, j = e - cg * 9u;
    projected[e] = projected_by_gid[(size_t)global_from_compact_gid[cg] * 9 + j];
}

int launch_project_visible(bh_ctx* ctx, uint32_t nv, const float* projected_by_gid, const uint32_t* gid, float* projected) {
    if (nv == 0) return 0;
    const uint64_t total = (uint64_t)nv * 9u;
    if (total > 0xFFFFFFFFull) return set_error(ctx, BH_ERR_UNSUPPORTED, "more than 2^32/9 visible splats");
    hipLaunchKernelGGL(project_visible_kernel, dim3((unsigned)((total + PROJ_WG - 1) / PROJ_WG)), dim3(PROJ_WG), 0, ctx->stream, nv,
                       projected_by_gid, gid, projected);
    BH_LAUNCH_CHECK(ctx, "project_visible_kernel");
    return 0;
}

template <bool FAR, int SPW>
__global__ __launch_bounds__(PROJ_WG) void map_gaussians_kernel(
    uint32_t nv, uint32_t tile_bw, uint32_t tile_bh, uint32_t tile_y0, uint32_t tile_y1, const float* __restrict__ projected_by_gid,
    const uint32_t* __restrict__ global_from_compact_gid, float* __restrict__ projected,
    const uint32_t* __restrict__ cum_tiles_hit, uint32_t* __restrict__ tile_id_from_isect,
    uint32_t* __restrict__ compact_gid_from_isect, float4* __restrict__ zero_span, uint32_t zero_f4, uint32_t budget,
    uint32_t* __restrict__ slice_info, const uint32_t* __restrict__ far_counts, const uint32_t* __restrict__ far_block_totals,
    const uint32_t* __restrict__ far_group_totals, const uint32_t* __restrict__ done_bits, const uint32_t* __restrict__ gate,
    const uint32_t* __restrict__ zcut, const uint32_t* __restrict__ depth_keys_sorted, const uint32_t* __restrict__ nv_dev, uint32_t pair_cap) {
    __shared__ WalkLds s_walk[PROJ_WAVES];
    __shared__ uint32_t s_far[2 * PROJ_WAVES];
    if (FAR && *gate == 0u) return;
    if (nv_dev) {
        const uint32_t live = *nv_dev;
        nv = live < nv ? live : nv;
        const size_t zf = ((size_t)nv * 10 + 3) / 4;
        zero_f4 = zf < (size_t)zero_f4 ? (uint32_t)zf : zero_f4;
    }
    const uint32_t tid_lin = blockIdx.x * PROJ_WG + threadIdx.x;
    for (size_t i = tid_lin; i < zero_f4; i += (size_t)gridDim.x * PROJ_WG) zero_span[i] = make_float4(0.0f, 0.0f, 0.0f, 0.0f);
    const int lane = threadIdx.x & 63, wave = threadIdx.x >> 6;
    const uint32_t cg0 = (blockIdx.x * PROJ_WAVES + (uint32_t)wave) * (uint32_t)SPW;
    const uint32_t cg = lane < SPW ? cg0 + (uint32_t)lane : 0xFFFFFFFFu;
    uint32_t far_base = 0, far_cnt = 0;
    if (FAR) {
        far_cnt = cg < nv ? far_counts[cg] : 0u;
        uint32_t ahead = 0;
        const uint32_t group = blockIdx.x / FAR_GROUP_BLOCKS;
        for (uint32_t g = threadIdx.x; g < group; g += PROJ_WG) ahead += far_group_totals[g];
        { const uint32_t b = group * FAR_GROUP_BLOCKS + threadIdx.x; if (threadIdx.x < FAR_GROUP_BLOCKS && b < blockIdx.x) ahead += far_block_totals[b]; }
        uint32_t incl = far_cnt;
#pragma unroll
        for (int off = 1; off < 64; off <<= 1) {
            const uint32_t t = __shfl_up(incl, off);
            if (lane >= off) incl += t;
        }
#pragma unroll
        for (int off = 32; off > 0; off >>= 1) ahead += __shfl_down(ahead, off);
        if (lane == 63) s_far[wave] = incl;
        if (lane == 0) s_far[PROJ_WAVES + wave] = ahead;
        __syncthreads();
        uint32_t before = 0, block_ahead = 0, block_total = 0;
// ... 463 lines not shown
```

Before: 1356.

## Deal listed splats into depth-sort buckets directly from projection kernel

The projection kernel now uses the view's previous-frame depth quantile splitters to place each listed splat straight into a per-bucket region via atomic slot counters. This lets the depth sort skip its histogram and split launches and run a single bucket kernel. Double-buffered deal counters are cleared inside the projection kernel. On bucket overflow the host detects a flag and reruns the full sort, at the cost of extra atomics in K1 and a fallback path.

```diff
diff --git a/brush_amd/_ffi.py b/brush_amd/_ffi.py
--- a/brush_amd/_ffi.py
+++ b/brush_amd/_ffi.py
@@ -451,6 +451,10 @@
                      "bh_debug_split_counts": (C.c_int, [C.c_void_p, C.POINTER(C.c_uint32)]),
                      "bh_debug_depth_sort": (C.c_int, [C.c_void_p, C.c_void_p, C.c_void_p, C.c_void_p, C.c_uint32, C.c_void_p, C.c_void_p, C.c_void_p, C.c_void_p,
                                                        C.POINTER(C.c_int), C.POINTER(C.c_uint32)]),
+                     "bh_debug_depth_deal": (C.c_int, [C.c_void_p, C.c_void_p, C.c_void_p, C.c_void_p, C.c_uint32, C.c_void_p, C.c_void_p, C.c_void_p, C.c_void_p,
+                                                       C.c_uint32, C.c_uint32, C.POINTER(C.c_uint64), C.POINTER(C.c_int)]),
+                     "bh_debug_dsort_deal_counts": (C.c_int, [C.c_void_p, C.POINTER(C.c_uint32)]),
+                     "bh_debug_set_deal_capacity": (C.c_int, [C.c_void_p, C.c_uint32]),
                      "bh_debug_image_loss_window": (C.c_int, [C.c_void_p, C.c_void_p, C.c_void_p, C.c_uint32, C.c_uint32, C.POINTER(BhLossConfig), C.c_float, C.c_uint32,
                                                               C.c_uint32, C.c_void_p, C.c_void_p])}
 
diff --git a/brush_amd/csrc/api.hip b/brush_amd/csrc/api.hip
--- a/brush_amd/csrc/api.hip
+++ b/brush_amd/csrc/api.hip
@@ -7,6 +7,7 @@
 
 #include "../../include/brush_hip_intrinsics.h"
 #include "context.h"
+#include "depth_deal.h"
 #include "device_rng.h"
 #include "param_table.h"
 
@@ -270,6 +271,7 @@
         if (b.ptr) (void)hipFree(b.ptr);
     if (ctx->host_counters) (void)hipHostFree(ctx->host_counters);
     if (ctx->dsort_spl) (void)hipFree(ctx->dsort_spl);
+    if (ctx->deal_ctr) (void)hipFree(ctx->deal_ctr);
     if (ctx->sort_groups) (void)hipFree(ctx->sort_groups);
     if (ctx->readback_ev) (void)hipEventDestroy(ctx->readback_ev);
     if (ctx->gate_ev) (void)hipEventDestroy(ctx->gate_ev);
@@ -380,6 +382,8 @@
      [](bh_ctx* c, const char* v) { return parse_flag(v, &c->knob_generic_depth_sort); }},
     {"dsort_splitters", "0|1: the fused depth sort splits at the 254 depth quantiles of the view's previous frame (default 1) or always linearly over the frame's key range",
      [](bh_ctx* c, const char* v) { return parse_flag(v, &c->knob_dsort_splitters); }},
+    {"dsort_deal", "0|1: K1 deals the listed splats straight into the depth sort's buckets when the view's splitter table holds quantiles (default 1) or the histogram and split launches always run",
+     [](bh_ctx* c, const char* v) { return parse_flag(v, &c->knob_dsort_deal); }},
     {"tile_sort", "auto|bucket|lsd: the forward's tile sort (auto: bucket sort unless the view's pairs are concentrated in few tiles)",
      [](bh_ctx* c, const char* v) { const std::string w(v); if (w == "auto") { c->knob_tile_sort = 0; return true; } if (w == "bucket") { c->knob_tile_sort = 1; return true; } if (w == "lsd") { c->knob_tile_sort = 2; return true; } return false; }},
     {"spec_k5", "0|1: queue the list builder before the host has read the frame's counts (default 1; 0: behind the count readback)",
@@ -686,6 +690,13 @@
     float4* spec_vc = nullptr;
     uint32_t *spec_tile_ids = nullptr, *spec_isect_gids = nullptr;
     if (n > 0) {
+        fused_scan = depth_sort_supported(n) && !ctx->knob_generic_depth_sort;
+        const bool sums_on_device = fused_scan && !ctx->knob_readback_copy;
+        bool* spl_written = nullptr;
+        uint32_t* spl_listed = nullptr;
+        uint32_t* spl = view_splitters(view, cut_active, &spl_written, &spl_listed);
+        if (!spl && ctx->dsort_spl) { spl = ctx->dsort_spl; spl_written = &ctx->dsort_spl_written; spl_listed = &ctx->dsort_spl_keys; }
+        DealArgs dealt;
         {
             ProfScope ps(ctx, "ProjectSplats");
             if (!ctx->counters_ready) BH_HIP(ctx, hipMemsetAsync(counter_pairs, 0, 2 * counter_set_bytes, ctx->stream));
@@ -723,14 +734,14 @@
                 prep.span_f4 = (uint32_t)(req.grad_floats / 4);
                 ctx->clears.k1_cleared_span();
             }
+            BH_TRY(depth_deal_prepare(ctx, n, spl, sums_on_device && spl_written && *spl_written && depth_deal_table_usable(*spl_listed), &prep));
+            dealt = prep.deal;
             BH_TRY(launch_project_forward(ctx, f.u, n, mip, sh_degree, transforms, sh_coeffs, raw_opacities, depth_keys, isect_counts, max_radius,
                                           f.proj_by_gid, counters, prep, cut_active ? vtab : nullptr, near_counts));
             ctx->counter_phase ^= 1u;
             ctx->counters_ready = true;
         }
         auto* hslots = reinterpret_cast<unsigned long long*>(ctx->host_counters + 16);
-        fused_scan = depth_sort_supported(n) && !ctx->knob_generic_depth_sort;
-        const bool sums_on_device = fused_scan && !ctx->knob_readback_copy;
         const bool poll_tag = sums_on_device && !ctx->knob_event_waits;
         if (!sums_on_device) {
             BH_HIP(ctx, hipMemcpyAsync(hslots, counters, counter_read_bytes, hipMemcpyDeviceToHost, ctx->stream));
@@ -742,11 +753,9 @@
                 cum_early = (uint32_t*)ensure(ctx, SLOT_CUM_TILES_HIT, npad * 4);
                 if (!cum_early) return BH_ERR_OOM;
                 if (poll_tag && ++ctx->readback_tag == 0u) ctx->readback_tag = 1u;
-                bool* spl_written = nullptr;
-                uint32_t* spl = view_splitters(view, cut_active, &spl_written);
                 BH_TRY(depth_sort_scan(ctx, depth_keys, counters + COUNTER_MINMAX_WORD, cut_active ? near_counts : isect_counts, n, depths_sorted, f.gfc, cum_early,
                                        sums_on_device ? counters : nullptr, ctx->host_counters + 16, ctx->readback_ev, poll_tag ? ctx->readback_tag : 0u,
-                                       sums_on_device ? dev_sums : nullptr, spl, spl_written));
+                                       sums_on_device ? dev_sums : nullptr, spl, spl_written, &dealt));
             } else {
                 BH_TRY(radix_argsort(ctx, depth_keys, nullptr, n, 32, depths_sorted, f.gfc));
             }
@@ -786,6 +795,14 @@
         f.ni = (uint32_t)hc[1];
         near_total = cut_active ? (uint32_t)hc[2] : f.ni;
         f.nv = cut_active ? (uint32_t)hc[3] : nv_true;
+        if (dealt.ctr && reinterpret_cast<const volatile uint32_t*>(hslots)[HOST_DEAL_WORD] != 0u) {
+            ProfScope ps(ctx, "DepthSort");
+            ctx->deal_fallbacks++;
+            BH_TRY(depth_sort_scan(ctx, depth_keys, counters + COUNTER_MINMAX_WORD, cut_active ? near_counts : isect_counts, n, depths_sorted, f.gfc, cum_early,
+                                   counters, ctx->host_counters + 16, ctx->readback_ev, 0u, dev_sums, spl, spl_written));
+            k5_queued = false;
+        }
+        if (fused_scan && spl_listed && (spl_written == nullptr || *spl_written)) *spl_listed = f.nv;
     } else {
         BH_HIP(ctx, hipMemsetAsync(tile_offsets, 0, ((size_t)f.num_tiles * 2 + LPT_HEADER_WORDS) * 4, ctx->stream));
         if (visible_words) BH_HIP(ctx, hipMemsetAsync(f.visible, 0, visible_words * 4, ctx->stream));
@@ -1005,7 +1022,7 @@
     if (!ctx) return BH_ERR_INVALID_ARG;
     BH_HIP(ctx, hipSetDevice(ctx->device));
     if (ctx->far_job.pending) BH_TRY(finish_far_slice(ctx, nullptr));
-    if (ctx->dsort_spl) { BH_HIP(ctx, hipMemsetAsync(ctx->dsort_spl, 0, DSORT_SPL_STRIDE * 4, ctx->stream)); ctx->dsort_spl_written = false; }
+    if (ctx->dsort_spl) { BH_HIP(ctx, hipMemsetAsync(ctx->dsort_spl, 0, DSORT_SPL_STRIDE * 4, ctx->stream)); ctx->dsort_spl_written = false; ctx->dsort_spl_keys = 0u; }
     if (ctx->views.empty()) return 0;
     BH_HIP(ctx, hipStreamSynchronize(ctx->stream));
     deliver_pending_loss(ctx);
@@ -1384,6 +1401,64 @@
     BH_HIP(ctx, hipStreamSynchronize(ctx->stream));
     return 0;
 }
+__global__ __launch_bounds__(256) void debug_deal_kernel(const uint32_t* __restrict__ keys, const uint32_t* __restrict__ counts, uint32_t n, uint32_t stride, bh::DealArgs d) {
+    __shared__ uint32_t s_spl[bh::DEAL_SPL_WORDS];
+    bh::deal_stage(d, s_spl);
+    __syncthreads();
+    const uint32_t t = blockIdx.x * 256u + threadIdx.x;
+    if (t >= n) return;
+    const uint32_t e = (uint32_t)(((unsigned long long)t * stride) % n);
+    const uint32_t key = keys[e];
+    if (key != 0xFFFFFFFFu) bh::deal_put(d, bh::deal_take(d, s_spl, key, counts[e]), key, e);
+}
+extern "C" int bh_debug_depth_deal(bh_ctx* ctx, const uint32_t* keys, const uint32_t* minmax, const uint32_t* counts, uint32_t n, uint32_t* out_keys, uint32_t* out_vals,
+                                   uint32_t* cum, uint32_t* spl, uint32_t cap, uint32_t stride, unsigned long long* ctr_out, int* fell_back) {
+    if (!ctx) return BH_ERR_INVALID_ARG;
+    if (!keys || !minmax || !counts || !out_keys || !out_vals || !cum || !spl || !ctr_out || !fell_back || stride == 0u)
+        return set_error(ctx, BH_ERR_INVALID_ARG, "debug_depth_deal: bad argument");
+    if (n == 0 || !depth_sort_supported(n)) return set_error(ctx, BH_ERR_INVALID_ARG, "debug_depth_deal: n is outside the fused sort's reach");
+    BH_HIP(ctx, hipSetDevice(ctx->device));
+    DealArgs d;
+    d.spl = spl;
+    d.cap = cap ? cap : deal_capacity(n);
+    d.region = (uint2*)ensure(ctx, SLOT_DEAL_REGION, (size_t)DEAL_BUCKETS * d.cap * sizeof(uint2));
+    if (!d.region) return BH_ERR_OOM;
+    if (hipMalloc((void**)&d.ctr, (size_t)DEAL_SET_U64 * 8) != hipSuccess) { (void)hipGetLastError(); return BH_ERR_OOM; }
+    int rc = check_hip(ctx, hipMemsetAsync(d.ctr, 0, (size_t)DEAL_SET_U64 * 8, ctx->stream), "debug_depth_deal: clear");
+    if (rc == 0) {
+        hipLaunchKernelGGL(debug_deal_kernel, dim3((n + 255u) / 256u), dim3(256), 0, ctx->stream, keys, counts, n, stride, d);
+        rc = check_hip(ctx, hipGetLastError(), "debug_deal_kernel");
+    }
+    bool written = true;
+    if (rc == 0) rc = depth_sort_scan(ctx, keys, minmax, counts, n, out_keys, out_vals, cum, nullptr, nullptr, nullptr, 0u, nullptr, spl, &written, &d);
+    unsigned long long host[DEAL_BUCKETS + 1u];
+    if (rc == 0) rc = check_hip(ctx, hipMemcpy2DAsync(host, 8, d.ctr, (size_t)DEAL_LINE_U64 * 8, 8, DEAL_BUCKETS + 1u, hipMemcpyDeviceToHost, ctx->stream), "debug_depth_deal: counters");
+    if (rc == 0) rc = check_hip(ctx, hipStreamSynchronize(ctx->stream), "debug_depth_deal: sync");
+    if (rc == 0) {
+        for (uint32_t i = 0; i <= DEAL_BUCKETS; ++i) ctr_out[i] = host[i];
+        *fell_back = host[DEAL_BUCKETS] != 0ull ? 1 : 0;
+        if (*fell_back) {
+            ctx->deal_fallbacks++;
+            rc = depth_sort_scan(ctx, keys, minmax, counts, n, out_keys, out_vals, cum, nullptr, nullptr, nullptr, 0u, nullptr, spl, &written);
+            if (rc == 0) rc = check_hip(ctx, hipStreamSynchronize(ctx->stream), "debug_depth_deal: sync");
+        }
+    } else {
+        (void)hipStreamSynchronize(ctx->stream);
+    }
+    (void)hipFree(d.ctr);
+    return rc;
+}
+extern "C" int bh_debug_set_deal_capacity(bh_ctx* ctx, uint32_t cap) {
+    if (!ctx) return BH_ERR_INVALID_ARG;
+    ctx->deal_cap_override = cap;
+    return 0;
+}
+extern "C" int bh_debug_dsort_deal_counts(bh_ctx* ctx, uint32_t* out) {
+    if (!ctx || !out) return BH_ERR_INVALID_ARG;
+    out[0] = ctx->deal_frames;
+    out[1] = ctx->deal_fallbacks;
+    return 0;
+}
 extern "C" int bh_debug_image_loss_window(bh_ctx* ctx, const float* img_hwc4, const uint32_t* gt_packed, uint32_t h, uint32_t w, const BhLossConfig* cfg,
                                           float alpha_weight, uint32_t tile_y0, uint32_t tile_y1, float* loss_out, float* v_output) {
     if (!ctx) return BH_ERR_INVALID_ARG;
diff --git a/brush_amd/csrc/context.h b/brush_amd/csrc/context.h
--- a/brush_amd/csrc/context.h
+++ b/brush_amd/csrc/context.h
@@ -97,6 +97,7 @@
     SLOT_FEATURE_TERM,
     SLOT_FEATURE_GRAD,
     SLOT_ENVMAP_FRAME,
+    SLOT_DEAL_REGION,
     SLOT_SCENE,
     SLOT_COUNT
 };
@@ -118,6 +119,7 @@
 constexpr uint32_t FAR_GROUP_BLOCKS = 64;
 constexpr size_t COUNTER_READ_BYTES = COUNTER_SLOTS * 8 * COUNTER_K1_U64;
 constexpr uint32_t HOST_SUM_WORDS = 2 * COUNTER_K1_U64 + 1;
+constexpr uint32_t HOST_DEAL_WORD = HOST_SUM_WORDS;
 constexpr size_t HOST_LOSS_WORD = 16 + COUNTER_READ_BYTES / 4;
 constexpr size_t HOST_GATE_WORD = HOST_LOSS_WORD + 16;
 constexpr size_t HOST_GATE_TAG_WORD = HOST_GATE_WORD + 1;
@@ -148,6 +150,7 @@
     uint32_t last_pairs = 0;
     uint32_t complete_frames = 0;
     bool spl_written[2] = {false, false};
+    uint32_t spl_keys[2] = {0, 0};
     bool casual = false;
 };
 constexpr uint32_t CUT_MIN_PAIRS = 1500000u;
@@ -180,6 +183,16 @@
 constexpr uint32_t BWD_CKPT_MAX_SLOTS = 96u * 1024u;
 constexpr uint32_t DSORT_SPL_STRIDE = 260;
 constexpr uint32_t VIEW_SPL_WORDS = 2 * DSORT_SPL_STRIDE;
+constexpr uint32_t DEAL_BUCKETS = 255;
+constexpr uint32_t DEAL_LINE_U64 = 16;
+constexpr uint32_t DEAL_SET_U64 = (DEAL_BUCKETS + 1u) * DEAL_LINE_U64;
+constexpr uint32_t DEAL_OVERFLOW_U64 = DEAL_BUCKETS * DEAL_LINE_U64;
+struct DealArgs {
+    const uint32_t* spl = nullptr;
+    unsigned long long* ctr = nullptr;
+    uint2* region = nullptr;
+    uint32_t cap = 0;
+};
 constexpr size_t MAX_VIEW_STATES = 4096;
 constexpr uint64_t DIRECT_ALLREDUCE_MIN_FLOATS = 1u << 16;
 constexpr uint32_t AUTO_EXACT_FRAMES = 12;
@@ -427,12 +440,19 @@
     uint32_t knob_cut_margin_pct = 150;
     bh::FarJob far_job;
     uint32_t refine_n = 0, refine_new_n = 0;
+    bool dsort_deal_lds_raised = false;
     bool dsort_lds_raised = false;
     uint32_t* sort_groups = nullptr;
     size_t sort_groups_cap = 0, sort_groups_dirty = 0;
     uint32_t sort_groups_cur = 0;
     uint32_t* dsort_spl = nullptr;
     bool dsort_spl_written = false;
+    uint32_t dsort_spl_keys = 0;
+    unsigned long long* deal_ctr = nullptr;
+    uint32_t deal_phase = 0;
+    uint32_t deal_frames = 0, deal_fallbacks = 0;
+    uint32_t deal_cap_override = 0;
+    bool knob_dsort_deal = true;
     bool knob_dsort_splitters = true;
     bool adam_lds_raised = false;
     uint32_t update_lds_raised = 0;
@@ -514,7 +534,7 @@
 ViewState* frame_view(bh_ctx* ctx, const ForwardRequest& req, uint32_t tile_bw, uint32_t tile_bh, bool casual);
 bool cut_this_frame(const bh_ctx* ctx, ViewState* vs, bool allow_cut);
 uint32_t* view_table(const ViewState* vs);
-uint32_t* view_splitters(ViewState* vs, bool cut, bool** written);
+uint32_t* view_splitters(ViewState* vs, bool cut, bool** written, uint32_t** listed = nullptr);
 uint32_t cut_margin_pct(const bh_ctx* ctx, const ViewState* vs);
 uint32_t list_budget(bh_ctx* ctx, ViewState* cut_view, uint32_t near_total, uint32_t ni);
 void view_rendered(ViewState* vs, uint32_t ni);
@@ -590,6 +610,8 @@
     uint32_t split_min = SPLIT_MIN_WORK;
     float split_of_max = 0.45f;
     bool list_all_visible = false;
+    DealArgs deal;
+    unsigned long long* deal_next = nullptr;
 };
 int launch_project_forward(bh_ctx* ctx, const ViewUniforms& u, uint32_t n, bool mip, uint32_t sh_degree, const float* transforms,
                            const float* sh, const float* raw_opac, uint32_t* depth_keys, uint32_t* isect_counts, float* max_radius,
@@ -627,7 +649,9 @@
 bool depth_sort_supported(uint32_t n);
 int depth_sort_scan(bh_ctx* ctx, const uint32_t* keys, const uint32_t* minmax, const uint32_t* counts, uint32_t n, uint32_t* out_keys,
                     uint32_t* out_vals, uint32_t* cum, const uint32_t* rb_set = nullptr, uint32_t* rb_host = nullptr, hipEvent_t rb_done = nullptr,
-                    uint32_t rb_tag = 0, uint32_t* rb_dev = nullptr, uint32_t* spl = nullptr, bool* spl_written = nullptr);
+                    uint32_t rb_tag = 0, uint32_t* rb_dev = nullptr, uint32_t* spl = nullptr, bool* spl_written = nullptr, const DealArgs* dealt = nullptr);
+int depth_deal_prepare(bh_ctx* ctx, uint32_t n, const uint32_t* spl, bool table_usable, ForwardPrep* prep);
+bool depth_deal_table_usable(uint32_t listed_by_writer);
 int prefix_sum(bh_ctx* ctx, const uint32_t* in, const uint32_t* gather, uint32_t n, uint32_t* out, bool exclusive, const uint32_t* gate = nullptr);
 int launch_tile_offsets(bh_ctx* ctx, const uint32_t* tile_ids_sorted, uint32_t num_isect, uint32_t num_tiles,
                         uint32_t* tile_offsets, bool pre_zeroed = false);
diff --git a/brush_amd/csrc/depth_deal.h b/brush_amd/csrc/depth_deal.h
--- /dev/null
+++ b/brush_amd/csrc/depth_deal.h
@@ -0,0 +1,33 @@
+#pragma once
+#include "context.h"
+
+namespace bh {
+
+constexpr uint32_t DEAL_SPL_WORDS = 256;
+
+inline uint32_t deal_capacity(uint32_t n) { return n / 128u > 2048u ? (n + 127u) / 128u : 2048u; }
+
+BH_DEV void deal_stage(const DealArgs& d, uint32_t* s_spl ) {
+    for (uint32_t i = threadIdx.x; i < DEAL_SPL_WORDS; i += blockDim.x) s_spl[i] = d.spl[i];
+}
+
+BH_DEV uint32_t deal_digit(uint32_t key, const uint32_t* s_spl) {
+    uint32_t dg = 0;
+#pragma unroll
+    for (uint32_t step = 128u; step != 0u; step >>= 1) dg += s_spl[dg + step - 1u] <= key ? step : 0u;
+    return dg < DEAL_BUCKETS ? dg : DEAL_BUCKETS - 1u;
+}
+
+struct DealSlot { uint32_t bucket, slot; };
+BH_DEV DealSlot deal_take(const DealArgs& d, const uint32_t* s_spl, uint32_t key, uint32_t tiles) {
+    if (s_spl[255] == 0u) return DealSlot{DEAL_BUCKETS, 0u};
+    const uint32_t dg = deal_digit(key, s_spl);
+    const unsigned long long old = atomicAdd(&d.ctr[(size_t)dg * DEAL_LINE_U64], ((unsigned long long)tiles << 32) | 1ull);
+    return DealSlot{dg, (uint32_t)old};
+}
+BH_DEV void deal_put(const DealArgs& d, DealSlot at, uint32_t key, uint32_t id) {
+    if (at.bucket < DEAL_BUCKETS && at.slot < d.cap) d.region[(size_t)at.bucket * d.cap + at.slot] = make_uint2(key, id);
+    else d.ctr[DEAL_OVERFLOW_U64] = 1ull;
+}
+
+}
diff --git a/brush_amd/csrc/depth_sort.hip b/brush_amd/csrc/depth_sort.hip
--- a/brush_amd/csrc/depth_sort.hip
+++ b/brush_amd/csrc/depth_sort.hip
@@ -1,6 +1,7 @@
 #include <cstddef>
 
 #include "context.h"
+#include "depth_deal.h"
 #include "sort_groups.h"
 
 namespace bh {
@@ -92,7 +93,8 @@
     return ((unsigned long long)hi << 32) | lo;
 }
 
-BH_DEV void counter_sums_to_host(const uint32_t* __restrict__ set, uint32_t* __restrict__ host_sums, int lane, uint32_t tag, uint32_t* __restrict__ dev_sums) {
+BH_DEV void counter_sums_to_host(const uint32_t* __restrict__ set, uint32_t* __restrict__ host_sums, int lane, uint32_t tag, uint32_t* __restrict__ dev_sums,
+                                 uint32_t deal_overflow = 0u) {
     const unsigned long long* c64 = reinterpret_cast<const unsigned long long*>(set);
     unsigned long long tot[COUNTER_K1_U64];
 #pragma unroll
@@ -109,11 +111,12 @@
     if (lane == 0) {
         if (dev_sums) {
 #pragma unroll
-            for (uint32_t c = 0; c < COUNTER_K1_U64; ++c) dev_sums[c] = tot[c] > 0xFFFFFFFFull ? 0xFFFFFFFFu : (uint32_t)tot[c];
+            for (uint32_t c = 0; c < COUNTER_K1_U64; ++c) dev_sums[c] = deal_overflow ? 0u : (tot[c] > 0xFFFFFFFFull ? 0xFFFFFFFFu : (uint32_t)tot[c]);
         }
         volatile unsigned long long* h64 = reinterpret_cast<volatile unsigned long long*>(host_sums);
 #pragma unroll
         for (uint32_t c = 0; c < COUNTER_K1_U64; ++c) h64[c] = tot[c];
+        reinterpret_cast<volatile uint32_t*>(host_sums)[HOST_DEAL_WORD] = deal_overflow;
         if (tag) {
             __threadfence_system();
             reinterpret_cast<volatile uint32_t*>(host_sums)[HOST_SUM_WORDS - 1u] = tag;
@@ -409,21 +412,40 @@
     if (r >= start && r - start < size) spl_out[j] = sorted[r - start];
 }
 
-__global__ __launch_bounds__(BK_WG) void dsort_bucket_kernel(uint32_t* __restrict__ a_keys, uint32_t* __restrict__ a_vals ,
-                                                            uint32_t* __restrict__ out_keys, uint32_t* __restrict__ out_vals,
-                                                            const uint32_t* __restrict__ minmax, const uint32_t* __restrict__ digit_totals,
-                                                            const uint32_t* __restrict__ counts, uint32_t* __restrict__ cum ,
-                                                            uint32_t* __restrict__ spl_out , uint32_t spl_min_keys) {
+constexpr uint32_t TIE_RUN_MAX = 8;
+struct DealIn {
+    const unsigned long long* ctr;
+    const uint2* region;
+    uint32_t cap;
+    const uint32_t* rb_set; uint32_t* rb_host; uint32_t rb_tag; uint32_t* rb_dev;
+};
+template <bool DEAL>
+BH_DEV void dsort_bucket_body(uint32_t* __restrict__ a_keys, uint32_t* __restrict__ a_vals, uint32_t* __restrict__ out_keys, uint32_t* __restrict__ out_vals,
+                              const uint32_t* __restrict__ minmax, const uint32_t* __restrict__ digit_totals, const uint32_t* __restrict__ counts,
+                              uint32_t* __restrict__ cum, uint32_t* __restrict__ spl_out, uint32_t spl_min_keys, const DealIn& deal) {
     extern __shared__ __attribute__((aligned(16))) uint32_t s_dyn[];
     __shared__ uint32_t s_base[DS_RADIX];
     __shared__ uint32_t s_hist[DS_RADIX];
     __shared__ uint32_t s_red[2 * BK_WAVES];
     const int tid = threadIdx.x, lane = tid & 63, wave = tid >> 6;
-    const uint32_t b = blockIdx.x;
+    if (DEAL && blockIdx.x == 0u) {
+        if (wave == 0 && deal.rb_set) counter_sums_to_host(deal.rb_set, deal.rb_host, tid, deal.rb_tag, deal.rb_dev, deal.ctr[DEAL_OVERFLOW_U64] != 0ull ? 1u : 0u);
+        return;
+    }
+    if (DEAL && deal.ctr[DEAL_OVERFLOW_U64] != 0ull) return;
+    const uint32_t b = DEAL ? blockIdx.x - 1u : blockIdx.x;
+    const uint2* reg = DEAL ? deal.region + (size_t)b * deal.cap : nullptr;
     uint32_t start, size, tiles_before, nv;
     {
-        const uint32_t gt = tid < DS_RADIX ? digit_totals[tid] : 0u;
-        const uint32_t ct = tid < 255 ? digit_totals[DS_RADIX + tid] : 0u;
+        uint32_t gt, ct;
+        if (DEAL) {
+            const unsigned long long w = tid < (int)DEAL_BUCKETS ? deal.ctr[(size_t)tid * DEAL_LINE_U64] : 0ull;
+            gt = (uint32_t)w;
+            ct = (uint32_t)(w >> 32);
+        } else {
+            gt = tid < DS_RADIX ? digit_totals[tid] : 0u;
+            ct = tid < 255 ? digit_totals[DS_RADIX + tid] : 0u;
+        }
         uint32_t tot;
         const uint32_t gex = bk_excl_scan(gt, nv, s_red);
         const uint32_t cex = bk_excl_scan(ct, tot, s_red);
@@ -460,30 +482,34 @@
         uint32_t* fdb = fcnt + BK_WAVES * FAST_NDIG;
         uint32_t lo = 0xFFFFFFFFu, hi = 0u;
         for (uint32_t i = tid; i < size; i += BK_WG) {
-            const uint32_t k = a_keys[start + i];
+            uint32_t k, v;
+            if (DEAL) { const uint2 kv = reg[i]; k = kv.x; v = kv.y; }
+            else { k = a_keys[start + i]; v = a_vals[start + i]; }
             s_dyn[i] = k;
-            s_dyn[FAST_CAP + i] = a_vals[start + i];
+            s_dyn[FAST_CAP + i] = v;
             lo = min(lo, k);
             hi = max(hi, k);
         }
-        const uint32_t bits = bk_key_bits(lo, hi, s_red);
-        const uint32_t passes = (bits + 8u) / 9u;
-        const uint32_t base_w = passes ? bits / passes : 0u, wide = passes ? bits % passes : 0u;
+        const uint32_t kbits = bk_key_bits(lo, hi, s_red);
         const unsigned long long lt_mask = (1ull << lane) - 1ull;
         const uint32_t steps = (size + (uint32_t)BK_WG - 1u) / (uint32_t)BK_WG;
         const uint32_t wave_first = wave * steps * 64u;
         uint32_t cur = 0;
+        auto lsd_sort = [&](const bool by_id, const uint32_t slo, const uint32_t bits) {
+        const uint32_t passes = (bits + 8u) / 9u;
+        const uint32_t base_w = passes ? bits / passes : 0u, wide = passes ? bits % passes : 0u;
         for (uint32_t p = 0; p < passes; ++p) {
             const uint32_t width = base_w + (p < wide ? 1u : 0u);
             const uint32_t pshift = p * base_w + (p < wide ? p : wide);
             const uint32_t mask = (1u << width) - 1u;
             const uint32_t* sk = s_dyn + cur * (2 * FAST_CAP); const uint32_t* sv = sk + FAST_CAP;
+            const uint32_t* ss = by_id ? sv : sk;
             uint32_t* dk = s_dyn + (cur ^ 1u) * (2 * FAST_CAP); uint32_t* dv = dk + FAST_CAP;
             for (int i = tid; i < BK_WAVES * FAST_NDIG; i += BK_WG) fcnt[i] = 0;
             __syncthreads();
             for (uint32_t r = 0; r < steps; ++r) {
                 const uint32_t e = wave_first + r * 64u + lane;
-                if (e < size) atomicAdd(&fcnt[wave * FAST_NDIG + (((sk[e] - lo) >> pshift) & mask)], 1u);
+                if (e < size) atomicAdd(&fcnt[wave * FAST_NDIG + (((ss[e] - slo) >> pshift) & mask)], 1u);
             }
             __syncthreads();
             {
@@ -505,7 +531,7 @@
                 const uint32_t e = wave_first + r * 64u + lane;
                 const bool valid = e < size;
                 const uint32_t key = valid ? sk[e] : 0u, val = valid ? sv[e] : 0u;
-                const uint32_t d = valid ? ((key - lo) >> pshift) & mask : mask;
+                const uint32_t d = valid ? (((by_id ? val : key) - slo) >> pshift) & mask : mask;
                 uint32_t plo = 0xFFFFFFFFu, phi = 0xFFFFFFFFu;
                 for (uint32_t bb = 0; bb < width; ++bb) {
                     const uint32_t bit = (d >> bb) & 1u;
@@ -523,6 +549,33 @@
             __syncthreads();
             cur ^= 1u;
         }
+        };
+        lsd_sort(false, lo, kbits);
+        if (DEAL) {
+            const uint32_t* tk = s_dyn + cur * (2 * FAST_CAP); uint32_t* tv = s_dyn + cur * (2 * FAST_CAP) + FAST_CAP;
+            int tied = 0;
+            for (uint32_t i = tid; i < size; i += BK_WG) {
+                const uint32_t k = tk[i];
+                if (i + 1u < size && tk[i + 1u] == k && (i == 0u || tk[i - 1u] != k)) {
+                    uint32_t e = i + 2u;
+                    while (e < size && e - i <= TIE_RUN_MAX && tk[e] == k) ++e;
+                    if (e - i > TIE_RUN_MAX) { tied = 1; continue; }
+                    for (uint32_t a = i + 1u; a < e; ++a) {
+                        const uint32_t v = tv[a];
+                        uint32_t c = a;
+                        while (c > i && tv[c - 1u] > v) { tv[c] = tv[c - 1u]; --c; }
+                        tv[c] = v;
+                    }
+                }
+            }
+            if (__syncthreads_or(tied)) {
+                uint32_t ilo = 0xFFFFFFFFu, ihi = 0u;
+                for (uint32_t i = tid; i < size; i += BK_WG) { ilo = min(ilo, tv[i]); ihi = max(ihi, tv[i]); }
+                const uint32_t ibits = bk_key_bits(ilo, ihi, s_red);
+                lsd_sort(true, ilo, ibits);
+                lsd_sort(false, lo, kbits);
+            }
+        }
         const uint32_t* fk = s_dyn + cur * (2 * FAST_CAP); const uint32_t* fv = fk + FAST_CAP;
         uint32_t* spare = s_dyn + (cur ^ 1u) * (2 * FAST_CAP);
         bk_write_splitters(fk, start, size, nv, spl_out, spl_min_keys);
@@ -562,6 +615,59 @@
         return;
     }
     ChunkLds<BK_WG>& L = *reinterpret_cast<ChunkLds<BK_WG>*>(s_dyn);
+    if (DEAL) {
+        uint32_t klo = 0xFFFFFFFFu, khi = 0u, ilo = 0xFFFFFFFFu, ihi = 0u;
+        for (uint32_t i = tid; i < size; i += BK_WG) {
+            const uint2 kv = reg[i];
+            klo = min(klo, kv.x); khi = max(khi, kv.x);
+            ilo = min(ilo, kv.y); ihi = max(ihi, kv.y);
+        }
+        const uint32_t kbits = bk_key_bits(klo, khi, s_red), ibits = bk_key_bits(ilo, ihi, s_red);
+        const uint32_t kpasses = (kbits + 7u) / 8u, ipasses = (ibits + 7u) / 8u, passes = kpasses + ipasses;
+        uint32_t* src_k = (passes & 1u) ? a_keys : out_keys; uint32_t* src_v = (passes & 1u) ? a_vals : out_vals;
+        uint32_t* dst_k = (passes & 1u) ? out_keys : a_keys; uint32_t* dst_v = (passes & 1u) ? out_vals : a_vals;
+        for (uint32_t i = tid; i < size; i += BK_WG) {
+            const uint2 kv = reg[i];
+            src_k[start + i] = kv.x;
+            src_v[start + i] = kv.y;
+        }
+        __threadfence_block();
+        __syncthreads();
+        const uint32_t nchunks = (size + DS_TILE - 1) / DS_TILE;
+        for (uint32_t p = 0; p < passes; ++p) {
+            const bool by_id = p < ipasses;
+            const uint32_t q = by_id ? p : p - ipasses, sbits = by_id ? ibits : kbits, np = by_id ? ipasses : kpasses, slo = by_id ? ilo : klo;
+            const uint32_t base_w = sbits / np, wide = sbits % np;
+            const uint32_t width = base_w + (q < wide ? 1u : 0u);
+            const uint32_t pshift = q * base_w + (q < wide ? q : wide);
+            const uint32_t mask = (1u << width) - 1u;
+            auto digit = [=](uint32_t x) { return ((x - slo) >> pshift) & mask; };
+            const uint32_t* dsrc = by_id ? src_v : src_k;
+            if (tid < DS_RADIX) s_hist[tid] = 0;
+            __syncthreads();
+            for (uint32_t i = tid; i < size; i += BK_WG) atomicAdd(&s_hist[digit(dsrc[start + i])], 1u);
+            __syncthreads();
+            {
+                uint32_t tot;
+                const uint32_t ex = bk_excl_scan(tid < DS_RADIX ? s_hist[tid] : 0u, tot, s_red);
+                if (tid < DS_RADIX) s_base[tid] = start + ex;
+            }
+            __syncthreads();
+            for (uint32_t c = 0; c < nchunks; ++c) {
+                const uint32_t first = start + c * DS_TILE;
+                const uint32_t count = size - c * DS_TILE < (uint32_t)DS_TILE ? size - c * DS_TILE : (uint32_t)DS_TILE;
+                if (by_id) scatter_chunk<BK_WG>(L, s_base, src_v, src_k, first, count, dst_v, dst_k, digit);
+                else scatter_chunk<BK_WG>(L, s_base, src_k, src_v, first, count, dst_k, dst_v, digit);
+            }
+            __threadfence_block();
+            __syncthreads();
+            uint32_t* tk = src_k; src_k = dst_k; dst_k = tk;
+            uint32_t* tv = src_v; src_v = dst_v; dst_v = tv;
+        }
+        bk_write_splitters(out_keys + start, start, size, nv, spl_out, spl_min_keys);
+        if (cum != nullptr) bk_scan_counts(out_vals + start, size, counts, tiles_before, cum + start, &L.keys[0], s_red);
+        return;
+    }
     uint32_t lo = 0xFFFFFFFFu, hi = 0u;
     for (uint32_t i = tid; i < size; i += BK_WG) {
         const uint32_t k = a_keys[start + i];
@@ -605,6 +711,20 @@
     }
     bk_write_splitters(out_keys + start, start, size, nv, spl_out, spl_min_keys);
     if (cum != nullptr) bk_scan_counts(out_vals + start, size, counts, tiles_before, cum + start, &L.keys[0], s_red);
+}
+
+__global__ __launch_bounds__(BK_WG) void dsort_bucket_kernel(uint32_t* __restrict__ a_keys, uint32_t* __restrict__ a_vals ,
+                                                            uint32_t* __restrict__ out_keys, uint32_t* __restrict__ out_vals,
+                                                            const uint32_t* __restrict__ minmax, const uint32_t* __restrict__ digit_totals,
+                                                            const uint32_t* __restrict__ counts, uint32_t* __restrict__ cum ,
+                                                            uint32_t* __restrict__ spl_out , uint32_t spl_min_keys) {
+    dsort_bucket_body<false>(a_keys, a_vals, out_keys, out_vals, minmax, digit_totals, counts, cum, spl_out, spl_min_keys, DealIn{});
+}
+__global__ __launch_bounds__(BK_WG) void dsort_deal_bucket_kernel(uint32_t* __restrict__ a_keys, uint32_t* __restrict__ a_vals ,
+                                                                 uint32_t* __restrict__ out_keys, uint32_t* __restrict__ out_vals,
+                                                                 const uint32_t* __restrict__ minmax, const uint32_t* __restrict__ counts,
+                                                                 uint32_t* __restrict__ cum, uint32_t* __restrict__ spl_out, uint32_t spl_min_keys, DealIn deal) {
+    dsort_bucket_body<true>(a_keys, a_vals, out_keys, out_vals, minmax, nullptr, counts, cum, spl_out, spl_min_keys, deal);
 }
 
 #define BH_DSORT_MAX_N (16u << 20)
@@ -645,10 +765,53 @@
     return 0;
 }
 
+constexpr uint32_t DEAL_MIN_N = 16384;
+int depth_deal_prepare(bh_ctx* ctx, uint32_t n, const uint32_t* spl, bool table_usable, ForwardPrep* prep) {
+    prep->deal = DealArgs{};
+    prep->deal_next = nullptr;
+    if (ctx->deal_ctr == nullptr) {
+        if (!ctx->knob_dsort_deal) return 0;
+        if (hipMalloc((void**)&ctx->deal_ctr, (size_t)2 * DEAL_SET_U64 * 8) != hipSuccess) { (void)hipGetLastError(); ctx->deal_ctr = nullptr; return BH_ERR_OOM; }
+        BH_HIP(ctx, hipMemsetAsync(ctx->deal_ctr, 0, (size_t)2 * DEAL_SET_U64 * 8, ctx->stream));
+        ctx->deal_phase = 0u;
+    }
+    unsigned long long* cur = ctx->deal_ctr + (size_t)DEAL_SET_U64 * (ctx->deal_phase & 1u);
+    prep->deal_next = ctx->deal_ctr + (size_t)DEAL_SET_U64 * ((ctx->deal_phase & 1u) ^ 1u);
+    ctx->deal_phase ^= 1u;
+    if (!ctx->knob_dsort_deal || !ctx->knob_dsort_splitters || spl == nullptr || !table_usable || n < DEAL_MIN_N || !depth_sort_supported(n)) return 0;
+    const uint32_t cap = ctx->deal_cap_override ? ctx->deal_cap_override : deal_capacity(n);
+    uint2* region = (uint2*)ensure(ctx, SLOT_DEAL_REGION, (size_t)DEAL_BUCKETS * cap * sizeof(uint2));
+    if (!region) return BH_ERR_OOM;
+    prep->deal.spl = spl;
+    prep->deal.ctr = cur;
+    prep->deal.region = region;
+    prep->deal.cap = cap;
+    return 0;
+}
+bool depth_deal_table_usable(uint32_t listed_by_writer) { return listed_by_writer >= SPL_MIN_KEYS; }
+
 int depth_sort_scan(bh_ctx* ctx, const uint32_t* keys, const uint32_t* minmax, const uint32_t* counts, uint32_t n, uint32_t* out_keys,
                     uint32_t* out_vals, uint32_t* cum, const uint32_t* rb_set, uint32_t* rb_host, hipEvent_t rb_done, uint32_t rb_tag, uint32_t* rb_dev, uint32_t* spl,
-                    bool* spl_written) {
+                    bool* spl_written, const DealArgs* dealt) {
     if (n == 0) return 0;
+    if (dealt && dealt->ctr) {
+        uint32_t* a_keys = (uint32_t*)ensure(ctx, SLOT_SORT_KEYS_A, (size_t)n * 4);
+        uint32_t* a_vals = (uint32_t*)ensure(ctx, SLOT_SORT_VALS_A, (size_t)n * 4);
+        if (!a_keys || !a_vals) return BH_ERR_OOM;
+        if (!ctx->dsort_deal_lds_raised) {
+            BH_HIP(ctx, hipFuncSetAttribute((const void*)dsort_deal_bucket_kernel, hipFuncAttributeMaxDynamicSharedMemorySize, (int)(FAST_LDS_WORDS * 4)));
+            ctx->dsort_deal_lds_raised = true;
+        }
+        DealIn in;
+        in.ctr = dealt->ctr; in.region = dealt->region; in.cap = dealt->cap;
+        in.rb_set = rb_set; in.rb_host = rb_host; in.rb_tag = rb_tag; in.rb_dev = rb_dev;
+        hipLaunchKernelGGL(dsort_deal_bucket_kernel, dim3(DEAL_BUCKETS + 1u), dim3(BK_WG), FAST_LDS_WORDS * 4, ctx->stream, a_keys, a_vals, out_keys, out_vals, minmax, counts, cum,
+                           const_cast<uint32_t*>(dealt->spl), SPL_MIN_KEYS, in);
+        BH_LAUNCH_CHECK(ctx, "dsort_deal_bucket_kernel");
+        if (rb_set && !rb_tag) BH_HIP(ctx, hipEventRecord(rb_done, ctx->stream));
+        ctx->deal_frames++;
+        return 0;
+    }
     const uint32_t nblocks = (n + DS_TILE - 1) / DS_TILE;
     if (!ctx->knob_dsort_splitters) spl = nullptr;
     else if (spl == nullptr) {
diff --git a/brush_amd/csrc/lists.hip b/brush_amd/csrc/lists.hip
--- a/brush_amd/csrc/lists.hip
+++ b/brush_amd/csrc/lists.hip
@@ -115,8 +115,9 @@
 
 uint32_t* view_table(const ViewState* vs) { return vs ? vs->zcut : nullptr; }
 
-uint32_t* view_splitters(ViewState* vs, bool cut, bool** written) {
+uint32_t* view_splitters(ViewState* vs, bool cut, bool** written, uint32_t** listed) {
     *written = vs ? &vs->spl_written[cut ? 1 : 0] : nullptr;
+    if (listed) *listed = vs ? &vs->spl_keys[cut ? 1 : 0] : nullptr;
     return vs ? vs->zcut + 2 * (size_t)vs->tile_bw * vs->tile_bh + (cut ? DSORT_SPL_STRIDE : 0u) : nullptr;
 }
 
diff --git a/brush_amd/csrc/project.hip b/brush_amd/csrc/project.hip
--- a/brush_amd/csrc/project.hip
+++ b/brush_amd/csrc/project.hip
@@ -1,4 +1,5 @@
 #include "context.h"
+#include "depth_deal.h"
 #include "device_camera.h"
 #include "device_f64_sum.h"
 #include "device_sh.h"
@@ -205,9 +206,11 @@
     __shared__ uint32_t s_listed[PROJ_WAVES];
     __shared__ uint32_t s_kmax[PROJ_WAVES];
     __shared__ uint32_t s_nmax[PROJ_WAVES];
+    __shared__ uint32_t s_bins[ORDER_BINS];
+    static_assert(DEAL_SPL_WORDS <= ORDER_BINS, "the splitters are staged in the bins' words");
+    uint32_t* const s_spl = s_bins;
     const uint32_t gid = blockIdx.x * PROJ_WG + threadIdx.x;
     if (prep.order_out && blockIdx.x < 8u) {
-        __shared__ uint32_t s_bins[ORDER_BINS];
         const uint32_t per = band_slots(prep.order_tiles);
         __shared__ uint32_t s_band_work, s_band_cnt, s_band_tail, s_band_max;
         for (uint32_t i = threadIdx.x; i < ORDER_BINS; i += PROJ_WG) s_bins[i] = 0u;
@@ -272,10 +275,15 @@
         }
         __syncthreads();
     }
+    if (prep.deal.ctr) {
+        deal_stage(prep.deal, s_spl);
+        __syncthreads();
+    }
     if (gid < prep.visible_words) prep.visible[gid] = 0u;
     if (gid < prep.tile_words) prep.tile_table[gid] = 0u;
     if (gid < prep.slice_words) prep.slice_table[gid] = 0u;
     if (gid < COUNTER_SET_U64 && prep.next_counters) prep.next_counters[gid] = 0ull;
+    if (gid < DEAL_SET_U64 && prep.deal_next) prep.deal_next[gid] = 0ull;
     for (size_t i = gid; i < prep.span_f4; i += (size_t)gridDim.x * PROJ_WG) prep.span[i] = make_float4(0.0f, 0.0f, 0.0f, 0.0f);
     const int lane = threadIdx.x & 63, wave = threadIdx.x >> 6;
     uint32_t key = 0xFFFFFFFFu;
@@ -353,6 +361,9 @@
     const uint32_t tiles_hit = nb ? w.count[wrank] : 0u;
     const uint32_t near_hit = (nb && zcut) ? w.near[wrank] : 0u;
     const bool listed = visible && (!zcut || near_hit > 0u || prep.list_all_visible);
+    constexpr bool DEAL_EARLY = DEG <= 2;
+    DealSlot deal_place = DealSlot{0u, 0u};
+    if (DEAL_EARLY && prep.deal.ctr && listed) deal_place = deal_take(prep.deal, s_spl, key, zcut ? near_hit : tiles_hit);
     if (listed) {
         const Vec3A v = normalize(sub(mean, camera_pos(u)));
         constexpr int C = (DEG + 1) * (DEG + 1);
@@ -401,6 +412,8 @@
         s_nmax[wave] = nmax;
     }
     __syncthreads();
+    if (!DEAL_EARLY && prep.deal.ctr && listed) deal_place = deal_take(prep.deal, s_spl, key, zcut ? near_hit : tiles_hit);
+    if (prep.deal.ctr && listed) deal_put(prep.deal, deal_place, key, gid);
     if (threadIdx.x == 0) {
         uint32_t v = 0, h = 0, nh = 0, ls = 0, km = 0, nm = 0;
 #pragma unroll
@@ -449,6 +462,10 @@
     if (prep.next_counters && COUNTER_SET_U64 > covered) {
         BH_HIP(ctx, hipMemsetAsync(prep.next_counters, 0, COUNTER_SET_BYTES, ctx->stream));
         prep.next_counters = nullptr;
+    }
+    if (prep.deal_next && DEAL_SET_U64 > covered) {
+        BH_HIP(ctx, hipMemsetAsync(prep.deal_next, 0, (size_t)DEAL_SET_U64 * 8, ctx->stream));
+        prep.deal_next = nullptr;
     }
     if (prep.tile_table && prep.tile_words > covered) {
         BH_HIP(ctx, hipMemsetAsync(prep.tile_table, 0, (size_t)prep.tile_words * 4, ctx->stream));
```

After: 1385, median of 6. 2.2% higher.
